# zhangganlin/GlORIE-SLAM

Measured on AMD Instinct MI355X. Metric: DSPO BA-update iters/sec + rendered rays/sec, 640x480 Replica keyframe graph, higher is better.
Workload: dtype f16 corr/ConvGRU, f32 Jacobians, f64 solve; render: f32 (decoder matmuls as 3-term f16 splits, f32 accumulate); 1 GPU; G8: 8 keyframes, 36 edges, 60x80 (640x480/8), BA itrs=2, DSPO stages alternating, context part of the GRU gates (one map per source keyframe) re-evaluated for all keyframes every 12 steps; multiview_filter.thresh = 0.25 (reference ships 0.01, configs/mono_point_slam.yaml:75: with untrained weights 0.01 rejects > 80 % of every frame and no depth_scale step would reach stage 2); render: 524k-point c; edges_local=36, edges_total=36, hw=4800, keyframes=8, parallelism=single GPU

## Files before the change

glorie_slam_amd/_lib.py:

```python
import ctypes
import os
import threading

import torch

_PKG_DIR = os.path.dirname(os.path.abspath(__file__))
LIB_PATH = os.path.join(_PKG_DIR, "lib", "libglorie_hip.so")

GLORIE_F16, GLORIE_F32 = 0, 1
_STATUS = {0: "GLORIE_OK", -1: "GLORIE_EINVAL", -2: "GLORIE_EHIP", -3: "GLORIE_ENOMEM",
           -4: "GLORIE_EUNSUPPORTED"}

_c_int, _c_f, _vp, _sz = ctypes.c_int, ctypes.c_float, ctypes.c_void_p, ctypes.c_size_t

SIGNATURES = {
    "glorie_version": (ctypes.c_char_p, []),
    "glorie_last_hip_error": (_c_int, []),
    "glorie_ctx_create": (_c_int, [ctypes.POINTER(_vp), _sz]),
    "glorie_ctx_destroy": (_c_int, [_vp]),
    "glorie_ctx_reserve": (_c_int, [_vp, _sz]),
    "glorie_ctx_generation": (ctypes.c_ulonglong, [_vp]),
    "glorie_corr_index_fwd": (_c_int, [_vp, _vp, _vp] + [_c_int] * 7 + [_vp]),
    "glorie_corr_lookup_pyramid": (_c_int, [_vp, _c_int, _vp, _vp] + [_c_int] * 7 + [_vp]),
    "glorie_corr_otf": (_c_int, [_vp, _vp, _c_int, _vp, _vp, _vp, _vp] + [_c_int] * 4 + [_vp]),
    "glorie_corr_otf_encode": (_c_int, [_vp, _vp, _c_int, _vp, _vp, _vp, _vp] + [_c_int] * 4 + [_vp, _vp, _vp, _c_int, _vp]),
    "glorie_altcorr_fwd": (_c_int, [_vp] * 4 + [_c_int] * 8 + [_vp]),
    "glorie_bias_act": (_c_int, [_vp, _c_int, _vp, _vp, _c_int, ctypes.c_long, _c_int, _c_int, _vp]),
    "glorie_gru_glo_terms": (_c_int, [_vp, _c_int, _vp, _vp, _c_int, _vp, _vp, _c_int, _vp, _c_int, _vp, _c_int, _c_int, _vp]),
    "glorie_gru_gate_zr": (_c_int, [_vp, _c_int, _vp, _c_int, _vp, _c_int, _vp, _c_int, _vp, _c_int, _c_int, _c_int, _vp]),
    "glorie_gru_gate_q": (_c_int, [_vp, _c_int, _vp, _c_int, _vp, _c_int, _vp, _c_int, _vp, _c_int, _vp, _c_int, _c_int, _c_int, _vp]),
    "glorie_segment_mean": (_c_int, [_vp, _c_int, _vp, _c_int, _vp, _c_int, _vp, _c_int, _c_int, _c_int, _vp]),
    "glorie_conv3x3_small": (_c_int, [_vp, _c_int, _vp, _c_int, _vp, _vp, _c_int, _c_int, _c_int, ctypes.c_float, _vp, _vp, _c_int, _c_int, _c_int, _vp]),
    "glorie_gru_glo_from_tiles": (_c_int, [_vp, _vp, _vp, _c_int, _vp, _c_int, _c_int, _vp]),
    "glorie_update_bookkeeping": (_c_int, [_vp, _vp, _vp, ctypes.c_long, _vp, _vp, _vp, _vp, _c_int, _c_int, _c_f, _vp, _c_int,
                                           _vp]),
    "glorie_conv_igemm_heads": (_c_int, [_vp, _c_int, _c_int, _vp, _c_int, _c_int, _vp, _vp, _c_int, _c_int, _vp, _vp,
                                         _c_int, _c_int, _c_int, _c_int, _vp]),
    "glorie_conv_upsample": (_c_int, [_vp, _c_int, _c_int, _vp, _vp, _vp, _vp, _vp, _c_int, _c_int, _c_int, _c_int, _vp]),
    "glorie_conv_stencil": (_c_int, [_vp, _vp, _c_int, _c_int, _c_int, ctypes.c_float, _vp, _vp, _c_int, _c_int, _c_int, _vp]),
    "glorie_conv_igemm": (_c_int, [_vp, _c_int, _c_int, _vp, _c_int, _c_int, _vp, _c_int, _c_int, _c_int, _vp,
                                   _c_int, _c_int, _vp, _c_int, _vp, _c_int, _vp, _c_int, _vp, _c_int, _vp, _c_int, _vp,
                                   _c_int, _c_int, _c_int, _vp]),
    "glorie_flow_conv7": (_c_int, [_vp, _vp, _vp, _vp, _c_int, _c_int, _c_int, _c_int, _vp]),
    "glorie_motion": (_c_int, [_vp, _vp, _vp, _vp, _c_int, _c_int, _c_int, ctypes.c_float, _vp]),
    "glorie_motion_padded": (_c_int, [_vp, _vp, _vp, _vp, _c_int, _c_int, _c_int, ctypes.c_float, _vp]),
    "glorie_flow_pad": (_c_int, [_vp, _vp, _c_int, _c_int, _c_int, _vp]),
    "glorie_flow_conv7_padded": (_c_int, [_vp, _vp, _vp, _vp, _c_int, _c_int, _c_int, _c_int, _vp]),
    "glorie_publish_flag": (_c_int, [_vp, _vp, _vp, _vp]),
    "glorie_dspo_prepare": (_c_int, [_vp] * 4 + [_c_int] * 4 + [ctypes.c_float, _c_int, ctypes.c_float, _vp, _vp, _c_int] + [_vp] * 9),
    "glorie_corr_lookup_pyramid_tiled": (_c_int, [_vp, _c_int, _vp, _vp] + [_c_int] * 5 + [_vp]),
    "glorie_corr_build": (_c_int, [_vp] * 5 + [_c_int] * 5 + [_vp]),
    "glorie_corr_lookup_arena": (_c_int, [_vp, _c_int, _vp, _vp, _vp] + [_c_int] * 5 + [_vp]),
    "glorie_corr_lookup_tiled_cl": (_c_int, [_vp, _c_int, _vp, _vp, _c_int, _vp] + [_c_int] * 5 + [_vp]),
    "glorie_corr_dm_level_halfs": (ctypes.c_long, [_c_int, _c_int, _c_int]),
    "glorie_corr_dm_build": (_c_int, [_vp] * 5 + [_c_int] * 5 + [_vp]),
    "glorie_corr_dm_lookup": (_c_int, [_vp, _vp, _vp, _c_int, _c_int, _c_int, _c_int, _vp, _vp, _vp, _vp, _c_int, _vp]),
    "glorie_valid_depth_mask": (_c_int, [_vp] * 4 + [_c_int] * 4 + [ctypes.c_float, _c_int, _vp, _vp, _vp]),
    "glorie_reproject": (_c_int, [_vp] * 7 + [_c_int] * 3 + [_vp]),
    "glorie_reproject_motion": (_c_int, [_vp] * 9 + [_c_int] * 3 + [ctypes.c_float, _vp]),
    "glorie_frame_distance": (_c_int, [_vp] * 6 + [_c_int] * 3 + [_c_f, _vp]),
    "glorie_iproj": (_c_int, [_vp] * 4 + [_c_int] * 3 + [_vp]),
    "glorie_depth_filter": (_c_int, [_vp] * 6 + [_c_int] * 4 + [_vp]),
    "glorie_cvx_upsample": (_c_int, [_vp] * 4 + [_c_int] * 5 + [_vp]),
    "glorie_cvx_upsample_nhwc": (_c_int, [_vp, _vp, _vp, _c_int, _vp, _c_int, _c_int, _c_int, _c_int, _vp]),
    "glorie_ba": (_c_int, [_vp] * 10 + [_c_int] * 8 + [_c_f, _c_f, _c_int, _c_int, _vp, _vp, _vp]),
    "glorie_ba_build_system": (_c_int, [_vp] * 10 + [_c_int] * 8 + [_vp, _vp]),
    "glorie_ba_solve_update": (_c_int, [_vp] * 5 + [_c_int] * 7 + [_c_f, _c_f, _c_int, _c_int] + [_vp] * 4),
    "glorie_ba_pack_system": (_c_int, [_vp, _vp, _c_int, _c_int, _vp]),
    "glorie_comm_unique_id": (_c_int, [_vp]),
    "glorie_comm_init": (_c_int, [_vp, _vp, _c_int, _c_int]),
    "glorie_comm_destroy": (_c_int, [_vp]),
    "glorie_comm_world": (_c_int, [_vp]),
    "glorie_allreduce_normal_eq": (_c_int, [_vp, _vp, _sz, _vp]),
    "glorie_allgather_rows": (_c_int, [_vp, _vp, _vp, _sz, _vp]),
    "glorie_dspo_scale_shift": (_c_int, [_vp] * 14 + [_c_int] * 6 + [_c_f, _c_f, _c_f, _vp, _vp]),
    "glorie_knn_build": (_c_int, [_vp, _vp, _c_int, _c_f, _c_int, _vp, _vp, _vp, _vp]),
    "glorie_knn_query": (_c_int, [_vp, _vp, _vp, _vp, _c_int, _c_int, _c_f, _vp, _vp, _vp, _vp, _vp]),
    "glorie_idw_gather": (_c_int, [_vp, _vp, _vp, _vp, _c_int, _c_int, _c_int, _c_f, _vp, _c_int,
                                   _c_int, _vp, _vp, _vp, _vp]),
    "glorie_knn_query_image": (_c_int, [_vp, _vp, _vp, _vp, _c_int, _c_int, _c_f, _vp, _vp, _vp, _vp, _c_int, _c_int,
                                        _vp]),
    "glorie_knn_query_weights": (_c_int, [_vp, _vp, _vp, _vp, _c_int, _c_f, _vp, _vp, _vp, _vp, _c_int, _c_int, _c_int, _c_int,
                                          _c_int, _vp, _vp, _vp]),
    "glorie_idw_gather2": (_c_int, [_vp, _vp, _vp, _vp, _vp, _c_int, _c_int, _c_int, _c_f, _vp, _c_int,
                                    _c_int, _vp, _vp, _vp, _vp, _vp]),
    "glorie_decoder_pack_floats": (_sz, []),
    "glorie_render_mlp": (_c_int, [_vp] * 10 + [_c_int, _vp, _vp, _c_int, _vp, _vp]),
    "glorie_composite": (_c_int, [_vp, _vp, _c_int, _c_int, _c_f, _vp, _vp, _vp, _vp, _vp]),
    "glorie_ray_samples": (_c_int, [_vp] * 5 + [_c_int, _c_int, _c_f, _c_f] + [_vp] * 6),
    "glorie_ray_samples_camera": (_c_int, [_vp, _c_int, ctypes.c_long] + [_vp] * 3 + [_c_int, _c_int, _c_f, _c_f] + [_vp] * 6),
    "glorie_proj_depth": (_c_int, [_vp, _vp, ctypes.c_long, _vp, _c_f, _c_f, _c_f, _c_f, _c_int, _c_int, _vp, _vp]),
    "glorie_ray_counts": (_c_int, [_vp, _c_int, _c_int, _c_int, _vp, _vp, _vp]),
    "glorie_render_train_workspace": (_sz, [ctypes.c_long]),
    "glorie_render_train_fwd": (_c_int, [_vp] * 9 + [ctypes.c_long, _c_int, _vp, _vp, _vp]),
    "glorie_render_train_bwd": (_c_int, [_vp] * 10 + [ctypes.c_long, _c_int, _vp, _vp, _vp, _vp, _vp]),
    "glorie_composite_bwd": (_c_int, [_vp, _vp, _c_int, _c_int, _c_f, _vp, _vp, _vp, _vp]),
    "glorie_adam_step": (_c_int, [_vp, _vp, _vp, _vp, ctypes.c_long, _c_f, _c_f, _c_f, _c_f, _c_int, _vp, _c_int, _vp]),
    "glorie_adam_multi": (_c_int, [_vp, _c_int, ctypes.c_long, _c_int, _vp, _vp]),
    "glorie_adam_step_dev": (_c_int, [_vp, _vp, _vp, _vp, ctypes.c_long, _c_f, _c_f, _c_f, _c_f, _vp, _vp, _c_int, _vp]),
    "glorie_adam_multi_dev": (_c_int, [_vp, _c_int, ctypes.c_long, _vp, _vp, _vp]),
    "glorie_counter_add": (_c_int, [_vp, _c_int, _vp]),
    "glorie_ba_status": (_c_int, [_vp, ctypes.POINTER(_c_int), _vp]),
    "glorie_ba_set_gate": (_c_int, [_vp, _vp, _vp]),
    "glorie_pix_warp_workspace": (_sz, [_c_int]),
    "glorie_pix_warp_fwd": (_c_int, [_vp] * 4 + [_c_int, _vp, _vp, _c_int, _vp, _vp, _c_int, _c_int, _c_int] + [_c_f] * 4
                            + [_vp, _c_int] + [_vp] * 5 + [_vp]),
    "glorie_pix_warp_bwd": (_c_int, [_vp, _vp, _vp, _c_int, _vp, _vp]),
    "glorie_frustum_select_workspace": (_sz, [_c_int]),
    "glorie_frustum_select": (_c_int, [_vp, _c_int, _vp] + [_c_f] * 4 + [_c_int, _c_int, _c_f] + [_vp] * 6),
    "glorie_keyframe_overlap": (_c_int, [_vp, _vp, _vp, _c_int, _c_int, _vp, _c_int] + [_c_f] * 4
                                + [_c_int, _c_int, _c_f, _vp, _vp]),
    "glorie_color_grad_maps": (_c_int, [_vp, _c_int, _c_int, _c_int, _vp] + [ctypes.c_double] * 4 + [_vp] * 6),
    "glorie_topm_workspace": (_sz, [_c_int]),
    "glorie_topm": (_c_int, [_vp, _c_int, _c_int, _vp, _vp, _vp, _vp]),
    "glorie_npc_deform_workspace": (_sz, [_c_int]),
    "glorie_npc_deform": (_c_int, [_vp] * 4 + [_c_int] * 3 + [_vp] * 5 + [ctypes.c_long, _vp, ctypes.c_long, _c_int]
                          + [_c_f, _c_f, _c_int] + [_c_f] * 4 + [_vp, _vp, _vp]),
    "glorie_iproj_dirty": (_c_int, [_vp] * 5 + [_c_int] * 3 + [_vp, _vp, _c_int, _vp]),
    "glorie_proxy_depth": (_c_int, [_vp, _vp] + [_c_int] * 4 + [_vp] + [_c_f] * 4 + [_vp] * 5),
}

_lib = None
_lock = threading.Lock()


class GlorieError(RuntimeError):
    pass


def load():
    global _lib
    with _lock:
        if _lib is None:
            if not os.path.exists(LIB_PATH):
                raise GlorieError(
                    f"{LIB_PATH} is missing: build it with `python glorie_slam_amd/build.py` "
                    "(or __graft_entry__.build()); there is no CPU fallback for the hot path")
            lib = ctypes.CDLL(LIB_PATH)
            for name, (res, args) in SIGNATURES.items():
                fn = getattr(lib, name)
                fn.restype = res
                fn.argtypes = args
            _lib = lib
    return _lib


def check(status, what):
    if status != 0:
        lib = load()
        raise GlorieError(f"{what} failed: {_STATUS.get(status, status)} "
                          f"(hipError {lib.glorie_last_hip_error()})")


def stream_ptr(device=None):
    return ctypes.c_void_p(torch.cuda.current_stream(device).cuda_stream)


def ptr(t):
    return ctypes.c_void_p(t.data_ptr()) if t is not None else ctypes.c_void_p(0)


BA_TARGETS_HWC = 2


def need_cuda(*tensors):
    for t in tensors:
        if t is not None and not t.is_cuda:
            raise GlorieError("glorie_hip kernels take device tensors; got a CPU tensor "
                              "(there is no CPU fallback on the product path)")


def need_contiguous(**named):
    for k, t in named.items():
        if t is not None and not t.is_contiguous():
            raise RuntimeError(f"{k} must be contiguous")


def dtype_code(t):
    if t.dtype == torch.float16:
        return GLORIE_F16
    if t.dtype == torch.float32:
        return GLORIE_F32
    raise GlorieError(f"unsupported dtype {t.dtype}")


class Context:
# ... 36 lines not shown
```

glorie_slam_amd/csrc/ba.hip:

```cpp
#include <hip/hip_runtime.h>
#include <stdint.h>
#include <math.h>
#include "common.hiph"
#include "se3.hiph"
#include "ba_common.hiph"

namespace glorie {

__device__ __forceinline__ void block_inclusive_scan(int* a, int n) {
  const int tid = threadIdx.x;
  for (int off = 1; off < n; off <<= 1) {
    int tmp[4];
#pragma unroll
    for (int q = 0; q < 4; ++q) {
      const int f = tid + q * 1024;
      tmp[q] = (f < n) ? a[f] + (f >= off ? a[f - off] : 0) : 0;
    }
    __syncthreads();
#pragma unroll
    for (int q = 0; q < 4; ++q) {
      const int f = tid + q * 1024;
      if (f < n) a[f] = tmp[q];
    }
    __syncthreads();
// ... 986 lines not shown
}

constexpr int kPanelRows = 128;
__global__ __launch_bounds__(1024) void chol_panel_gemm_kernel(BaWork wk, int n, int j0, int nb) {
  if (ba_skipped(wk)) return;
  __shared__ double Wl[kCB * kCBP], P[kPanelRows * kCBP];
  if (wk.status[0] & (BA_ST_SOLVE_ABORT | BA_ST_M_MISMATCH)) return;
  const int tid = threadIdx.x, br = tid >> 5, bc = tid & 31;
  double* A = wk.Hd;
  const int base = j0 + nb, rem = n - base;
  if (br < nb && bc < nb) {
    double v = 0.0;
    if (bc < br) v = A[(size_t)(j0 + bc) * n + j0 + br];
    else if (bc == br) v = 1.0 / A[(size_t)(j0 + br) * n + j0 + br];
    Wl[br * kCBP + bc] = v;
  }
  const int t0 = blockIdx.x * kPanelRows;
  for (int idx = tid; idx < kPanelRows * kCB; idx += 1024) {
    const int tl = idx >> 5, m = idx & 31, t = t0 + tl;
    P[tl * kCBP + m] = (t <= rem && m < nb) ? A[(size_t)(t < rem ? base + t : n) * n + j0 + m] : 0.0;
  }
  __syncthreads();
  const int tl = tid & (kPanelRows - 1), g = tid >> 7, t = t0 + tl;
  double x[4];
#pragma unroll
  for (int q = 0; q < 4; ++q) x[q] = 0.0;
  const double* wg = Wl + g * kCBP;
  const double* ap = P + tl * kCBP;
#pragma unroll 4
  for (int m = 0; m < kCB; ++m) {
    const double am = ap[m];
#pragma unroll
    for (int q = 0; q < 4; ++q) x[q] = fma(am, (m <= 8 * q + g) ? wg[8 * q * kCBP + m] : 0.0, x[q]);
  }
  if (t <= rem) {
    double* arow = A + (size_t)(t < rem ? base + t : n) * n + j0;
#pragma unroll
    for (int q = 0; q < 4; ++q) {
      const int c = 8 * q + g;
      if (c < nb) arow[c] = x[q];
    }
  }
}

__global__ __launch_bounds__(256) void chol_backsub_block_kernel(BaWork wk, int n, int j0, int nb) {
  if (ba_skipped(wk)) return;
  __shared__ double Wl[kCB * kCBP], yb[kCB], xb[kCB];
  const int tid = threadIdx.x;
  double* A = wk.Hd;
  double* y = A + (size_t)n * n;
  if (wk.status[0] & (BA_ST_SOLVE_ABORT | BA_ST_M_MISMATCH)) {
    if (blockIdx.x == 0 && tid < nb) wk.dx[j0 + tid] = 0.0f;
    return;
  }
  for (int idx = tid; idx < kCB * kCB; idx += 256) {
    const int r = idx >> 5, c = idx & 31;
    double v = 0.0;
    if (r < nb && c < nb) {
      if (c < r) v = A[(size_t)(j0 + c) * n + j0 + r];
      else if (c == r) v = 1.0 / A[(size_t)(j0 + r) * n + j0 + r];
    }
    Wl[r * kCBP + c] = v;
  }
  if (tid < kCB) yb[tid] = tid < nb ? y[j0 + tid] : 0.0;
  __syncthreads();
  if (tid < kCB) {
    double v = 0.0;
    for (int r = tid; r < nb; ++r) v = fma(Wl[r * kCBP + tid], yb[r], v);
    xb[tid] = v;
  }
  __syncthreads();
  if (blockIdx.x == 0 && tid < nb) wk.dx[j0 + tid] = (float)xb[tid];
  const int r = blockIdx.x * 256 + tid;
  if (r < j0) {
    double v = y[r];
    for (int c = 0; c < nb; ++c) v -= A[(size_t)(j0 + c) * n + r] * xb[c];
    y[r] = v;
  }
}

__global__ __launch_bounds__(kBaThreads) void ba_update_kernel(
    BaWork wk, float* __restrict__ poses, float* __restrict__ disps,
    const int64_t* __restrict__ ii, const int64_t* __restrict__ jj, int HW, int t0, int t1,
    int motion_only, int depth_only, float* __restrict__ dx_out, float* __restrict__ dz_out) {
  if (ba_skipped(wk)) return;
  constexpr int EB = 128;
  __shared__ float ys[EB * 6];
  const int tid = threadIdx.x;
  const int s = blockIdx.y;
  if (wk.status[0] & BA_ST_M_MISMATCH) return;
  const int P = t1 - t0;
  if (blockIdx.x == 0 && s == 0) {
    for (int p = tid; p < P; p += kBaThreads) {
      float xi[6];
#pragma unroll
      for (int q = 0; q < 6; ++q) xi[q] = wk.dx[p * 6 + q];
      if (dx_out) {
#pragma unroll
        for (int q = 0; q < 6; ++q) dx_out[p * 6 + q] = xi[q];
      }
      if (!depth_only) {
        float* pp = poses + (size_t)(t0 + p) * 7;
        const Pose g = se3_retract(xi, load_pose(pp));
        pp[0] = g.t.x; pp[1] = g.t.y; pp[2] = g.t.z;
        pp[3] = g.q.x; pp[4] = g.q.y; pp[5] = g.q.z; pp[6] = g.q.w;
      }
    }
  }
  if (motion_only) return;
  const int k = wk.kx[s];
  const int e0 = wk.csr_ptr[s];
  const int deg = wk.csr_ptr[s + 1] - e0;
  const int pk = k - t0;
  const bool self_on = (pk > 0 && pk < P);
  const int px = blockIdx.x * kBaThreads + tid;
  float dw = 0.0f;
  for (int a0 = 0; a0 < deg; a0 += EB) {
    const int nb = min(EB, deg - a0);
    __syncthreads();
    for (int idx = tid; idx < nb * 6; idx += kBaThreads) {
      const int a = idx / 6, r = idx % 6;
      const int n = wk.csr_edge[e0 + a0 + a];
      const int pj = (int)jj[n] - t0;
      float y = (pj > 0 && pj < P) ? wk.dx[pj * 6 + r] : 0.0f;
      if (self_on) {
        const float* L = wk.Ledge + (size_t)n * 36;
        float acc = 0.0f;
#pragma unroll
        for (int m = 0; m < 6; ++m) acc += L[m * 6 + r] * wk.dx[pk * 6 + m];
        y -= acc;
      }
      ys[idx] = y;
    }
    __syncthreads();
    if (px < HW) {
      for (int a = 0; a < nb; ++a) {
        const int n = wk.csr_edge[e0 + a0 + a];
#pragma unroll
        for (int r = 0; r < 6; ++r) dw += wk.Eij[((size_t)n * 6 + r) * HW + px] * ys[a * 6 + r];
      }
    }
  }
  if (px >= HW) return;
  const float dz = wk.Q[(size_t)s * HW + px] * (wk.W[(size_t)s * HW + px] - dw);
  disps[(size_t)k * HW + px] += dz;
  if (dz_out) dz_out[(size_t)s * HW + px] = dz;
}

int ba_prepare(const BaWork& wk, const int64_t* ii, int B, int N, int M, int t0, int t1,
               hipStream_t st) {
  const size_t prep_lds = sizeof(int) * ((size_t)3 * B + (size_t)N);
  if (prep_lds > 150 * 1024) return GLORIE_EUNSUPPORTED;
  static PerDeviceOnce attr_set;
  if (attr_set.first()) {
    (void)hipFuncSetAttribute(reinterpret_cast<const void*>(ba_prepare_kernel),
                              hipFuncAttributeMaxDynamicSharedMemorySize, 150 * 1024);
  }
  hipLaunchKernelGGL(ba_prepare_kernel, dim3(1), dim3(1024), prep_lds, st, wk, ii, B, N, M, t0, t1);
  return check_launch();
}

}

using namespace glorie;

namespace glorie {

struct BaPlan {
  BaWork wk;
  int B, N, M, h, w, HW, t0, t1, P, n6, ppt, chunk_px, nchunks;
  size_t scratch_used;
};

static int ba_plan(glorie_ctx* ctx, int B, int N, int M, int h, int w, int t0, int t1,
                   double* hv_ext, BaPlan& pl) {
  if (!ctx || B < 0 || N < 0 || M < 0 || h < 0 || w < 0 || t1 < t0) return GLORIE_EINVAL;
  if (B > kMaxFramesLds || N > kMaxEdgesLds || t1 > B) return GLORIE_EUNSUPPORTED;
  pl.B = B; pl.N = N; pl.M = M; pl.h = h; pl.w = w; pl.HW = h * w; pl.t0 = t0; pl.t1 = t1;
  pl.P = t1 - t0; pl.n6 = 6 * pl.P;
#ifdef EXP_BA_CHUNK_WGS
  constexpr long kChunkWgs = EXP_BA_CHUNK_WGS;
#else
  constexpr long kChunkWgs = 256;
#endif
  int ppt = 1;
  const int per1 = (pl.HW + kBaThreads - 1) / kBaThreads;
  while (ppt < 4 && (long)M * ((per1 + ppt - 1) / ppt) > kChunkWgs) ++ppt;
  pl.ppt = ppt;
  pl.chunk_px = kBaThreads * ppt;
  pl.nchunks = (pl.HW + pl.chunk_px - 1) / pl.chunk_px;
  const size_t HW = pl.HW, n6 = pl.n6;
  size_t off = 0;
  auto carve = [&](size_t bytes) { size_t o = off; off = align_up(off + bytes, 256); return o; };
  const size_t o_slot = carve(sizeof(int) * (size_t)B);
  const size_t o_kx = carve(sizeof(int) * (size_t)(M + 1));
  const size_t o_ptr = carve(sizeof(int) * (size_t)(M + 2));
  const size_t o_edge = carve(sizeof(int) * (size_t)N);
  const size_t o_L = carve(sizeof(float) * 36 * (size_t)N);
  const size_t o_E = carve(sizeof(float) * 6 * (size_t)N * HW);
  const size_t o_Hp = carve(sizeof(float) * 27 * (size_t)N * pl.nchunks);
  const size_t o_Q = carve(sizeof(float) * (size_t)M * HW);
  const size_t o_W = carve(sizeof(float) * (size_t)M * HW);
  const size_t o_CW = carve(sizeof(float) * 2 * (size_t)N * HW);
  const size_t o_Hd = carve(sizeof(double) * (n6 * n6 + n6));
  const size_t o_acc = carve(2 * sizeof(unsigned long long) * (n6 * n6 + n6));
  const size_t o_dx = carve(sizeof(float) * n6);
  GLORIE_TRY(ctx_reserve(ctx, off));
  pl.scratch_used = off;
  char* base = reinterpret_cast<char*>(ctx->scratch);
  BaWork& wk = pl.wk;
  wk.slot_of_frame = reinterpret_cast<int*>(base + o_slot);
  wk.kx = reinterpret_cast<int*>(base + o_kx);
  wk.csr_ptr = reinterpret_cast<int*>(base + o_ptr);
  wk.csr_edge = reinterpret_cast<int*>(base + o_edge);
  wk.status = ctx->dstatus;
  wk.Ledge = reinterpret_cast<float*>(base + o_L);
  wk.Eij = reinterpret_cast<float*>(base + o_E);
  wk.Hpart = reinterpret_cast<float*>(base + o_Hp);
  wk.Q = reinterpret_cast<float*>(base + o_Q);
  wk.W = reinterpret_cast<float*>(base + o_W);
  wk.CWpart = reinterpret_cast<float*>(base + o_CW);
  wk.Hd = hv_ext ? hv_ext : reinterpret_cast<double*>(base + o_Hd);
  wk.vd = wk.Hd + n6 * n6;
  wk.Hacc = reinterpret_cast<unsigned long long*>(base + o_acc);
  wk.dx = reinterpret_cast<float*>(base + o_dx);
  wk.gate = ctx->ba_gate;
  wk.gate_hits = nullptr;
  static PerDeviceOnce attr_set;
  if (attr_set.first()) {
    (void)hipFuncSetAttribute(reinterpret_cast<const void*>(ba_solve_fused_kernel),
                              hipFuncAttributeMaxDynamicSharedMemorySize, 160 * 1024 - 64);
    (void)hipFuncSetAttribute(reinterpret_cast<const void*>(ba_solve_band_kernel),
                              hipFuncAttributeMaxDynamicSharedMemorySize, 160 * 1024 - 64);
  }
  return GLORIE_OK;
}

static int ba_build_system(const BaPlan& pl, const float* poses, const float* disps,
                           const float* intrinsics, const float* disps_sens, const float* targets,
                           const float* weights, const float* eta, const int64_t* ii,
                           const int64_t* jj, int flags, bool to_f64, hipStream_t st) {
  const BaWork& wk = pl.wk;
  const int motion_only = flags & 1, hwc = (flags & GLORIE_BA_TARGETS_HWC) ? 1 : 0;
  hipLaunchKernelGGL(ba_jacobian_kernel, dim3(pl.nchunks, pl.N), dim3(kBaThreads), 0, st, wk, poses,
                     disps, intrinsics, disps_sens, targets, weights, eta, ii, jj, pl.HW, pl.w,
                     pl.nchunks, pl.ppt, motion_only, hwc, (long)pl.n6 * pl.n6 + pl.n6);
  if (!motion_only)
    hipLaunchKernelGGL(ba_gram_kernel, dim3(pl.nchunks, pl.M), dim3(kBaThreads), 0, st, wk, ii, jj, pl.HW,
                       pl.chunk_px, pl.t0, pl.t1, pl.nchunks, eta, disps, disps_sens);
  else
    hipLaunchKernelGGL(ba_assemble_kernel, dim3(pl.N), dim3(64), 0, st, wk, ii, jj, pl.nchunks, pl.t0, pl.t1);
  if (to_f64) {
    const long total = (long)pl.n6 * pl.n6 + pl.n6;
    hipLaunchKernelGGL(ba_system_f64_kernel, dim3((unsigned)((total + 255) / 256)), dim3(256), 0, st, wk, total);
  }
  return check_launch();
}

static int ba_solve_update(const BaPlan& pl, float* poses, float* disps, const int64_t* ii,
                           const int64_t* jj, float lm, float ep, int motion_only, int depth_only,
                           float* dx_out, float* dz_out, bool from_acc, hipStream_t st) {
  const BaWork& wk = pl.wk;
  const int n6 = pl.n6;
  if (n6 <= kSolveMaxN) {
    const int bwf = n6 > 1 ? n6 - 1 : 1;
    const int need = n6 * (bwf + 1) + 2 * n6;
    hipLaunchKernelGGL(ba_solve_band_kernel, dim3(1), dim3(kBandThreads), sizeof(double) * (size_t)need, st, wk, n6,
                       lm, ep, need, bwf, from_acc ? 1 : 0);
  } else if (n6 <= kFusedMaxN) {
    const size_t rows = (size_t)(n6 + 1 > kCB ? n6 + 1 - kCB : 1);
    const size_t lds = sizeof(double) * (2 * kCB * kCBP + (rows * kCBP > (size_t)n6 ? rows * kCBP : (size_t)n6));
    const int band_doubles = (160 * 1024 - 256) / (int)sizeof(double);
    hipLaunchKernelGGL(ba_bandwidth_kernel, dim3(n6), dim3(64), 0, st, wk, n6);
    hipLaunchKernelGGL(ba_solve_band_kernel, dim3(1), dim3(kBandThreads), sizeof(double) * (size_t)band_doubles, st,
                       wk, n6, lm, ep, band_doubles, -1, 0);
    hipLaunchKernelGGL(ba_solve_fused_kernel, dim3(1), dim3(1024), lds, st, wk, n6, lm, ep);
  } else {
    hipLaunchKernelGGL(chol_damp_kernel, dim3((n6 + 255) / 256), dim3(256), 0, st, wk, n6, lm, ep);
    for (int j0 = 0; j0 < n6; j0 += kCB) {
      const int nb = (n6 - j0 < kCB) ? (n6 - j0) : kCB;
      const int rem = n6 - j0 - nb;
      hipLaunchKernelGGL(chol_diag_inv_kernel, dim3(1), dim3(1024), 0, st, wk, n6, j0, nb);
      hipLaunchKernelGGL(chol_panel_gemm_kernel, dim3((rem + kPanelRows) / kPanelRows), dim3(1024), 0, st, wk, n6, j0, nb);
      if (rem > 0) {
        const int tl = (rem + kTrailTile) / kTrailTile;
        hipLaunchKernelGGL(chol_trail_kernel, dim3(tl, tl), dim3(256), 0, st, wk, n6, j0, nb);
      }
    }
    for (int j0 = ((n6 - 1) / kCB) * kCB; j0 >= 0; j0 -= kCB) {
      const int nb = (n6 - j0 < kCB) ? (n6 - j0) : kCB;
      hipLaunchKernelGGL(chol_backsub_block_kernel, dim3(j0 > 0 ? (j0 + 255) / 256 : 1), dim3(256), 0, st, wk, n6, j0,
                         nb);
    }
  }
  const int upd_chunks = (pl.HW + kBaThreads - 1) / kBaThreads;
  hipLaunchKernelGGL(ba_update_kernel, dim3(upd_chunks, pl.M), dim3(kBaThreads), 0, st, wk, poses,
                     disps, ii, jj, pl.HW, pl.t0, pl.t1, motion_only, depth_only, dx_out, dz_out);
  return check_launch();
}

__global__ __launch_bounds__(256) void ba_zero_gated_kernel(const int* __restrict__ gate, int* __restrict__ dstatus,
                                                            double* __restrict__ hv, size_t n) {
  if (*gate != 0) return;
  const size_t i = (size_t)blockIdx.x * 256 + threadIdx.x;
  if (i < 4) dstatus[i] = 0;
  if (i < n) hv[i] = 0.0;
}

}

extern "C" int glorie_ba(glorie_ctx* ctx, float* poses, float* disps, const float* intrinsics,
                         const float* disps_sens, const float* targets, const float* weights,
                         const float* eta, const int64_t* ii, const int64_t* jj, int B, int N,
                         int M, int h, int w, int t0, int t1, int iterations, float lm, float ep,
                         int motion_only, int depth_only, float* dx_out, float* dz_out,
                         void* stream) {
  if (iterations < 0) return GLORIE_EINVAL;
  const int flags = motion_only;
  motion_only = flags & 1;
  BaPlan pl;
  GLORIE_TRY(ba_plan(ctx, B, N, M, h, w, t0, t1, nullptr, pl));
  if (N == 0 || pl.P == 0 || pl.HW == 0 || iterations == 0) return GLORIE_OK;
  if (!poses || !disps || !intrinsics || !targets || !weights || !ii || !jj) return GLORIE_EINVAL;
  if (!motion_only && !eta) return GLORIE_EINVAL;
  hipStream_t st = (hipStream_t)stream;
  GLORIE_TRY(ctx_poison(ctx, pl.scratch_used, st));
  {
    BaWork w0 = pl.wk;
    if (ctx->ba_gate && ctx->ba_gate_count) { w0.gate_hits = ctx->ba_gate_hits; ctx->ba_gate_count = false; }
    GLORIE_TRY(ba_prepare(w0, ii, B, N, M, t0, t1, st));
  }
  const bool direct = pl.n6 <= kSolveMaxN;
  for (int it = 0; it < iterations; ++it) {
    GLORIE_TRY(ba_build_system(pl, poses, disps, intrinsics, disps_sens, targets, weights, eta, ii, jj,
                               flags, !direct, st));
    GLORIE_TRY(ba_solve_update(pl, poses, disps, ii, jj, lm, ep, motion_only, depth_only, dx_out,
                               dz_out, direct, st));
  }
  return GLORIE_OK;
}

extern "C" int glorie_ba_build_system(glorie_ctx* ctx, const float* poses, const float* disps,
                                      const float* intrinsics, const float* disps_sens,
                                      const float* targets, const float* weights, const float* eta,
                                      const int64_t* ii, const int64_t* jj, int B, int N, int M,
                                      int h, int w, int t0, int t1, int motion_only, double* hv_out,
                                      void* stream) {
  BaPlan pl;
  GLORIE_TRY(ba_plan(ctx, B, N, M, h, w, t0, t1, hv_out, pl));
  if (!hv_out || pl.P == 0) return GLORIE_EINVAL;
  hipStream_t st = (hipStream_t)stream;
  if (N == 0 || pl.HW == 0) {
    const size_t nhv = (size_t)pl.n6 * pl.n6 + pl.n6;
    if (ctx->ba_gate) {
      hipLaunchKernelGGL(ba_zero_gated_kernel, dim3((unsigned)((nhv + 255) / 256)), dim3(256), 0, st, ctx->ba_gate,
                         ctx->dstatus, hv_out, nhv);
      return check_launch();
    }
    GLORIE_TRY(check_hip(hipMemsetAsync(ctx->dstatus, 0, 4 * sizeof(int), st)));
    return check_hip(hipMemsetAsync(hv_out, 0, sizeof(double) * nhv, st));
  }
  if (!poses || !disps || !intrinsics || !targets || !weights || !ii || !jj) return GLORIE_EINVAL;
  if (!(motion_only & 1) && !eta) return GLORIE_EINVAL;
  GLORIE_TRY(ctx_poison(ctx, pl.scratch_used, st));
  {
    BaWork w0 = pl.wk;
    if (ctx->ba_gate && ctx->ba_gate_count) { w0.gate_hits = ctx->ba_gate_hits; ctx->ba_gate_count = false; }
    GLORIE_TRY(ba_prepare(w0, ii, B, N, M, t0, t1, st));
  }
  return ba_build_system(pl, poses, disps, intrinsics, disps_sens, targets, weights, eta, ii, jj,
                         motion_only, true, st);
}

extern "C" int glorie_ba_solve_update(glorie_ctx* ctx, float* poses, float* disps,
                                      const int64_t* ii, const int64_t* jj, int B, int N, int M,
                                      int h, int w, int t0, int t1, float lm, float ep,
                                      int motion_only, int depth_only, const double* hv,
                                      float* dx_out, float* dz_out, void* stream) {
  BaPlan pl;
  GLORIE_TRY(ba_plan(ctx, B, N, M, h, w, t0, t1, const_cast<double*>(hv), pl));
  if (!hv || !poses || !disps || pl.P == 0) return GLORIE_EINVAL;
  if (N > 0 && (!ii || !jj)) return GLORIE_EINVAL;
  hipStream_t st = (hipStream_t)stream;
  if (N == 0 || pl.HW == 0) {
    pl.M = 1;
    return ba_solve_update(pl, poses, disps, ii, jj, lm, ep, 1, depth_only, dx_out,
                           nullptr, false, st);
  }
  return ba_solve_update(pl, poses, disps, ii, jj, lm, ep, motion_only, depth_only, dx_out, dz_out,
                         false, st);
}

extern "C" int glorie_ba_set_gate(glorie_ctx* ctx, const int* run_if_zero, int* hits) {
  if (!ctx) return GLORIE_EINVAL;
  ctx->ba_gate = run_if_zero;
  ctx->ba_gate_hits = run_if_zero ? hits : nullptr;
  ctx->ba_gate_count = run_if_zero && hits;
  return GLORIE_OK;
}

namespace glorie {
__global__ __launch_bounds__(256) void hv_pack_kernel(const double* __restrict__ hv, double* __restrict__ packed,
                                                      int n, int unpack) {
  const int r = blockIdx.y, c = blockIdx.x * 256 + threadIdx.x;
  double* dense = const_cast<double*>(hv);
  if (r == n) {
    if (c < n) {
      const size_t k = (size_t)n * (n + 1) / 2 + c;
      if (unpack) dense[(size_t)n * n + c] = packed[k];
      else packed[k] = hv[(size_t)n * n + c];
    }
    return;
  }
  if (c > r) return;
  const size_t k = (size_t)r * (r + 1) / 2 + c;
  if (unpack) dense[(size_t)r * n + c] = packed[k];
  else packed[k] = hv[(size_t)r * n + c];
}
}

extern "C" int glorie_ba_pack_system(const double* hv, double* packed, int n6, int unpack, void* stream) {
  if (!hv || !packed || n6 < 0) return GLORIE_EINVAL;
  if (n6 == 0) return GLORIE_OK;
  hipLaunchKernelGGL(glorie::hv_pack_kernel, dim3((n6 + 255) / 256, n6 + 1), dim3(256), 0, (hipStream_t)stream, hv,
                     packed, n6, unpack);
  return glorie::check_launch();
}

extern "C" int glorie_ba_status(glorie_ctx* ctx, int* status_out, void* stream) {
  if (!ctx || !status_out) return GLORIE_EINVAL;
  hipStream_t st = (hipStream_t)stream;
  GLORIE_TRY(check_hip(hipMemcpyAsync(status_out, ctx->dstatus, sizeof(int) * 4, hipMemcpyDeviceToHost, st)));
  return check_hip(hipStreamSynchronize(st));
}
```

glorie_slam_amd/csrc/conv.hip:

```cpp
#include <hip/hip_runtime.h>
#include <stdint.h>
#include <stdlib.h>
#include <string.h>
#include <type_traits>
#include "common.hiph"

namespace glorie {

typedef __attribute__((ext_vector_type(8))) _Float16 f16x8;
typedef __attribute__((ext_vector_type(4))) _Float16 f16x4;
typedef __attribute__((ext_vector_type(4))) float f32x4;

enum { EPI_BIAS_ACT = 0, EPI_GRU_ZR = 1, EPI_GRU_Q = 2, EPI_GLO = 3, EPI_HEADS = 4, EPI_UPSAMPLE = 5 };
enum { CACT_NONE = 0, CACT_RELU = 1, CACT_SIGMOID = 2 };

struct ConvArgs {
  const _Float16* xa; int xa_stride; int cha;
  const _Float16* xb; int xb_stride; int chb;
  const _Float16* w;
  int taps, npad, nout;
  long P; int H, W, HW;
  _Float16* out; int out_stride;
  _Float16* out2; int out2_stride;
  const float* terms; int terms_stride; int act;
// ... 286 lines not shown
      t[rb][ni] = s;
    }
  }
  float* red = reinterpret_cast<float*>(smem);
  __syncthreads();
  if (wm == 1) {
#pragma unroll
    for (int rb = 0; rb < 2; ++rb)
#pragma unroll
      for (int ni = 0; ni < NB; ++ni)
#pragma unroll
        for (int r = 0; r < 4; ++r) red[((wn * 8 + rb * 4 + ni) * 4 + r) * 64 + lane] = t[rb][ni][r];
  }
  __syncthreads();
  if (wm == 0) {
#pragma unroll
    for (int ni = 0; ni < NB; ++ni) {
      const long p = p0 + wn * 64 + ni * 16 + col;
      if (p >= a.P) continue;
      float* dst = a.tap_out + (size_t)(grp * a.tap_ncols) * a.P + p;
#pragma unroll
      for (int rb = 0; rb < 2; ++rb) {
        const int n = rb * 16 + kg * 4;
#pragma unroll
        for (int r = 0; r < 4; ++r) {
          const float v = t[rb][ni][r] + red[((wn * 8 + rb * 4 + ni) * 4 + r) * 64 + lane];
          if (n + r < a.tap_ncols) dst[(size_t)(n + r) * a.P] = v;
        }
      }
    }
  }
}

template <int MB, int NB>
__device__ __forceinline__ void conv_epilogue_glo(const ConvArgs& a, f32x4 (&acc)[MB][NB], long p0, long pbase, int wm,
                                                  int wn, int kg, int col, char* smem, int tile) {
  static_assert(MB == 4, "128-channel tile");
  const long pend = (p0 / a.HW + 1) * a.HW;
  float s0[MB][4];
#pragma unroll
  for (int mi = 0; mi < MB; ++mi)
#pragma unroll
    for (int k = 0; k < 4; ++k) s0[mi][k] = 0.0f;
  const int nb = wm * 64 + kg * 4;
#pragma unroll
  for (int ni = 0; ni < NB; ++ni) {
    const long p = pbase + ni * 16;
    const bool okp = p < pend;
    const long pc = okp ? p : pend - 1;
#pragma unroll
    for (int mi = 0; mi < MB; ++mi) {
      const int n = nb + mi * 16;
      const float4 b = *reinterpret_cast<const float4*>(a.terms + n);
      const f16x4 nv = *reinterpret_cast<const f16x4*>(a.net + pc * a.net_stride + n);
      const f32x4 v = acc[mi][ni];
      s0[mi][0] += okp ? csigmoid(v[0] + b.x) * (float)nv[0] : 0.0f;
      s0[mi][1] += okp ? csigmoid(v[1] + b.y) * (float)nv[1] : 0.0f;
      s0[mi][2] += okp ? csigmoid(v[2] + b.z) * (float)nv[2] : 0.0f;
      s0[mi][3] += okp ? csigmoid(v[3] + b.w) * (float)nv[3] : 0.0f;
    }
  }
#pragma unroll
  for (int mi = 0; mi < MB; ++mi)
#pragma unroll
    for (int k = 0; k < 4; ++k)
#pragma unroll
      for (int off = 8; off > 0; off >>= 1) s0[mi][k] += __shfl_xor(s0[mi][k], off, 64);
  float* red = reinterpret_cast<float*>(smem);
  __syncthreads();
  if (col == 0) {
#pragma unroll
    for (int mi = 0; mi < MB; ++mi)
#pragma unroll
      for (int k = 0; k < 4; ++k) red[wn * 128 + nb + mi * 16 + k] = s0[mi][k];
  }
  __syncthreads();
  const int tid = threadIdx.x;
  if (tid < 128) reinterpret_cast<float*>(a.out)[(size_t)tile * 128 + tid] = red[tid] + red[128 + tid];
}

__device__ __forceinline__ float round_prob(float v, bool f32) { return f32 ? v : (float)(_Float16)v; }

template <int MB, int NB>
__device__ __forceinline__ void conv_epilogue_upsample(const ConvArgs& a, f32x4 (&acc)[MB][NB], long p0, int n0, int wm,
                                                       int wn, int kg, int col, char* smem) {
  static_assert(MB == 4 && NB == 4, "128 x 128 tile");
  _Float16* T = reinterpret_cast<_Float16*>(smem);
  float4 bias[MB];
#pragma unroll
  for (int mi = 0; mi < MB; ++mi) bias[mi] = *reinterpret_cast<const float4*>(a.terms + n0 + wm * 64 + mi * 16 + kg * 4);
  __syncthreads();
#pragma unroll
  for (int ni = 0; ni < NB; ++ni) {
    const int pl = wn * 64 + ni * 16 + col;
#pragma unroll
    for (int mi = 0; mi < MB; ++mi) {
      const int b = wm * 4 + mi;
      const f32x4 v = acc[mi][ni];
      const f16x4 h = {(_Float16)(v[0] + bias[mi].x), (_Float16)(v[1] + bias[mi].y), (_Float16)(v[2] + bias[mi].z),
                       (_Float16)(v[3] + bias[mi].w)};
      *reinterpret_cast<f16x4*>(T + pl * 128 + ((b ^ (pl & 7)) * 16 + kg * 4)) = h;
    }
  }
  __syncthreads();
  const int tid = threadIdx.x;
  const int pl = tid & 127, hb = tid >> 7;
  const long p = p0 + pl;
  if (p >= a.P) return;
  const int asub = n0 >> 7;
  const int m = (int)(p / a.HW);
  const int q = (int)(p - (long)m * a.HW);
  const int y = q / a.W, x = q - y * a.W;
  const int frame = (int)a.up_ix[m];
  const float* dmap = a.up_disps + (size_t)frame * a.HW;
  float nb[9];
#pragma unroll
  for (int k = 0; k < 9; ++k) {
    const int yy = y + k / 3 - 1, xx = x + k % 3 - 1;
    const bool in = yy >= 0 && yy < a.H && xx >= 0 && xx < a.W;
    nb[k] = dmap[in ? yy * a.W + xx : q];
    if (!in) nb[k] = 0.0f;
  }
  float outv[4];
#pragma unroll
  for (int j = 0; j < 4; ++j) {
    const int b = hb * 4 + j;
    const f16x8* src = reinterpret_cast<const f16x8*>(T + pl * 128 + (b ^ (pl & 7)) * 16);
    const f16x8 lo = src[0], hi = src[1];
    float v[9];
#pragma unroll
    for (int k = 0; k < 8; ++k) v[k] = (float)lo[k];
    v[8] = (float)hi[0];
    float mx = v[0];
#pragma unroll
    for (int k = 1; k < 9; ++k) mx = fmaxf(mx, v[k]);
    float e[9], sum = 0.0f;
#pragma unroll
    for (int k = 0; k < 9; ++k) { e[k] = expf(v[k] - mx); sum += e[k]; }
    float o = 0.0f;
#pragma unroll
    for (int k = 0; k < 9; ++k)
      o = __fadd_rn(o, __fmul_rn(round_prob(e[k] / sum, a.up_f32 != 0), nb[k]));
    outv[j] = o;
  }
  float* dst = a.up_out + (size_t)frame * 64 * a.HW + (size_t)(8 * y + asub) * (8 * a.W) + 8 * x + hb * 4;
  *reinterpret_cast<float4*>(dst) = make_float4(outv[0], outv[1], outv[2], outv[3]);
}

template <int EPI, int NB, int BK, int NW, int ST, int MB = 4>
__global__ __launch_bounds__(64 * NW, (ST == 1 && MB * NB <= 16) ? 3 : 2) void conv_igemm_kernel(ConvArgs a) {
  constexpr int TN = 32 * MB;
  static_assert(ST == 1 || ST == 2, "LDS stages");
#if defined(__HIP_DEVICE_COMPILE__)
  constexpr int PT = (NW / 2) * 16 * NB;
  constexpr int RB = BK * 2;
  constexpr int SL = RB / 16;
  constexpr int RPI = 64 / SL;
  constexpr int XI = PT / RPI / NW;
  constexpr int WI = TN / RPI / NW;
  constexpr int XBYTES = PT * RB, WBYTES = TN * RB;
  constexpr int KK = BK / 32;
  extern __shared__ __attribute__((aligned(16))) char smem[];
  const int tid = threadIdx.x, lane = tid & 63, wv = tid >> 6;
  const int col = lane & 15, kg = lane >> 4;
  const int wm = wv & 1, wn = wv >> 1;

  auto key = [](int row) { return RB == 128 ? (row & 7) : ((row >> 1) & 3); };

  const int nwg = gridDim.x, ntn = (a.nout + TN - 1) / TN;
  const int xcd = blockIdx.x & 7, q = nwg >> 3, r = nwg & 7;
  const int lid = (xcd < r ? xcd * (q + 1) : r * (q + 1) + (xcd - r) * q) + (blockIdx.x >> 3);
  const int pt = lid / ntn, nt = lid - pt * ntn;
  const int tpm = (a.HW + PT - 1) / PT;
  const long p0 = EPI == EPI_GLO ? (long)(pt / tpm) * a.HW + (long)(pt % tpm) * PT : a.pbeg + (long)pt * PT;
  const int n0 = nt * TN;

  const int cpc = 64 / BK;
  const int nsteps_tap = (a.cha + a.chb) * cpc;
  const int C = (a.cha + a.chb) * 64;
  const int T = a.taps * nsteps_tap;

  const int back = a.taps == 9 ? a.W + 1 : 0;
  const __amdgpu_buffer_rsrc_t rA = __builtin_amdgcn_make_buffer_rsrc(
      (void*)(a.xa - (long)back * a.xa_stride), 0, 0x7fffffff, 0x00020000);
  const __amdgpu_buffer_rsrc_t rB = __builtin_amdgcn_make_buffer_rsrc(
      (void*)(a.xb - (long)back * a.xb_stride), 0, 0x7fffffff, 0x00020000);
  const __amdgpu_buffer_rsrc_t rW = __builtin_amdgcn_make_buffer_rsrc((void*)a.w, 0, 0x7fffffff, 0x00020000);

  const int srow = lane / SL, slot = lane % SL;
  const int row0 = wv * RPI + srow;
  const int sw0 = (slot ^ key(row0)) << 3;
  const unsigned voffA0 = (unsigned)(((p0 + row0) * a.xa_stride + sw0) * 2);
  const unsigned voffB0 = (unsigned)(((p0 + row0) * a.xb_stride + sw0) * 2);
  const unsigned woff0 = (unsigned)(((size_t)row0 * C + sw0) * 2);
  int vmask[XI];
#pragma unroll
  for (int i = 0; i < XI; ++i) {
    const long p = p0 + (i * NW + wv) * RPI + srow;
    int m = 0;
    if (p < a.P) {
      const int pi_ = (int)p, xw = pi_ % a.W, yh = (pi_ / a.W) % a.H;
      if (a.taps == 9) {
#pragma unroll
        for (int d = 0; d < 9; ++d) {
          const int dy = d / 3 - 1, dx = d % 3 - 1;
          if ((unsigned)(yh + dy) < (unsigned)a.H && (unsigned)(xw + dx) < (unsigned)a.W) m |= 1 << d;
        }
      } else {
        m = 1;
      }
    }
    vmask[i] = m;
  }

  auto stage = [&](int t, int buf) {
    const int per_chunk = a.taps * cpc;
    const int ch = t / per_chunk, rem = t - ch * per_chunk;
    const int d = rem / cpc, sub = rem - d * cpc;
    const int shift = (a.taps == 9 ? (d / 3 - 1) * a.W + (d % 3 - 1) : 0) + back;
    const bool segA = ch < a.cha;
    const int xs = segA ? a.xa_stride : a.xb_stride;
    const unsigned xsoff = (unsigned)((shift * xs + (segA ? ch : ch - a.cha) * 64 + sub * BK) * 2);
    const unsigned wsoff = (unsigned)((((size_t)d * a.npad + n0) * C + ch * 64 + sub * BK) * 2);
    char* lx = smem + buf * (XBYTES + WBYTES);
    char* lw = lx + XBYTES;
    const unsigned xstep = (unsigned)(NW * RPI * xs * 2), wstep = (unsigned)(NW * RPI * C * 2);
#ifdef EXP_NO_PIXEL_DMA
    if (d == 0)
#endif
// ... 843 lines not shown
  long full_pt = pt_all * ntn / ncu * ncu / ntn;
  full_pt -= full_pt % 8;
  if (full_pt < 0) full_pt = 0;
  long rest_px = a.P - full_pt * 512;
  int nbr = 4;
  long rest_pt = 0;
  if (rest_px > 0) {
    const long per_cu = (rest_px * ntn + ncu - 1) / ncu;
    nbr = (int)((per_cu + 127) / 128);
    if (nbr > 4 || full_pt == 0) nbr = 4;
    if (nbr < 1) nbr = 1;
    rest_pt = (rest_px + 128 * nbr - 1) / (128 * nbr);
  }
  if (nbr == 4) { full_pt = pt_all; rest_pt = 0; }
  const long nwg = (full_pt + rest_pt) * ntn;
  if (nwg <= 0) return GLORIE_OK;
  if (nwg > 0x7fffffffL) return GLORIE_EINVAL;
  a.pp_full = (int)(full_pt * ntn);
  a.pp_nbr = nbr;
  const dim3 grid((unsigned)nwg);
  switch (epilogue) {
    case EPI_BIAS_ACT: launch_ppw_one<EPI_BIAS_ACT>(a, grid, st); break;
    case EPI_GRU_Q: launch_ppw_one<EPI_GRU_Q>(a, grid, st); break;
    case EPI_HEADS: launch_ppw_one<EPI_HEADS>(a, grid, st); break;
    default: return GLORIE_EUNSUPPORTED;
  }
  return check_launch();
}

template <int MB>
static int launch_conv_halo(const ConvArgs& a, int epilogue, hipStream_t st) {
  constexpr int PT = 128, TN = 32 * MB;
  if (a.pair && (MB % 2)) return GLORIE_EINVAL;
  const long ptiles = (a.P - a.pbeg + PT - 1) / PT;
  if (ptiles <= 0) return GLORIE_OK;
  const long nwg = ptiles * ((a.nout + TN - 1) / TN);
  if (nwg > 0x7fffffffL) return GLORIE_EINVAL;
  const dim3 grid((unsigned)nwg);
  const size_t lds = halo_lds_bytes(a.W, MB);
  switch (epilogue) {
    case EPI_BIAS_ACT: launch_halo_one<EPI_BIAS_ACT, MB>(a, grid, lds, st); break;
    case EPI_GRU_ZR: launch_halo_one<EPI_GRU_ZR, MB>(a, grid, lds, st); break;
    case EPI_GRU_Q:
      if constexpr (MB == 4) launch_halo_one<EPI_GRU_Q, MB>(a, grid, lds, st);
      else return GLORIE_EUNSUPPORTED;
      break;
    case EPI_HEADS:
      if constexpr (MB == 4) launch_halo_one<EPI_HEADS, MB>(a, grid, lds, st);
      else return GLORIE_EUNSUPPORTED;
      break;
    default: return GLORIE_EUNSUPPORTED;
  }
  return check_launch();
}

template <int NB, int BK, int NW, int ST, int MB = 4>
static int launch_conv(const ConvArgs& a, int epilogue, hipStream_t st, long max_ptiles = -1) {
  constexpr int PT = (NW / 2) * 16 * NB;
  if (a.pair && (MB % 2)) return GLORIE_EINVAL;
  long ptiles = (a.P - a.pbeg + PT - 1) / PT;
  if (epilogue == EPI_GLO) ptiles = (a.P / a.HW) * ((a.HW + PT - 1) / PT);
  if (max_ptiles >= 0) ptiles = ptiles < max_ptiles ? ptiles : max_ptiles;
  if (ptiles <= 0) return GLORIE_OK;
  const long nwg = ptiles * ((a.nout + 32 * MB - 1) / (32 * MB));
  if (nwg > 0x7fffffffL) return GLORIE_EINVAL;
  const dim3 grid((unsigned)nwg);
  switch (epilogue) {
    case EPI_BIAS_ACT: launch_one<EPI_BIAS_ACT, NB, BK, NW, ST, MB>(a, grid, st); break;
    case EPI_GRU_ZR: launch_one<EPI_GRU_ZR, NB, BK, NW, ST, MB>(a, grid, st); break;
    case EPI_GLO:
      if constexpr (MB == 4 && NB == 4 && NW == 4 && ST == 1) launch_one<EPI_GLO, NB, BK, NW, ST, MB>(a, grid, st);
      else return GLORIE_EUNSUPPORTED;
      break;
    case EPI_HEADS:
      if constexpr (MB == 4 && NB == 4 && NW == 4 && ST == 1) launch_one<EPI_HEADS, NB, BK, NW, ST, MB>(a, grid, st);
      else return GLORIE_EUNSUPPORTED;
      break;
    case EPI_UPSAMPLE:
      if constexpr (MB == 4 && NB == 4 && NW == 4 && ST == 1) launch_one<EPI_UPSAMPLE, NB, BK, NW, ST, MB>(a, grid, st);
      else return GLORIE_EUNSUPPORTED;
      break;
    default: launch_one<EPI_GRU_Q, NB, BK, NW, ST, MB>(a, grid, st); break;
  }
  return check_launch();
}

}

using namespace glorie;

static int conv_igemm_impl(const void* xa, int xa_stride, int ca, const void* xb, int xb_stride,
                           int cb, const void* w_packed, int taps, int nout, int epilogue,
                           const float* terms, int terms_stride, int act, const void* net,
                           int net_stride, const void* z, int z_stride, void* out, int out_stride,
                           void* out2, int out2_stride, const void* pre, int pre_stride, const int* pre_map,
                           int N, int H, int W, void* stream, const void* tap_w, float* tap_out, int tap_groups,
                           int tap_ncols, const float* up_disps = nullptr, const int64_t* up_ix = nullptr,
                           float* up_out = nullptr, int up_f32 = 0) {
  if (N < 0 || H <= 0 || W <= 0 || (taps != 1 && taps != 9) || nout <= 0 || (nout & 3)) return GLORIE_EINVAL;
  if (ca < 0 || cb < 0 || (ca % 64) || (cb % 64) || ca + cb == 0) return GLORIE_EINVAL;
  const int pair = (epilogue >> 8) & 1;
  const int policy = (epilogue >> 12) & 15;
  epilogue &= 0xff;
  if (policy > 7) return GLORIE_EINVAL;
  if (epilogue < 0 || epilogue > 5) return GLORIE_EINVAL;
  if (pair && (epilogue > EPI_GRU_Q || (nout & 31))) return GLORIE_EINVAL;
  if (epilogue == EPI_UPSAMPLE && (!up_disps || !up_ix || !up_out || !terms || nout != 1024 || taps != 1 || pre))
    return GLORIE_EINVAL;
  if (epilogue == EPI_HEADS && (!tap_w || !tap_out || !terms || tap_groups < 1 || tap_ncols < 1 || tap_ncols > 32 ||
                                nout < 128 * tap_groups || (nout & 127) || act != CACT_RELU || pre))
    return GLORIE_EINVAL;
  if (N == 0) return GLORIE_OK;
  if ((ca && (!xa || (xa_stride & 7))) || (cb && (!xb || (xb_stride & 7)))) return GLORIE_EINVAL;
  if (!w_packed || !out || (out_stride & 3)) return GLORIE_EINVAL;
  if (epilogue == EPI_GRU_ZR && (nout != 256 || !terms || !net || !out2 || (terms_stride & 3))) return GLORIE_EINVAL;
  if (epilogue == EPI_GRU_Q && (nout != 128 || !terms || !net || !z || (terms_stride & 3))) return GLORIE_EINVAL;
  if (pre && (epilogue == EPI_BIAS_ACT || epilogue == EPI_GLO || (pre_stride & 3))) return GLORIE_EINVAL;
  if (epilogue == EPI_GLO && (nout != 128 || taps != 1 || !terms || !net)) return GLORIE_EINVAL;
  ConvArgs a;
  a.xa = reinterpret_cast<const _Float16*>(xa); a.xa_stride = xa_stride; a.cha = ca / 64;
  a.xb = reinterpret_cast<const _Float16*>(xb); a.xb_stride = xb_stride; a.chb = cb / 64;
  a.w = reinterpret_cast<const _Float16*>(w_packed);
  a.taps = taps; a.nout = nout; a.npad = (nout + kTileN - 1) / kTileN * kTileN;
  a.P = (long)N * H * W; a.H = H; a.W = W; a.HW = H * W;
  a.out = reinterpret_cast<_Float16*>(out); a.out_stride = out_stride;
  a.out2 = reinterpret_cast<_Float16*>(out2); a.out2_stride = out2_stride;
  a.terms = terms; a.terms_stride = terms_stride; a.act = act;
  a.net = reinterpret_cast<const _Float16*>(net); a.net_stride = net_stride;
  a.z = reinterpret_cast<const _Float16*>(z); a.z_stride = z_stride;
  a.pre = reinterpret_cast<const _Float16*>(pre); a.pre_stride = pre_stride; a.pre_map = pre ? pre_map : nullptr;
  a.pbeg = 0;
  a.tap_w = reinterpret_cast<const f16x8*>(tap_w); a.tap_out = tap_out; a.tap_groups = tap_groups;
  a.tap_ncols = tap_ncols;
  a.up_disps = up_disps; a.up_ix = up_ix; a.up_out = up_out; a.up_f32 = up_f32;
  a.pair = pair;
  a.pp_full = 0; a.pp_nbr = 4;
#ifdef EXP_CONV_STAMPS
  a.stamps = getenv("GLORIE_CONV_STAMPS") ? (unsigned long long*)strtoull(getenv("GLORIE_CONV_STAMPS"), nullptr, 0) : nullptr;
#else
  a.stamps = nullptr;
#endif
  const long lim = 0x7fffffffL;
  if (((a.P + W + 2) * (long)xa_stride + 64) * 2 > lim || ((a.P + W + 2) * (long)xb_stride + 64) * 2 > lim ||
      ((long)taps * a.npad * (ca + cb) + 64) * 2 > lim || (pre && (a.P * (long)pre_stride + 512) * 2 > lim) ||
      (a.P * (long)out_stride + nout) * 2 > lim || (out2 && (a.P * (long)out2_stride + 128) * 2 > lim))
    return GLORIE_EINVAL;
  hipStream_t st = (hipStream_t)stream;
  if (policy == 6) return launch_conv_pp(a, epilogue, st);
  if (policy == 7) return launch_conv_ppw(a, epilogue, st);
  {
    const char* ppw = getenv("GLORIE_CONV_PPW");
    const bool fits = (nout & 127) == 0 && (epilogue == EPI_BIAS_ACT || epilogue == EPI_GRU_Q || epilogue == EPI_HEADS);
    const bool want = ppw ? ppw[0] == '1' : (taps == 9 && (nout == 128 || epilogue == EPI_HEADS) && epilogue != EPI_BIAS_ACT &&
                                             a.P >= kConvPpwMinPixels);
    if (policy == 0 && fits && want && !(ppw && ppw[0] == '0')) return launch_conv_ppw(a, epilogue, st);
  }
  {
    if (policy == 0 && taps == 9 && a.pbeg == 0) {
      const long tiles128 = (a.P + 127) / 128 * ((nout + 127) / 128);
      if (nout > 64 && (nout & 255) != 0 && W <= 83 && (epilogue <= EPI_GRU_Q || epilogue == EPI_HEADS) &&
          !(epilogue == EPI_BIAS_ACT && tiles128 <= 384))
        return launch_conv_halo<4>(a, epilogue, st);
    }
  }
  if (epilogue == EPI_HEADS || epilogue == EPI_UPSAMPLE) return launch_conv<4, 64, 4, 1>(a, epilogue, st);
  if (nout <= 64 && epilogue == EPI_BIAS_ACT) return launch_conv<4, 64, 4, 1, 2>(a, epilogue, st);
  const int ntn = (nout + 127) / 128;
  const long slots128 = 3L * 256;
  const long full_rounds = ((a.P + 127) / 128 * ntn) / slots128;
  const long pt_a = full_rounds * slots128 / ntn;
  const char t0c = policy == 1 ? '1' : policy == 2 ? '6' : policy == 3 ? 's' : policy == 4 ? 'w' : 0;
  if (policy == 0 && (nout & 255) == 0 && taps == 9 && epilogue <= EPI_GRU_ZR && a.P >= 256L * 256)
    return launch_conv_pp(a, epilogue, st);
  if (t0c == 0 && (nout & 255) == 0) return launch_conv<4, 64, 4, 1, 8>(a, epilogue, st);
  if (t0c == 0 && epilogue == EPI_BIAS_ACT && (a.P + 127) / 128 * ntn <= 384) return launch_conv<2, 64, 4, 1>(a, epilogue, st);
  if (t0c == 0 && epilogue == EPI_BIAS_ACT && taps == 1) return launch_conv<2, 64, 4, 1>(a, epilogue, st);
  if (t0c == 'w') return launch_conv<8, 64, 4, 1, 4>(a, epilogue, st);
  if (t0c == '6') return launch_conv<2, 64, 4, 1>(a, epilogue, st);
  if (t0c == 's' && full_rounds >= 1) {
    const int rc_a = launch_conv<4, 64, 4, 1>(a, epilogue, st, pt_a);
    if (rc_a != GLORIE_OK) return rc_a;
    a.pbeg = pt_a * 128;
    return a.pbeg < a.P ? launch_conv<2, 64, 4, 1>(a, epilogue, st) : GLORIE_OK;
  }
  return launch_conv<4, 64, 4, 1>(a, epilogue, st);
}

extern "C" int glorie_conv_igemm(const void* xa, int xa_stride, int ca, const void* xb, int xb_stride,
                                 int cb, const void* w_packed, int taps, int nout, int epilogue,
                                 const float* terms, int terms_stride, int act, const void* net,
                                 int net_stride, const void* z, int z_stride, void* out, int out_stride,
                                 void* out2, int out2_stride, const void* pre, int pre_stride, const int* pre_map,
                                 int N, int H, int W, void* stream) {
  if ((epilogue & 0xff) == EPI_HEADS || (epilogue & 0xff) == EPI_UPSAMPLE) return GLORIE_EINVAL;
  return conv_igemm_impl(xa, xa_stride, ca, xb, xb_stride, cb, w_packed, taps, nout, epilogue, terms, terms_stride, act,
                         net, net_stride, z, z_stride, out, out_stride, out2, out2_stride, pre, pre_stride, pre_map, N, H,
                         W, stream, nullptr, nullptr, 0, 0);
}

extern "C" int glorie_conv_igemm_heads(const void* x, int x_stride, int c, const void* w_packed, int taps, int nout,
                                       const float* bias, const void* tap_w, int groups, int K, float* tap_out,
                                       void* out, int out_stride, int N, int H, int W, void* stream) {
  if (K < 1 || K > 3 || groups < 1 || groups > 4) return GLORIE_EINVAL;
  if (nout > 128 * groups && !out) return GLORIE_EINVAL;
  void* o = out ? out : (void*)tap_out;
  return conv_igemm_impl(x, x_stride, c, nullptr, 0, 0, w_packed, taps, nout, EPI_HEADS, bias, 0, CACT_RELU, nullptr, 0,
                         nullptr, 0, o, out ? out_stride : 4, nullptr, 0, nullptr, 0, nullptr, N, H, W, stream, tap_w,
                         tap_out, groups, 9 * K);
}

extern "C" int glorie_conv_upsample(const void* x, int x_stride, int c, const void* w_packed, const float* bias,
                                    const float* disps, const int64_t* ix, float* disps_up, int softmax_f32, int M,
                                    int H, int W, void* stream) {
  if (!disps || !ix || !disps_up || !bias) return GLORIE_EINVAL;
  return conv_igemm_impl(x, x_stride, c, nullptr, 0, 0, w_packed, 1, 1024, EPI_UPSAMPLE, bias, 0, CACT_NONE, nullptr, 0,
                         nullptr, 0, disps_up, 4, nullptr, 0, nullptr, 0, nullptr, M, H, W, stream, nullptr, nullptr, 0,
                         0, disps, ix, disps_up, softmax_f32);
}
```

glorie_slam_amd/csrc/dspo.hip:

```cpp
#include <hip/hip_runtime.h>
#include <stdint.h>
#include "common.hiph"
#include "se3.hiph"
#include "ba_common.hiph"

namespace glorie {

struct Dspo2Args {
  const float* poses;
  float* disps;
  const float* intr;
  const float* mono;
  float* scales;
  float* shifts;
  const uint8_t* vmask;
  const float* target;
  const float* weight;
  const float* eta;
  const int64_t* ii;
  const int64_t* jj;
  const uint8_t* edge_on;
  float alpha;
};

// ... 57 lines not shown
  }
}

__global__ __launch_bounds__(kBaThreads) void dspo2_accum_kernel(BaWork wk, Dspo2Args a, int HW,
                                                                 int w, int nchunks) {
  __shared__ float red[4][10];
  const int tid = threadIdx.x, lane = tid & 63, wv = tid >> 6;
  const int chunk = blockIdx.x, s = blockIdx.y;
  if (wk.status[0] & BA_ST_M_MISMATCH) return;
  const int k = wk.kx[s];
  const int e0 = wk.csr_ptr[s], e1 = wk.csr_ptr[s + 1];
  const int px = chunk * kBaThreads + tid;
  const bool live = px < HW;
  float Cp = 0.0f, Wp = 0.0f;
  int n_on = 0;
  const float fxi = a.intr[k * 4 + 0], fyi = a.intr[k * 4 + 1];
  const float cxi = a.intr[k * 4 + 2], cyi = a.intr[k * 4 + 3];
  const int yy = live ? px / w : 0, xx = live ? px - yy * w : 0;
  const float dsp = live ? a.disps[(size_t)k * HW + px] : 1.0f;
  for (int ei = e0; ei < e1; ++ei) {
    const int n = wk.csr_edge[ei];
    if (a.edge_on && !a.edge_on[n]) continue;
    ++n_on;
    const int jx = (int)a.jj[n];
    const Pose g = (jx == k) ? stereo_pose()
                             : relative_pose(load_pose(a.poses + k * 7), load_pose(a.poses + jx * 7));
    const float fxj = a.intr[jx * 4 + 0], fyj = a.intr[jx * 4 + 1];
    const float cxj = a.intr[jx * 4 + 2], cyj = a.intr[jx * 4 + 3];
    if (!live) continue;
    float X0[4], X1[4];
    X0[0] = ((float)xx - cxi) / fxi;
    X0[1] = ((float)yy - cyi) / fyi;
    X0[2] = 1.0f;
    X0[3] = dsp;
    se3_act(g, X0, X1);
    const float Z = (X1[2] < 0.1f) ? 1.0f : X1[2];
    const float d = 1.0f / Z;
    const float cu = fxj * (X1[0] * d) + cxj, cv = fyj * (X1[1] * d) + cyj;
    const float valid = (X1[2] > 0.2f) ? 1.0f : 0.0f;
    const float2 tg = reinterpret_cast<const float2*>(a.target)[(size_t)n * HW + px];
    const float2 wg = reinterpret_cast<const float2*>(a.weight)[(size_t)n * HW + px];
    const float wu = 0.001f * (valid * wg.x), wvv = 0.001f * (valid * wg.y);
    const float ru = tg.x - cu, rv = tg.y - cv;
    const float Jzu = fxj * d * g.t.x - fxj * X1[0] * d * d * g.t.z;
    const float Jzv = fyj * d * g.t.y - fyj * X1[1] * d * d * g.t.z;
    Cp += wu * Jzu * Jzu + wvv * Jzv * Jzv;
    Wp += wu * ru * Jzu + wvv * rv * Jzv;
  }
  if (n_on != 0) {
    float sums[10];
#pragma unroll
    for (int q = 0; q < 10; ++q) sums[q] = 0.0f;
    if (live) {
      const float mono = a.mono[(size_t)k * HW + px];
      const PriorJ J = prior_jacobians(mono, a.vmask[(size_t)k * HW + px] != 0, a.alpha);
      const float rd = sqrtf(a.alpha) * (dsp - (a.scales[k] * mono + a.shifts[k]));
      const float C = Cp + J.Jd * J.Jd + a.eta[(size_t)s * HW + px];
      const float Wv = Wp - J.Jd * rd;
      const float Q = 1.0f / C;
      wk.Q[(size_t)s * HW + px] = Q;
      wk.W[(size_t)s * HW + px] = Wv;
      const float e1v = J.Js * J.Jd, e2v = J.Jq * J.Jd;
      sums[0] = J.Js * J.Js; sums[1] = J.Js * J.Jq; sums[2] = J.Jq * J.Jq;
      sums[3] = e1v * Q * e1v; sums[4] = e1v * Q * e2v; sums[5] = e2v * Q * e2v;
      sums[6] = -J.Js * rd; sums[7] = -J.Jq * rd;
      sums[8] = e1v * Q * Wv; sums[9] = e2v * Q * Wv;
    }
#pragma unroll
    for (int q = 0; q < 10; ++q) sums[q] = wave_sum(sums[q]);
    if (lane == 0) {
#pragma unroll
      for (int q = 0; q < 10; ++q) red[wv][q] = sums[q];
    }
    __syncthreads();
    if (tid < 10)
      wk.Hpart[((size_t)s * nchunks + chunk) * 10 + tid] =
          (red[0][tid] + red[1][tid]) + (red[2][tid] + red[3][tid]);
  }
}

template <bool INLINE>
__global__ __launch_bounds__(kBaThreads) void dspo2_update_kernel(BaWork wk, Dspo2Args a, int HW,
                                                                  float* __restrict__ dz_out, int M, int nchunks,
                                                                  float lm, float ep) {
  __shared__ double vsum[INLINE ? 25 * 10 : 1];
  __shared__ float sdx[INLINE ? 2 * 25 : 1];
  __shared__ int fail;
  const int tid = threadIdx.x;
  const int s = blockIdx.y;
  if (wk.status[0] & BA_ST_M_MISMATCH) return;
  float ds, dq;
  if constexpr (INLINE) {
    if (tid == 0) fail = 0;
    if (tid < 10 * M) {
      const int f = tid / 10, q = tid - f * 10;
      double v = 0.0;
      for (int c = 0; c < nchunks; ++c) v += (double)wk.Hpart[((size_t)f * nchunks + c) * 10 + q];
      vsum[tid] = v;
    }
    __syncthreads();
    if (tid < M) {
      const bool on = frame_enabled(wk, a.edge_on, tid);
      double x1 = 0.0, x2 = 0.0;
      if (on) {
        const double* v = vsum + tid * 10;
        const double H11 = v[0] + ep + lm * v[0], H22 = v[2] + ep + lm * v[2];
        const double S11 = H11 - v[3], S12 = v[1] - v[4], S22 = H22 - v[5];
        const double b1 = v[6] - v[8], b2 = v[7] - v[9];
        const double l21 = (S11 > 0.0) ? S12 / sqrt(S11) : 0.0;
        const double l22sq = S22 - l21 * l21;
        if (!(S11 > 0.0) || !(l22sq > 0.0)) {
          atomicOr(&fail, 1);
        } else {
          const double det = S11 * S22 - S12 * S12;
          x1 = (S22 * b1 - S12 * b2) / det;
          x2 = (S11 * b2 - S12 * b1) / det;
        }
      }
      sdx[2 * tid + 0] = (float)x1;
      sdx[2 * tid + 1] = (float)x2;
    }
    __syncthreads();
    ds = fail ? 0.0f : sdx[2 * s + 0];
    dq = fail ? 0.0f : sdx[2 * s + 1];
    if (blockIdx.x == 0 && s == 0) {
      if (tid < 2 * M) wk.dx[tid] = fail ? 0.0f : sdx[tid];
      if (tid == 0 && fail) {
        atomicOr(&wk.status[0], BA_ST_CHOL_FAILED);
        atomicAdd(&wk.status[2], 1);
      }
    }
  } else {
    ds = wk.dx[2 * s + 0];
    dq = wk.dx[2 * s + 1];
  }
  if (!frame_enabled(wk, a.edge_on, s)) return;
  const int k = wk.kx[s];
  if (blockIdx.x == 0 && tid == 0) {
    a.scales[k] += ds;
    a.shifts[k] += dq;
  }
  const int px = blockIdx.x * kBaThreads + tid;
  if (px >= HW) return;
  const PriorJ J = prior_jacobians(a.mono[(size_t)k * HW + px], a.vmask[(size_t)k * HW + px] != 0, a.alpha);
  const float dz = wk.Q[(size_t)s * HW + px] *
                   (wk.W[(size_t)s * HW + px] - (J.Js * J.Jd * ds + J.Jq * J.Jd * dq));
  a.disps[(size_t)k * HW + px] = fmaxf(a.disps[(size_t)k * HW + px] + dz, 0.0f);
  if (dz_out) dz_out[(size_t)s * HW + px] = dz;
}

}

using namespace glorie;

extern "C" int glorie_dspo_scale_shift(glorie_ctx* ctx, const float* poses, float* disps,
                                       const float* intrinsics, const float* mono_disps,
                                       float* scales, float* shifts, const uint8_t* valid_mask,
                                       const float* target, const float* weight, const float* eta,
                                       const int64_t* ii, const int64_t* jj, const uint8_t* edge_on,
                                       int B, int N, int M, int h, int w, int iterations, float lm,
                                       float ep, float alpha, float* dz_out, void* stream) {
  if (!ctx || B < 0 || N < 0 || M < 0 || h < 0 || w < 0 || iterations < 0) return GLORIE_EINVAL;
  const int HW = h * w;
  if (N == 0 || M == 0 || HW == 0 || iterations == 0) return GLORIE_OK;
  if (!poses || !disps || !intrinsics || !mono_disps || !scales || !shifts || !valid_mask || !target ||
      !weight || !eta || !ii || !jj)
    return GLORIE_EINVAL;
  if (B > kMaxFramesLds || N > kMaxEdgesLds) return GLORIE_EUNSUPPORTED;
  hipStream_t st = (hipStream_t)stream;
  const int nchunks = (HW + kBaThreads - 1) / kBaThreads;
  size_t off = 0;
  auto carve = [&](size_t bytes) { size_t o = off; off = align_up(off + bytes, 256); return o; };
  const size_t o_slot = carve(sizeof(int) * (size_t)B);
  const size_t o_kx = carve(sizeof(int) * (size_t)(M + 1));
  const size_t o_ptr = carve(sizeof(int) * (size_t)(M + 2));
  const size_t o_edge = carve(sizeof(int) * (size_t)N);
  const size_t o_Hp = carve(sizeof(float) * 10 * (size_t)M * nchunks);
  const size_t o_Q = carve(sizeof(float) * (size_t)M * HW);
  const size_t o_W = carve(sizeof(float) * (size_t)M * HW);
  const size_t o_dx = carve(sizeof(float) * 2 * (size_t)M);
  GLORIE_TRY(ctx_reserve(ctx, off));
  GLORIE_TRY(ctx_poison(ctx, off, st));
  char* base = reinterpret_cast<char*>(ctx->scratch);
  BaWork wk{};
  wk.slot_of_frame = reinterpret_cast<int*>(base + o_slot);
  wk.kx = reinterpret_cast<int*>(base + o_kx);
  wk.csr_ptr = reinterpret_cast<int*>(base + o_ptr);
  wk.csr_edge = reinterpret_cast<int*>(base + o_edge);
  wk.status = ctx->dstatus;
  wk.Hpart = reinterpret_cast<float*>(base + o_Hp);
  wk.Q = reinterpret_cast<float*>(base + o_Q);
  wk.W = reinterpret_cast<float*>(base + o_W);
  wk.dx = reinterpret_cast<float*>(base + o_dx);
  GLORIE_TRY(ba_prepare(wk, ii, B, N, M, 0, 0, st));
  Dspo2Args a{poses, disps, intrinsics, mono_disps, scales, shifts, valid_mask, target, weight, eta,
              ii, jj, edge_on, alpha};
  for (int it = 0; it < iterations; ++it) {
    hipLaunchKernelGGL(dspo2_accum_kernel, dim3(nchunks, M), dim3(kBaThreads), 0, st, wk, a, HW, w, nchunks);
    if (M <= 25) {
      hipLaunchKernelGGL(dspo2_update_kernel<true>, dim3(nchunks, M), dim3(kBaThreads), 0, st, wk, a, HW, dz_out, M,
                         nchunks, lm, ep);
    } else {
      hipLaunchKernelGGL(dspo2_solve_kernel, dim3(1), dim3(256), 0, st, wk, a, M, nchunks, lm, ep);
      hipLaunchKernelGGL(dspo2_update_kernel<false>, dim3(nchunks, M), dim3(kBaThreads), 0, st, wk, a, HW, dz_out, M,
                         nchunks, lm, ep);
    }
    GLORIE_TRY(check_launch());
  }
  return GLORIE_OK;
}
```

glorie_slam_amd/csrc/gru.hip:

```cpp
#include <hip/hip_runtime.h>
#include <stdint.h>
#include "common.hiph"

namespace glorie {

typedef __attribute__((ext_vector_type(8))) _Float16 h8;

__device__ __forceinline__ float sigmoidf_(float x) { return 1.0f / (1.0f + __expf(-x)); }
__device__ __forceinline__ float tanhf_(float x) {
  const float e = __expf(-2.0f * fabsf(x));
  const float t = (1.0f - e) / (1.0f + e);
  return copysignf(t, x);
}

enum { ACT_NONE = 0, ACT_RELU = 1, ACT_SIGMOID = 2, ACT_SOFTPLUS = 3 };

template <int C8T>
__global__ __launch_bounds__(256) void bias_act_kernel(const _Float16* __restrict__ x, int xs,
                                                       const float* __restrict__ bias,
                                                       _Float16* __restrict__ y, int ys, long P,
                                                       int C8R, int act) {
  const int C8 = C8T ? C8T : C8R;
  const long idx = (long)blockIdx.x * 256 + threadIdx.x;
  if (idx >= P * C8) return;
// ... 188 lines not shown
template <int NT>
__global__ __launch_bounds__(256) void conv_taps_kernel(const _Float16* __restrict__ x, int xs,
                                                        const float* __restrict__ in_bias, int in_relu,
                                                        const f16x8* __restrict__ wp,
                                                        float* __restrict__ taps, int ncols, int tstride,
                                                        long P) {
  const int lane = threadIdx.x & 63, wv = threadIdx.x >> 6;
  const int col = lane & 15, kg = lane >> 4;
  const int grp = blockIdx.y;
  f16x8 bfrag[NT][4];
#pragma unroll
  for (int t = 0; t < NT; ++t)
#pragma unroll
    for (int kk = 0; kk < 4; ++kk) bfrag[t][kk] = wp[(((size_t)grp * NT + t) * 4 + kk) * 64 + lane];
  float ib[4][8];
#pragma unroll
  for (int kk = 0; kk < 4; ++kk)
#pragma unroll
    for (int k = 0; k < 8; ++k) ib[kk][k] = in_bias ? in_bias[grp * 128 + kk * 32 + kg * 8 + k] : 0.0f;
  const long ntiles = (P + 15) / 16;
  for (long tile = (long)blockIdx.x * 4 + wv; tile < ntiles; tile += (long)gridDim.x * 4) {
    const long p0 = tile * 16;
    const long pa = min(p0 + col, P - 1);
    const f16x8* src = reinterpret_cast<const f16x8*>(x + pa * xs + grp * 128 + kg * 8);
    f16x8 afrag[4];
#pragma unroll
    for (int kk = 0; kk < 4; ++kk) afrag[kk] = src[kk * 4];
    if (in_bias || in_relu) {
#pragma unroll
      for (int kk = 0; kk < 4; ++kk)
#pragma unroll
        for (int k = 0; k < 8; ++k) {
          float f = (float)afrag[kk][k] + ib[kk][k];
          if (in_relu) f = fmaxf(f, 0.0f);
          afrag[kk][k] = (_Float16)f;
        }
    }
#pragma unroll
    for (int t = 0; t < NT; ++t) {
      f32x4 acc = f32x4{0.f, 0.f, 0.f, 0.f};
#pragma unroll
      for (int kk = 0; kk < 4; ++kk)
        acc = __builtin_amdgcn_mfma_f32_16x16x32_f16(afrag[kk], bfrag[t][kk], acc, 0, 0, 0);
      const int n = t * 16 + col;
      if (n < ncols) {
#pragma unroll
        for (int r = 0; r < 4; ++r) {
          const long pr = p0 + kg * 4 + r;
          if (pr < P) taps[pr * tstride + grp * ncols + n] = acc[r];
        }
      }
    }
  }
}

__device__ __forceinline__ float softplusf_(float x) { return x > 20.0f ? x : log1pf(__expf(x)); }

template <bool PLANAR>
__global__ __launch_bounds__(256) void conv_stencil_kernel(const float* __restrict__ taps, int ncols,
                                                           int tstride, const float* __restrict__ bias,
                                                           int K, int groups, int act_packed, float scale,
                                                           float* __restrict__ out, long P, int H, int W,
                                                           float* __restrict__ out_last = nullptr) {
  const long idx = (long)blockIdx.x * 256 + threadIdx.x;
  if (idx >= P * K * groups) return;
  const int gk = PLANAR ? (int)(idx / P) : (int)(idx % (K * groups));
  const long p = PLANAR ? idx - (long)gk * P : idx / (K * groups);
  const int grp = gk / K, j = gk - grp * K;
  const int xw = (int)(p % W), yh = (int)((p / W) % H);
  float acc = bias ? bias[grp * K + j] : 0.0f;
#pragma unroll
  for (int d = 0; d < 9; ++d) {
    const int dy = d / 3 - 1, dx = d % 3 - 1;
    if ((unsigned)(yh + dy) < (unsigned)H && (unsigned)(xw + dx) < (unsigned)W)
      acc += PLANAR ? taps[(size_t)(grp * ncols + d * K + j) * P + (p + dy * W + dx)]
                    : taps[(p + dy * W + dx) * tstride + grp * ncols + d * K + j];
  }
  const int act = (act_packed >> (4 * grp)) & 15;
  if (act == ACT_RELU) acc = fmaxf(acc, 0.0f);
  else if (act == ACT_SIGMOID) acc = sigmoidf_(acc);
  else if (act == ACT_SOFTPLUS) acc = softplusf_(acc);
  if (out_last && grp == groups - 1) out_last[(size_t)p * K + j] = acc * scale;
  else out[((size_t)grp * P + p) * K + j] = acc * scale;
}

}

using namespace glorie;

extern "C" int glorie_bias_act(const void* x, int x_stride, const float* bias, void* y, int y_stride,
                               long P, int C, int act, void* stream) {
  if (P < 0 || C <= 0 || (C & 7) || (x_stride & 7) || (y_stride & 7)) return GLORIE_EINVAL;
  if (P == 0) return GLORIE_OK;
  if (!x || !y) return GLORIE_EINVAL;
  const long total = P * (C / 8);
  const dim3 grid((unsigned)((total + 255) / 256));
  auto launch = [&](auto kernel) {
    hipLaunchKernelGGL(kernel, grid, dim3(256), 0, (hipStream_t)stream,
                       reinterpret_cast<const _Float16*>(x), x_stride, bias,
                       reinterpret_cast<_Float16*>(y), y_stride, P, C / 8, act);
  };
  switch (C / 8) {
    case 8: launch(bias_act_kernel<8>); break;
    case 16: launch(bias_act_kernel<16>); break;
    case 48: launch(bias_act_kernel<48>); break;
    default: launch(bias_act_kernel<0>); break;
  }
  return check_launch();
}

__global__ __launch_bounds__(128) void glo_from_tiles_kernel(const float* __restrict__ tiles, const float* __restrict__ G,
                                                             const float* __restrict__ Gb, int M,
                                                             float* __restrict__ g, int HW) {
  __shared__ float glo[128];
  const int n = blockIdx.x;
  const int tpm = (HW + 127) >> 7;
  const float* tp = tiles + (size_t)n * tpm * 128 + threadIdx.x;
  float s = 0.0f;
  int t = 0;
  for (; t + 8 <= tpm; t += 8) {
    float v[8];
#pragma unroll
    for (int k = 0; k < 8; ++k) v[k] = tp[(size_t)(t + k) * 128];
#pragma unroll
    for (int k = 0; k < 8; ++k) s += v[k];
  }
  for (; t < tpm; ++t) s += tp[(size_t)t * 128];
  const int o = blockIdx.y * 128 + threadIdx.x;
  const int oc = min(o, M - 1);
  float gv[16];
#pragma unroll
  for (int k = 0; k < 16; ++k) gv[k] = G[(size_t)k * M + oc];
  glo[threadIdx.x] = s / (float)HW;
  __syncthreads();
  if (o >= M) return;
  float acc0 = Gb[o], acc1 = 0.0f, acc2 = 0.0f, acc3 = 0.0f;
#pragma unroll
  for (int c0 = 0; c0 < 128; c0 += 16) {
    float nx[16];
    if (c0 + 16 < 128) {
#pragma unroll
      for (int k = 0; k < 16; ++k) nx[k] = G[(size_t)(c0 + 16 + k) * M + o];
    }
#pragma unroll
    for (int k = 0; k < 16; k += 4) {
      acc0 = fmaf(glo[c0 + k], gv[k], acc0);
      acc1 = fmaf(glo[c0 + k + 1], gv[k + 1], acc1);
      acc2 = fmaf(glo[c0 + k + 2], gv[k + 2], acc2);
      acc3 = fmaf(glo[c0 + k + 3], gv[k + 3], acc3);
    }
    if (c0 + 16 < 128) {
#pragma unroll
      for (int k = 0; k < 16; ++k) gv[k] = nx[k];
    }
  }
  g[(size_t)n * M + o] = (acc0 + acc1) + (acc2 + acc3);
}

extern "C" int glorie_gru_glo_from_tiles(const float* tiles, const float* G, const float* Gb, int M, float* g, int N,
                                         int HW, void* stream) {
  if (N < 0 || HW < 1 || M <= 0) return GLORIE_EINVAL;
  if (N == 0) return GLORIE_OK;
  if (!tiles || !G || !Gb || !g) return GLORIE_EINVAL;
  hipLaunchKernelGGL(glo_from_tiles_kernel, dim3(N, (M + 127) / 128), dim3(128), 0, (hipStream_t)stream, tiles, G, Gb, M,
                     g, HW);
  return check_launch();
// ... 43 lines not shown
}

__global__ __launch_bounds__(256) void update_bookkeeping_kernel(
    const float* __restrict__ coords1, const float* __restrict__ delta, float* __restrict__ target, long n_target,
    const float* __restrict__ eta, const int64_t* __restrict__ frames, float* __restrict__ damping_table,
    float* __restrict__ damping_ba, long n_eta, int HW, float ep, int64_t* __restrict__ age, int n_edges) {
#pragma clang fp contract(off)
  const long i = (long)blockIdx.x * 256 + threadIdx.x;
  if (i < n_target) target[i] = coords1[i] + delta[i];
  if (i < n_eta) {
    const float e = eta[i];
    const long g = i / HW;
    damping_table[(size_t)frames[g] * HW + (i - g * HW)] = e;
    const float m = e * 0.2f;
    damping_ba[i] = m + ep;
  }
  if (age && i < n_edges) age[i] += 1;
}

extern "C" int glorie_update_bookkeeping(const float* coords1, const float* delta, float* target, long n_target,
                                         const float* eta, const int64_t* frames, float* damping_table,
                                         float* damping_ba, int G, int HW, float ep, int64_t* age, int n_edges,
                                         void* stream) {
  if (n_target < 0 || G < 0 || HW <= 0 || n_edges < 0) return GLORIE_EINVAL;
  const long n_eta = (long)G * HW;
  const long n = n_target > n_eta ? n_target : n_eta;
  if (n == 0) return GLORIE_OK;
  if ((n_target && (!coords1 || !delta || !target)) || (n_eta && (!eta || !frames || !damping_table || !damping_ba)))
    return GLORIE_EINVAL;
  hipLaunchKernelGGL(update_bookkeeping_kernel, dim3((unsigned)((n + 255) / 256)), dim3(256), 0, (hipStream_t)stream,
                     coords1, delta, target, n_target, eta, frames, damping_table, damping_ba, n_eta, HW, ep, age, n_edges);
  return check_launch();
}

extern "C" int glorie_segment_mean(const void* x, int x_stride, const float* bias, int relu,
                                   const int64_t* ix, int N, void* out, int o_stride, int G, int HW,
                                   void* stream) {
  if (N < 0 || G < 0 || HW <= 0 || (x_stride & 7) || (o_stride & 7)) return GLORIE_EINVAL;
  if (G == 0) return GLORIE_OK;
  if (!out || (N > 0 && (!x || !ix))) return GLORIE_EINVAL;
  hipLaunchKernelGGL(segment_mean_kernel, dim3((HW * 16 + 255) / 256, G), dim3(256), 0,
                     (hipStream_t)stream, reinterpret_cast<const _Float16*>(x), x_stride, bias, relu,
                     ix, N, reinterpret_cast<_Float16*>(out), o_stride, HW);
  return check_launch();
}

extern "C" int glorie_conv3x3_small(const void* x, int x_stride, const float* in_bias, int in_relu,
                                    const void* w_packed, const float* out_bias, int groups, int K,
                                    int act_packed, float scale, float* taps, float* out, int N, int H,
                                    int W, void* stream) {
  if (N < 0 || H <= 0 || W <= 0 || groups < 1 || groups > 4 || K < 1 || K > 3 || (x_stride & 7))
    return GLORIE_EINVAL;
  if (N == 0) return GLORIE_OK;
  if (!x || !w_packed || !taps || !out) return GLORIE_EINVAL;
  const long P = (long)N * H * W;
  const int ncols = 9 * K, tstride = ncols * groups;
  const long ntiles = (P + 15) / 16;
  const unsigned gx = (unsigned)min((ntiles + 3) / 4, (long)2048);
  hipStream_t st = (hipStream_t)stream;
  if (ncols <= 16)
    hipLaunchKernelGGL(conv_taps_kernel<1>, dim3(gx, groups), dim3(256), 0, st,
                       reinterpret_cast<const _Float16*>(x), x_stride, in_bias, in_relu,
                       reinterpret_cast<const f16x8*>(w_packed), taps, ncols, tstride, P);
  else
    hipLaunchKernelGGL(conv_taps_kernel<2>, dim3(gx, groups), dim3(256), 0, st,
                       reinterpret_cast<const _Float16*>(x), x_stride, in_bias, in_relu,
                       reinterpret_cast<const f16x8*>(w_packed), taps, ncols, tstride, P);
  const long total = P * K * groups;
  hipLaunchKernelGGL(conv_stencil_kernel<false>, dim3((unsigned)((total + 255) / 256)), dim3(256), 0, st, taps,
                     ncols, tstride, out_bias, K, groups, act_packed, scale, out, P, H, W);
  return check_launch();
}

extern "C" int glorie_conv_stencil(const float* taps, const float* out_bias, int groups, int K, int act_packed,
                                   float scale, float* out, float* out_last, int N, int H, int W, void* stream) {
  if (N < 0 || H <= 0 || W <= 0 || groups < 1 || groups > 4 || K < 1 || K > 3) return GLORIE_EINVAL;
  if (N == 0) return GLORIE_OK;
  if (!taps || !out) return GLORIE_EINVAL;
  const long P = (long)N * H * W, total = P * K * groups;
  hipLaunchKernelGGL(conv_stencil_kernel<true>, dim3((unsigned)((total + 255) / 256)), dim3(256), 0, (hipStream_t)stream,
                     taps, 9 * K, 9 * K * groups, out_bias, K, groups, act_packed, scale, out, P, H, W, out_last);
  return check_launch();
}
```

glorie_slam_amd/depth_video.py:

```python
import os

import numpy as np
import torch
from torch.multiprocessing import Value

from . import droid_backends
from . import _lib as L


class DepthVideo:
    def __init__(self, cfg, printer=None):
        self.cfg = cfg
        self.output = f"{cfg['data']['output']}/{cfg['setting']}/{cfg['scene']}" if 'data' in cfg else ''
        ht = self.ht = cfg['cam']['H_out']
        wd = self.wd = cfg['cam']['W_out']
        self.counter = Value('i', 0)
        buffer = cfg['tracking']['buffer']
        self.BA_type = cfg['tracking']['backend']['BA_type']
        self.mono_thres = cfg['tracking']['mono_thres']
        self.device = cfg['device']
        self.down_scale = s = 8
        dev = self.device
        f32 = dict(device=dev, dtype=torch.float)

# ... 201 lines not shown
            n = self.counter.value
            s = self.disps[:n].mean()
            self.disps[:n] /= s
            self.poses[:n, :3] *= s
            self.set_dirty(0, n)

    def reproject(self, ii, jj, motion=None):
        ii, jj = DepthVideo.format_indicies(ii, jj, self.device)
        coords, valid = droid_backends.reproject(self.poses, self.disps, self.intrinsics, ii, jj, motion=motion)
        return coords[None], valid[None]

    def distance(self, ii=None, jj=None, beta=0.3, bidirectional=True):
        return_matrix = False
        if ii is None:
            return_matrix = True
            N = self.counter.value
            ii, jj = torch.meshgrid(torch.arange(N), torch.arange(N), indexing="ij")
        ii, jj = DepthVideo.format_indicies(ii, jj, self.device)
        intr0 = self.intrinsics[0].contiguous()
        if bidirectional:
            poses = self.poses[:self.counter.value].clone()
            d1 = droid_backends.frame_distance(poses, self.disps, intr0, ii, jj, beta)
            d2 = droid_backends.frame_distance(poses, self.disps, intr0, jj, ii, beta)
            d = .5 * (d1 + d2)
        else:
            d = droid_backends.frame_distance(self.poses, self.disps, intr0, ii, jj, beta)
        return d.reshape(N, N) if return_matrix else d

    def deferred_flag_init(self):
        if getattr(self, "_flag_host", None) is None:
            self._flag_host = torch.zeros(1, dtype=torch.int32).pin_memory()
            self._flag_np = self._flag_host.numpy()
            self._flag_count = torch.zeros(2, dtype=torch.int32, device=self.device)
            self._flag_expected = 0

    def publish_target(self):
        self.deferred_flag_init()
        return self._flag_count, self._flag_host.data_ptr()

    def publish_any_on(self, any_on):
        from . import _lib as L
        self.deferred_flag_init()
        L.check(L.load().glorie_publish_flag(L.ptr(any_on), L.ptr(self._flag_count), self._flag_host.data_ptr(),
                                             L.stream_ptr()), "glorie_publish_flag")

    def await_any_on(self, timeout=0.05):
        import time
        self._flag_expected += 1
        want = self._flag_expected
        t_end = time.perf_counter() + timeout
        while True:
            word = int(self._flag_np[0])
            if (word >> 1) == want:
                return word & 1
            if time.perf_counter() > t_end:
                torch.cuda.current_stream().synchronize()
                word = int(self._flag_np[0])
                if (word >> 1) > want:
                    import warnings
                    warnings.warn("deferred depth_scale decision: launch count %d, expected %d - resynchronised"
                                  % (word >> 1, want))
                    self._flag_expected = word >> 1
                elif (word >> 1) < want:
                    self._flag_expected = word >> 1
                    raise RuntimeError("deferred depth_scale decision: the replay published nothing (launch count %d, "
                                       "expected %d)" % (word >> 1, want))
                return word & 1

    def dspo(self, target, weight, eta, ii, jj, t0=1, t1=None, itrs=2, lm=1e-4, ep=0.1,
             motion_only=False, opt_type="pose_depth", gate=None):
        with self.get_lock():
            if t1 is None:
                t1 = max(ii.max().item(), jj.max().item()) + 1
            h, w = self.ht // self.down_scale, self.wd // self.down_scale
            if opt_type == "pose_depth":
                target = target.reshape(-1, h, w, 2).contiguous()
                weight = weight.reshape(-1, h, w, 2).contiguous()
                if self.is_sharded():
                    from . import dist as gdist
                    gdist.ba_sharded(self.ctx(), self.poses, self.disps, self.intrinsics[0].contiguous(),
                                     target, weight, eta.contiguous(), ii, jj, t0, t1, itrs, lm, ep,
                                     motion_only, False, group=self.shard["group"], targets_hwc=True,
                                     force_collective=self.shard["force"])
                else:
                    droid_backends.ba(self.poses, self.disps, self.intrinsics[0].contiguous(), None,
                                      target, weight, eta, ii, jj, t0, t1, itrs, lm, ep, motion_only,
                                      False, ctx=self.ctx(), want_updates=False, targets_hwc=True, gate=gate)
                self.disps.clamp_(min=1e-5)
                return True
            elif opt_type == "depth_scale":
                from . import dspo as _dspo
                return _dspo.depth_scale_stage(self, target, weight, eta, ii, jj, itrs, lm, ep)
            raise NotImplementedError(opt_type)

    def ba(self, target, weight, eta, ii, jj, t0=1, t1=None, iters=2, lm=1e-4, ep=0.1,
           motion_only=False, opt_type="pose_depth", eta_fallback=None):
        if self.BA_type == "DSPO":
            ok = self.dspo(target, weight, eta, ii, jj, t0, t1, iters, lm, ep, motion_only, opt_type)
            if isinstance(ok, torch.Tensor):
                if self._fb_hits is None:
                    if torch.cuda.is_current_stream_capturing():
                        raise RuntimeError("the fallback counter must exist before a capture (run one eager step first)")
                    self._fb_hits = torch.zeros(1, dtype=torch.int32, device=ok.device)
                self.dspo(target, weight, eta if eta_fallback is None else eta_fallback, ii, jj, t0, t1, iters, lm, ep,
                          motion_only, "pose_depth", gate=(ok, self._fb_hits))
                return
            if not ok:
                self.count_host_fallback()
                self.dspo(target, weight, eta if eta_fallback is None else eta_fallback, ii, jj, t0, t1, iters, lm, ep,
                          motion_only, "pose_depth")
        elif self.BA_type == "DBA":
            self.dspo(target, weight, eta, ii, jj, t0, t1, iters, lm, ep, motion_only, "pose_depth")
        else:
            raise NotImplementedError(self.BA_type)

    @torch.no_grad()
    def update_valid_depth_mask(self, up=True, fused=True):
        if up:
            with self.get_lock():
                dirty_index, = torch.where(self.dirty.clone())
            if len(dirty_index) == 0:
                return
        else:
            dirty_index = torch.arange(self.counter.value, device=self.device)
        src = self.fresh_disps_up() if up else self.disps
        intr = (self.intrinsics[0].detach() * (self.down_scale if up else 1.0)).contiguous()
        mv = self.cfg['tracking']['multiview_filter']
        if fused and src.is_cuda:
            masks = droid_backends.valid_depth_mask(self.poses, src, intr, dirty_index.contiguous(), mv['thresh'],
                                                    mv['visible_num'])
        else:
            disps = torch.index_select(src, 0, dirty_index)
            depths = 1.0 / disps
            thresh = (mv['thresh'] * depths.mean(dim=[1, 2])).contiguous()
            count = droid_backends.depth_filter(self.poses, src, intr, dirty_index.contiguous(), thresh)
            depths[~(count >= mv['visible_num'])] = torch.nan
            med = depths.view(depths.shape[0], -1).nanmedian(dim=1).values
            masks = depths < 3 * med[:, None, None]
        if up:
            self.valid_depth_mask[dirty_index] = masks
            self.dirty[dirty_index] = False
        else:
            self.valid_depth_mask_small[dirty_index] = masks

    def get_depth_scale_and_shift(self, index, mono_depth, est_depth, weights):
        from .common import align_scale_and_shift
        scale, shift, _ = align_scale_and_shift(mono_depth, est_depth, weights)
        self.depth_scale[index] = scale
        self.depth_shift[index] = shift
        return [self.depth_scale[index], self.depth_shift[index]]

    def get_pose(self, index, device):
        p = self.poses[index].detach().to(device=device, dtype=torch.float32)
        t, (qx, qy, qz, qw) = p[:3], p[3:]
        R = torch.stack([torch.stack([1 - 2 * (qy * qy + qz * qz), 2 * (qx * qy - qz * qw), 2 * (qx * qz + qy * qw)]),
                         torch.stack([2 * (qx * qy + qz * qw), 1 - 2 * (qx * qx + qz * qz), 2 * (qy * qz - qx * qw)]),
                         torch.stack([2 * (qx * qz - qy * qw), 2 * (qy * qz + qx * qw), 1 - 2 * (qx * qx + qy * qy)])])
        c2w = torch.eye(4, dtype=torch.float32, device=p.device)
        c2w[:3, :3] = R.t()
        c2w[:3, 3] = -(R.t() @ t)
        return c2w

    def get_depth_and_pose(self, index, device):
        with self.get_lock():
            est_depth = 1.0 / self.fresh_disps_up()[index].clone().to(device)
            depth_mask = self.valid_depth_mask[index].clone().to(device)
            c2w = self.get_pose(index, device)
        return est_depth, depth_mask, c2w

    def save_video(self, path):
        poses, depths, stamps, masks = [], [], [], []
# ... 14 lines not shown
```

glorie_slam_amd/droid_backends.py:

```python
import ctypes
import os

import torch

from . import _lib as L


_CHECK_STATUS = os.environ.get("GLORIE_CHECK_STATUS", "0") not in ("", "0")


def _i64(t, name):
    if t.dtype != torch.int64:
        raise RuntimeError(f"{name} must be int64 (the reference kernels read `long`)")
    return t


def corr_index_forward(volume, coords, radius):
    L.need_cuda(volume, coords)
    L.need_contiguous(volume=volume, coords=coords)
    if coords.dtype != torch.float32:
        raise RuntimeError("coords must be float32")
    N, h1, w1, h2, w2 = volume.shape
    rd = 2 * radius + 1
    out = torch.empty((N, rd, rd, h1, w1), dtype=volume.dtype, device=volume.device)
# ... 248 lines not shown
    L.need_cuda(coords1, coords0, target)
    L.need_contiguous(coords1=coords1, coords0=coords0, target=target)
    h, w = coords0.shape[-3], coords0.shape[-2]
    n = coords1.numel() // (h * w * 2)
    if target.numel() != coords1.numel() or coords0.numel() != h * w * 2:
        raise RuntimeError("motion: shape mismatch")
    out = torch.empty((n, h, w, 4), dtype=torch.float32, device=coords1.device)
    L.check(L.load().glorie_motion(L.ptr(coords1), L.ptr(coords0), L.ptr(target), L.ptr(out), n, h, w,
                                   float(limit), L.stream_ptr()), "glorie_motion")
    return out


def motion_padded(coords1, coords0, target, padded, limit=64.0):
    L.need_cuda(coords1, coords0, target, padded.buf)
    L.need_contiguous(coords1=coords1, coords0=coords0, target=target)
    h, w = coords0.shape[-3], coords0.shape[-2]
    n = coords1.numel() // (h * w * 2)
    if target.numel() != coords1.numel() or coords0.numel() != h * w * 2 or not padded.fits(n, h, w, coords1.device):
        raise RuntimeError("motion_padded: shape mismatch")
    L.check(L.load().glorie_motion_padded(L.ptr(coords1), L.ptr(coords0), L.ptr(target), L.ptr(padded.buf), n, h, w,
                                          float(limit), L.stream_ptr()), "glorie_motion_padded")
    return padded


def valid_depth_mask(poses, disps, intrinsics, ix, mv_thresh, visible_num):
    L.need_cuda(poses, disps, intrinsics, ix)
    L.need_contiguous(poses=poses, disps=disps, intrinsics=intrinsics, ix=ix)
    _i64(ix, "ix")
    B, h, w = disps.shape
    num = ix.shape[0]
    mask = torch.empty((num, h, w), dtype=torch.bool, device=disps.device)
    scratch = torch.empty(num * h * w * 4 + num * 1044 + 64, dtype=torch.uint8, device=disps.device)
    L.check(L.load().glorie_valid_depth_mask(L.ptr(poses), L.ptr(disps), L.ptr(intrinsics), L.ptr(ix), B, num, h, w,
                                             float(mv_thresh), int(visible_num), L.ptr(mask), L.ptr(scratch),
                                             L.stream_ptr()), "glorie_valid_depth_mask")
    return mask


def dspo_prepare(poses, disps, intrinsics, mono_disps, n, mv_thresh, visible_num, mono_thres, ii, jj,
                 valid_mask, depth_scale, depth_shift, publish=None):
    L.need_cuda(poses, disps, intrinsics, mono_disps, ii, jj, valid_mask, depth_scale, depth_shift)
    L.need_contiguous(poses=poses, disps=disps, intrinsics=intrinsics, mono_disps=mono_disps, ii=ii, jj=jj,
                      valid_mask=valid_mask, depth_scale=depth_scale, depth_shift=depth_shift)
    _i64(ii, "ii"), _i64(jj, "jj")
    if valid_mask.dtype != torch.bool or valid_mask.shape != disps.shape:
        raise RuntimeError("valid_mask must be a bool tensor of the shape of disps")
    B, h, w = disps.shape
    N = ii.shape[0]
    dev = disps.device
    edge_on = torch.empty(N, dtype=torch.uint8, device=dev)
    any_on = torch.empty(1, dtype=torch.int32, device=dev)
    scratch = torch.empty(n * h * w * 4 + n * 32 + 64, dtype=torch.uint8, device=dev)
    L.check(L.load().glorie_dspo_prepare(L.ptr(poses), L.ptr(disps), L.ptr(intrinsics), L.ptr(mono_disps), B,
                                         int(n), h, w, float(mv_thresh), int(visible_num),
                                         float(mono_thres or 0.0), L.ptr(ii), L.ptr(jj), N, L.ptr(valid_mask),
                                         L.ptr(depth_scale), L.ptr(depth_shift), L.ptr(edge_on), L.ptr(any_on),
                                         L.ptr(scratch), L.ptr(publish[0]) if publish else None,
                                         publish[1] if publish else None, L.stream_ptr()), "glorie_dspo_prepare")
    return edge_on, any_on


def cvx_upsample(disps, ix, mask, disps_up, softmax_f32=False):
    L.need_cuda(disps, ix, mask, disps_up)
    _i64(ix, "ix")
    M = ix.shape[0]
    h, w = disps.shape[1:]
    if mask.numel() != M * 576 * h * w:
        raise RuntimeError(f"mask has {mask.numel()} elements, expected {M}*576*{h}*{w}")
    if mask.dim() == 4 and mask.dtype == torch.float16 and not mask.is_contiguous() \
            and mask.is_contiguous(memory_format=torch.channels_last):
        L.need_contiguous(disps=disps, ix=ix, disps_up=disps_up)
        L.check(L.load().glorie_cvx_upsample_nhwc(L.ptr(disps), L.ptr(ix), L.ptr(mask), 576, L.ptr(disps_up),
                                                  M, h, w, int(bool(softmax_f32)), L.stream_ptr()),
                "glorie_cvx_upsample_nhwc")
        return disps_up
    L.need_contiguous(disps=disps, ix=ix, mask=mask, disps_up=disps_up)
    L.check(L.load().glorie_cvx_upsample(L.ptr(disps), L.ptr(ix), L.ptr(mask), L.ptr(disps_up), M, h,
                                         w, L.dtype_code(mask), int(bool(softmax_f32)),
                                         L.stream_ptr()), "glorie_cvx_upsample")
    return disps_up


def ba(poses, disps, intrinsics, disps_sens, targets, weights, eta, ii, jj, t0, t1,
       iterations, lm, ep, motion_only, depth_only=False, ctx=None, want_updates=True, targets_hwc=False, gate=None):
    L.need_cuda(poses, disps, intrinsics, targets, weights, ii, jj)
    L.need_contiguous(targets=targets, weights=weights, poses=poses, disps=disps,
                      intrinsics=intrinsics, disps_sens=disps_sens, ii=ii, jj=jj)
    _i64(ii, "ii"), _i64(jj, "jj")
    if eta is not None and not eta.is_contiguous():
        eta = eta.contiguous()
    B, h, w = disps.shape
    N = ii.shape[0]
    P = t1 - t0
    M = eta.shape[0] if eta is not None else 0
    if motion_only and eta is None:
        M = 0
    ctx = ctx or L.default_context()
    dx = torch.zeros((max(P, 0), 6), dtype=torch.float32, device=poses.device) if want_updates else None
    dz = torch.zeros((M, h * w), dtype=torch.float32, device=poses.device) if want_updates else None
    if disps_sens is not None and (disps_sens.shape != disps.shape):
        raise RuntimeError("disps_sens must have the shape of disps")
    if motion_only and M == 0:
        M = int(torch.unique(torch.cat([torch.arange(t0, t1, device=ii.device), ii])).numel())
    lib = L.load()
    if gate is not None:
        L.check(lib.glorie_ba_set_gate(ctx.handle, L.ptr(gate[0]), L.ptr(gate[1])), "glorie_ba_set_gate")
    try:
        L.check(lib.glorie_ba(ctx.handle, L.ptr(poses), L.ptr(disps), L.ptr(intrinsics),
                              L.ptr(disps_sens), L.ptr(targets), L.ptr(weights), L.ptr(eta),
                              L.ptr(ii), L.ptr(jj), B, N, M, h, w, int(t0), int(t1),
                              int(iterations), float(lm), float(ep),
                              int(bool(motion_only)) | (L.BA_TARGETS_HWC if targets_hwc else 0),
                              int(bool(depth_only)), L.ptr(dx),
                              L.ptr(dz) if (dz is not None and dz.numel()) else None,
                              L.stream_ptr()), "glorie_ba")
    finally:
        if gate is not None:
            lib.glorie_ba_set_gate(ctx.handle, None, None)
    if _CHECK_STATUS:
        st = ctx.ba_status()
        if st[0] & 1:
            raise RuntimeError(f"ba: eta has {M} rows but unique(cat(arange(t0, t1), ii)) has {st[1]} frames")
        if st[0] & 4:
            import warnings
            warnings.warn(f"ba: {st[2]} Gauss-Newton iteration(s) had a non positive definite system (zero update)")
    return [dx, dz] if want_updates else []
```

glorie_slam_amd/droid_net.py:

```python
import os

import numpy as np
import torch
import torch.nn as nn
import torch.nn.functional as F

from . import droid_backends


def _conv(cin, cout, k):
    return nn.Conv2d(cin, cout, kernel_size=(k, k), padding=(k // 2, k // 2))


def cvx_upsample(data, mask):
    batch, ht, wd, dim = data.shape
    mask = mask.reshape(batch, 576, ht, wd)
    ix = torch.arange(batch, device=data.device)
    out = torch.empty(batch, 8 * ht, 8 * wd, dim, dtype=torch.float32, device=data.device)
    for c in range(dim):
        up = torch.empty(batch, 8 * ht, 8 * wd, dtype=torch.float32, device=data.device)
        droid_backends.cvx_upsample(data[..., c].float().contiguous(), ix, mask.contiguous(), up, softmax_f32=True)
        out[..., c] = up
    return out

# ... 231 lines not shown
        W["ce1_p"] = OtfCorrBlock.pack_encoder(m.corr_encoder[0].weight)
        W["ce1_cl"] = U.pack_corr_encoder(m.corr_encoder[0].weight)
        W["ce1_dm"] = U.pack_corr_encoder_dm(m.corr_encoder[0].weight)
        W["ce2"], W["ce2_b"] = U.pack_conv_igemm(m.corr_encoder[2].weight, pair=True), f32(m.corr_encoder[2].bias)
        W["fe1"], W["fe1_b"] = U.pack_flow_conv7(m.flow_encoder[0].weight), f32(m.flow_encoder[0].bias)
        W["fe2"], W["fe2_b"] = U.pack_conv_igemm(m.flow_encoder[2].weight, pair=True), f32(m.flow_encoder[2].bias)
        W["zr"] = U.pack_conv_igemm(torch.cat([g.convz.weight, g.convr.weight], 0), pair=True)
        W["q"] = U.pack_conv_igemm(g.convq.weight, pair=True)
        dyn = lambda wt: torch.cat([wt[:, 0:128], wt[:, 256:448]], 1)
        W["zr_dyn"] = U.pack_conv_igemm(torch.cat([dyn(g.convz.weight), dyn(g.convr.weight)], 0), pair=True)
        W["q_dyn"] = U.pack_conv_igemm(dyn(g.convq.weight), pair=True)
        W["pre"] = U.pack_conv_igemm(torch.cat([g.convz.weight[:, 128:256], g.convr.weight[:, 128:256],
                                                g.convq.weight[:, 128:256]], 0), pair=True)
        W["w"], W["w_b"] = U.pack_conv_igemm(g.w.weight), f32(g.w.bias)
        W["G"] = f32(torch.cat([g.convz_glo.weight.view(128, 128), g.convr_glo.weight.view(128, 128),
                                g.convq_glo.weight.view(128, 128)], 0).t())
        W["G_b"] = f32(torch.cat([g.convz_glo.bias + g.convz.bias, g.convr_glo.bias + g.convr.bias,
                                  g.convq_glo.bias + g.convq.bias]))
        W["h1"] = U.pack_conv_igemm(torch.cat([m.delta[0].weight, m.weight[0].weight, m.agg.conv1.weight], 0))
        W["h1_b"] = f32(torch.cat([m.delta[0].bias, m.weight[0].bias, m.agg.conv1.bias]))
        W["h2"] = U.pack_conv3x3_small([m.delta[2].weight, m.weight[2].weight])
        W["h2_taps"] = U.pack_head_taps([m.delta[2].weight, m.weight[2].weight])
        W["h2_b"] = f32(torch.cat([m.delta[2].bias, m.weight[2].bias]))
        W["a2"], W["a2_b"] = U.pack_conv_igemm(m.agg.conv2.weight, pair=True), f32(m.agg.conv2.bias)
        W["eta"], W["eta_b"] = U.pack_conv3x3_small([m.agg.eta[0].weight]), f32(m.agg.eta[0].bias)
        W["up"], W["up_b"] = U.pack_conv_igemm(m.agg.upmask[0].weight), f32(m.agg.upmask[0].bias)
        W["up_cvx"], W["up_cvx_b"] = U.pack_upmask_conv(m.agg.upmask[0].weight, m.agg.upmask[0].bias)
        self.W = W
        self._ver = ver
        self._inp_key = None

    @torch.no_grad()
    def precompute_context(self):
        from . import update_ops as U
        hx = self._hx
        n, _, ht, wd = hx.shape
        if self._pre is None or self._pre.shape[0] != n or self._pre.shape[2:] != hx.shape[2:] \
                or self._pre.device != hx.device:
            self._pre = torch.empty((n, 384, ht, wd), dtype=torch.float16, device=hx.device,
                                    memory_format=torch.channels_last)
        U.conv_igemm(hx[:, 0:128], None, self.W["pre"], 9, 384, self._pre)
        return self._pre

    @staticmethod
    def _cl(t):
        b, n, c, h, w = t.shape
        return t.reshape(b * n, c, h, w).half().contiguous(memory_format=torch.channels_last)

    def _side_streams(self, dev):
        if self._streams is None or self._streams[0].device != dev:
            self._streams = (torch.cuda.Stream(dev), torch.cuda.Stream(dev))
        return self._streams

    @torch.no_grad()
    def precompute_shared_context(self, context):
        from . import update_ops as U
        table, frames, index = context
        g = int(frames.shape[0])
        ht, wd = table.shape[-2:]
        x = table[frames].half().contiguous(memory_format=torch.channels_last)
        if self._pre_kf is None or self._pre_kf.shape[0] < g or tuple(self._pre_kf.shape[2:]) != (ht, wd) \
                or self._pre_kf.device != x.device:
            self._pre_kf = torch.empty((max(g, 8), 384, ht, wd), dtype=torch.float16, device=x.device,
                                       memory_format=torch.channels_last)
        U.conv_igemm(x, None, self.W["pre"], 9, 384, self._pre_kf[:g])
        n = int(index.shape[0])
        if self._pre_map is None or self._pre_map.shape[0] < n or self._pre_map.device != x.device:
            self._pre_map = torch.zeros(max(n, 64), dtype=torch.int32, device=x.device)
        self._pre_map[:n].copy_(index)
        return self._pre_kf[:g], self._pre_map[:n]

    def _shared_context(self, context):
        table, frames, index = context
        key = (table.data_ptr(), table._version, frames.data_ptr(), frames._version, index.data_ptr(), index._version,
               int(frames.shape[0]), int(index.shape[0]), self._ver)
        if self._ctx_key != key:
            self.precompute_shared_context(context)
            self._ctx_key = key
            self._ctx_refs = (table, frames, index)
        return self._pre_kf[:int(frames.shape[0])], self._pre_map[:int(index.shape[0])]

    @torch.no_grad()
    def __call__(self, net, inp, corr, flow=None, ii=None, jj=None, groups=None, context=None, lazy_up=False,
                 weight_out=None):
        from . import update_ops as U
        self._sync()
        W = self.W
        batch, num, _, ht, wd = net.shape
        n, hw = batch * num, ht * wd
        dev = net.device
        cl_map = lambda c: torch.empty((n, c, ht, wd), dtype=torch.float16, device=dev,
                                       memory_format=torch.channels_last)
        if self._hx is None or tuple(self._hx.shape) != (n, 320, ht, wd) or self._hx.device != dev:
            self._hx = cl_map(320)
            self._inp_key = None
        hx = self._hx
        net0 = self._cl(net)
        main = torch.cuda.current_stream(dev)
        side = self._side_streams(dev) if self.parallel else ((main, self._side_streams(dev)[1]) if self.glo_stream
                                                              else (main, main))
        for st in side:
            if st is not main:
                st.wait_stream(main)
        with torch.cuda.stream(side[0]):
            if isinstance(flow, U.PaddedFlow):
                pf = flow
            else:
                if flow is None:
                    flow = torch.zeros(batch, num, 4, ht, wd, device=dev)
                fl = flow.reshape(n, 4, ht, wd).permute(0, 2, 3, 1).float().contiguous()
                if self._flow_pad is None or not self._flow_pad.fits(n, ht, wd, dev):
                    self._flow_pad = U.PaddedFlow(n, ht, wd, dev)
                pf = U.flow_pad(fl, self._flow_pad)
            f1 = U.flow_conv7_padded(pf, W["fe1"], W["fe1_b"], cl_map(128))
            U.conv_igemm(f1, None, W["fe2"], 9, 64, hx[:, 256:320], terms=W["fe2_b"], act=U.ACT_RELU)
        shared = context is not None and self.hoist_inp
        with torch.cuda.stream(side[1]):
            if shared:
                pre_kf, pre_map = self._shared_context(context)
            elif self._inp_key is None or self._inp_key[0] is not inp or self._inp_key[1] != inp._version:
                U.bias_act(self._cl(inp), None, U.ACT_NONE, out=hx[:, 0:128])
                self._inp_key = (inp, inp._version)
                if self.hoist_inp:
                    self.precompute_context()
            if self.fuse_glo:
                g = U.gru_glo_terms_fused(net0, W["w"], W["w_b"], W["G"], W["G_b"])
            else:
                wn = U.conv_igemm(net0, None, W["w"], 1, 128, cl_map(128))
                g = U.gru_glo_terms(wn, W["w_b"], net0, W["G"], W["G_b"])
        if self.glo_stream and not self.parallel:
            main.wait_stream(side[1])
        if hasattr(corr, "encode_into"):
            c1 = cl_map(128)
            evc = self.corr_events
            if evc is not None:
                c0e, c1e = torch.cuda.Event(enable_timing=True), torch.cuda.Event(enable_timing=True)
                c0e.record()
            corr.encode_into(W, c1)
            if evc is not None:
                c1e.record()
                evc.append((c0e, c1e))
        else:
            if callable(corr):
                corr = corr()
            if corr.dim() == 4 and corr.shape[1] == 256 and corr.dtype == torch.float16:
                c1 = U.conv_igemm(corr, None, W["ce1_cl"], 1, 128, cl_map(128), terms=W["ce1_b"], act=U.ACT_RELU)
            else:
                c1 = torch.matmul(corr.reshape(n, -1, hw).half().transpose(1, 2), W["ce1_t"])
                c1 = c1.view(n, ht, wd, 128).permute(0, 3, 1, 2)
                U.bias_act(c1, W["ce1_b"], U.ACT_RELU)
        U.conv_igemm(c1, None, W["ce2"], 9, 128, hx[:, 128:256], terms=W["ce2_b"], act=U.ACT_RELU)
        for st in side:
            if st is not main:
                main.wait_stream(st)
        z, rnet = cl_map(128), cl_map(128)
        aliased = net0.data_ptr() == net.data_ptr() and net.dtype == torch.float16
        new = net0 if (self.inplace and aliased) else cl_map(128)
        if self.hoist_inp:
            dynx = hx[:, 128:320]
            pre, pmap = (pre_kf, pre_map) if shared else (self._pre, None)
            ev = self.gate_events
            if ev is not None:
                e0, e1 = torch.cuda.Event(enable_timing=True), torch.cuda.Event(enable_timing=True)
                e0.record()
            U.conv_igemm(net0, dynx, W["zr_dyn"], 9, 256, z, epilogue=U.EPI_GRU_ZR, terms=g[:, 0:256], net=net0,
                         out2=rnet, pre=pre[:, 0:256], pre_map=pmap)
            if ev is not None:
                e1.record()
                ev.append((e0, e1))
            evq = self.q_events
            if evq is not None:
                q0, q1 = torch.cuda.Event(enable_timing=True), torch.cuda.Event(enable_timing=True)
                q0.record()
            U.conv_igemm(rnet, dynx, W["q_dyn"], 9, 128, new, epilogue=U.EPI_GRU_Q, terms=g[:, 256:384], net=net0,
                         z=z, pre=pre[:, 256:384], pre_map=pmap)
            if evq is not None:
                q1.record()
                evq.append((q0, q1))
        else:
            U.conv_igemm(net0, hx, W["zr"], 9, 256, z, epilogue=U.EPI_GRU_ZR, terms=g[:, 0:256], net=net0, out2=rnet)
            U.conv_igemm(rnet, hx, W["q"], 9, 128, new, epilogue=U.EPI_GRU_Q, terms=g[:, 256:384], net=net0, z=z)
        net_out = new.view(batch, num, 128, ht, wd)
        if self.fuse_heads:
            agg_in = cl_map(128)
            evh = self.heads_events
            if evh is not None:
                h0, h1e = torch.cuda.Event(enable_timing=True), torch.cuda.Event(enable_timing=True)
                h0.record()
            rows = U.conv_igemm_heads(new, W["h1"], 9, 384, W["h1_b"], W["h2_taps"], 2, out=agg_in)
            if evh is not None:
                h1e.record()
                evh.append((h0, h1e))
            wo = weight_out if (weight_out is not None and weight_out.is_cuda and weight_out.dtype == torch.float32
                                and weight_out.is_contiguous() and weight_out.numel() == n * ht * wd * 2) else None
            dw = U.conv_stencil(rows, W["h2_b"], n, ht, wd, 2, 2, (U.ACT_NONE, U.ACT_SIGMOID), out_last=wo)
        else:
            h1 = U.conv_igemm(new, None, W["h1"], 9, 384, cl_map(384), terms=W["h1_b"], act=U.ACT_RELU)
            dw = U.conv3x3_small(h1, W["h2"], W["h2_b"], 2, (U.ACT_NONE, U.ACT_SIGMOID))
            agg_in = h1[:, 256:384]
        delta = dw[0].view(batch, num, ht, wd, 2)
        weight = dw[1].view(batch, num, ht, wd, 2) if (not self.fuse_heads or wo is None) else \
            weight_out.view(batch, num, ht, wd, 2)
        if ii is None:
            return net_out, delta, weight
        if groups is None:
            uniq, ix = torch.unique(ii.to(dev), sorted=True, return_inverse=True)
            ngroups = uniq.shape[0]
        else:
            ix, ngroups = groups
        agg = U.segment_mean(agg_in, ix.contiguous(), ngroups)
        a2 = torch.empty((ngroups, 128, ht, wd), dtype=torch.float16, device=dev,
                         memory_format=torch.channels_last)
        U.conv_igemm(agg, None, W["a2"], 9, 128, a2, terms=W["a2_b"], act=U.ACT_RELU)
        eta = U.conv3x3_small(a2, W["eta"], W["eta_b"], 1, (U.ACT_SOFTPLUS,), scale=0.01)
        if lazy_up:
            return net_out, delta, weight, eta.view(batch, ngroups, ht, wd), U.LazyUpmask(a2, W["up_cvx"], W["up_cvx_b"])
        up = torch.empty((ngroups, 576, ht, wd), dtype=torch.float16, device=dev,
                         memory_format=torch.channels_last)
        U.conv_igemm(a2, None, W["up"], 1, 576, up, terms=W["up_b"])
        return net_out, delta, weight, eta.view(batch, ngroups, ht, wd), up.view(batch, ngroups, 576, ht, wd)


class CorrBlock:

    def __init__(self, fmap1, fmap2, num_levels=4, radius=3, tiled=None):
        self.num_levels = num_levels
        self.radius = radius
        corr = CorrBlock.corr(fmap1, fmap2)
        batch, num, h1, w1, h2, w2 = corr.shape
        self.dims = (h1, w1, h2, w2)
        if tiled is None:
            tiled = corr.is_cuda and radius == 3 and (h1 * w1) % 8 == 0 and corr.dtype == torch.float16
        self.tiled = bool(tiled)
        corr = corr.reshape(batch * num * h1 * w1, 1, h2, w2)
        self.corr_pyramid = []
        for i in range(num_levels):
            if self.tiled:
                self.corr_pyramid.append(droid_backends.tile_corr_level(corr[:, 0]))
            else:
                self.corr_pyramid.append(corr.view(batch * num, h1, w1, h2 // 2 ** i, w2 // 2 ** i))
            if i + 1 < num_levels:
                corr = F.avg_pool2d(corr, kernel_size=2, stride=2)

    @staticmethod
    def corr(fmap1, fmap2):
        batch, num, dim, ht, wd = fmap1.shape
        a = fmap1.reshape(batch * num, dim, ht * wd) / 4.0
        b = fmap2.reshape(batch * num, dim, ht * wd) / 4.0
        return torch.matmul(a.transpose(1, 2), b).view(batch, num, ht, wd, ht, wd)

    def __call__(self, coords, channels_last=False):
        batch, num, ht, wd, _ = coords.shape
        if channels_last and self.tiled and self.num_levels == 4 and self.radius == 3:
            return droid_backends.corr_lookup_tiled_cl(self.corr_pyramid, coords.reshape(batch * num, ht, wd, 2).float()
                                                       .contiguous(), self.dims[2], self.dims[3], interleaved=True)
        c = coords.permute(0, 1, 4, 2, 3).contiguous().view(batch * num, 2, ht, wd).float()
        if self.tiled:
            out = droid_backends.corr_lookup_pyramid_tiled(self.corr_pyramid, c, self.dims[2], self.dims[3])
        else:
            pyr = [v if v.is_contiguous() else v.contiguous() for v in self.corr_pyramid]
            out = droid_backends.corr_lookup_pyramid(pyr, c, self.radius)
        return out.view(batch, num, -1, ht, wd)

    @staticmethod
    def _with_slack(rows):
        total = sum(r.shape[0] for r in rows)
        store = torch.zeros((total + 2, rows[0].shape[1]), dtype=rows[0].dtype, device=rows[0].device)
        at = 1
        for r in rows:
            store[at:at + r.shape[0]] = r
            at += r.shape[0]
        return store[1:total + 1]

    def cat(self, other):
        if self.tiled != other.tiled:
            raise RuntimeError("cannot concatenate tiled and row-major correlation pyramids")
        if self.tiled:
            self.corr_pyramid = [self._with_slack([a, b]) for a, b in zip(self.corr_pyramid, other.corr_pyramid)]
        else:
            self.corr_pyramid = [torch.cat([a, b], 0) for a, b in zip(self.corr_pyramid, other.corr_pyramid)]
        return self

    def __getitem__(self, index):
        if self.tiled:
            hw = self.dims[0] * self.dims[1]
            self.corr_pyramid = [self._with_slack([v.view(-1, hw, v.shape[1])[index].reshape(-1, v.shape[1])])
                                 for v in self.corr_pyramid]
        else:
            self.corr_pyramid = [v[index] for v in self.corr_pyramid]
        return self


class CorrArena:

    def __init__(self, h, w, device, num_levels=4, radius=3, capacity=16, layout=None):
        assert radius == 3
# ... 239 lines not shown
```

glorie_slam_amd/dspo.py:

```python
import torch

from . import _lib as L
from .common import align_scale_and_shift


def scale_shift_step(video, target, weight, eta, ii, jj, edge_on, itrs, lm, ep, alpha=0.01):
    h, w = video.ht // video.down_scale, video.wd // video.down_scale
    target = target.reshape(-1, h, w, 2).contiguous().float()
    weight = weight.reshape(-1, h, w, 2).contiguous().float()
    eta = eta.reshape(-1, h, w).contiguous().float()
    N, M, B = ii.shape[0], eta.shape[0], video.disps.shape[0]
    vm = video.valid_depth_mask_small.contiguous().view(torch.uint8)
    eo = edge_on.to(torch.uint8).contiguous() if edge_on is not None else None
    L.check(L.load().glorie_dspo_scale_shift(
        video.ctx().handle, L.ptr(video.poses), L.ptr(video.disps), L.ptr(video.intrinsics),
        L.ptr(video.mono_disps), L.ptr(video.depth_scale), L.ptr(video.depth_shift), L.ptr(vm),
        L.ptr(target), L.ptr(weight), L.ptr(eta), L.ptr(ii.contiguous()), L.ptr(jj.contiguous()),
        L.ptr(eo), B, N, M, h, w, int(itrs), float(lm), float(ep), float(alpha), None,
        L.stream_ptr()), "glorie_dspo_scale_shift")


def _prepare_torch(video, n, ii, jj):
    video.update_valid_depth_mask(up=False)
    mono_d, est_d, valid_d = video.mono_disps[:n], video.disps[:n], video.valid_depth_mask_small[:n]
    scale_t, shift_t, error_t = align_scale_and_shift(mono_d, est_d, valid_d)
    video.depth_scale[:n] = scale_t
    video.depth_shift[:n] = shift_t
    if not video.mono_thres:
        return None, None
    avg = est_d.mean(dim=[1, 2])
    bad = (error_t / avg > video.mono_thres) | error_t.isnan() | (scale_t < 0) | \
          (valid_d.sum(dim=[1, 2]) < valid_d.shape[1] * valid_d.shape[2] * 0.5)
    bad_full = torch.zeros(video.disps.shape[0], dtype=torch.bool, device=bad.device)
    bad_full[:n] = bad
    edge_on = ~(bad_full[ii] | bad_full[jj])
    return edge_on, edge_on.any().to(torch.int32).reshape(1)


def depth_scale_stage(video, target, weight, eta, ii, jj, itrs, lm, ep, fused=True):
    n = video.counter.value
    self_publish = False
    if fused and video.disps.is_cuda and n > 0:
        from . import droid_backends
        mv = video.cfg['tracking']['multiview_filter']
        shard_ = getattr(video, "shard", None)
        self_publish = bool(video.mono_thres and torch.cuda.is_current_stream_capturing()
                            and not video.is_sharded())
        edge_on, any_on = droid_backends.dspo_prepare(
            video.poses, video.disps, video.intrinsics[0].contiguous(), video.mono_disps, n, mv['thresh'],
            mv['visible_num'], video.mono_thres, ii.contiguous(), jj.contiguous(), video.valid_depth_mask_small,
            video.depth_scale, video.depth_shift, publish=video.publish_target() if self_publish else None)
        if not video.mono_thres:
            edge_on = None
    else:
        edge_on, any_on = _prepare_torch(video, n, ii, jj)
    if edge_on is not None:
        if video.is_sharded():
            from . import dist as gdist
            gdist.allreduce_flag_any(any_on, video.shard["group"], ctx=video._ctx, force=video.shard["force"])
        if any_on.is_cuda and not video.is_sharded() and not torch.cuda.is_current_stream_capturing():
            if n <= 0:
                return False
            scale_shift_step(video, target, weight, eta, ii, jj, edge_on, itrs, lm, ep, alpha=0.01)
            video.disps.clamp_(min=1e-5)
            return any_on
        if any_on.is_cuda and torch.cuda.is_current_stream_capturing():
            if not self_publish:
                video.publish_any_on(any_on)
            video.deferred_fallback = True
        elif not bool(any_on.item()):
            return False
    if n <= 0:
        return False
    scale_shift_step(video, target, weight, eta, ii, jj, edge_on, itrs, lm, ep, alpha=0.01)
    video.disps.clamp_(min=1e-5)
    return True
```

glorie_slam_amd/factor_graph.py:

```python
import numpy as np
import os

import torch

from . import droid_backends
from .droid_net import ArenaLookup, CorrArena, CorrBlock, AltCorrBlock, FusedUpdate, FusedLookup, OtfCorrBlock


def coords_grid(ht, wd, device):
    y, x = torch.meshgrid(torch.arange(ht, device=device).float(),
                          torch.arange(wd, device=device).float(), indexing="ij")
    return torch.stack([x, y], dim=-1)


class FactorGraph:
    def __init__(self, video, update_op, device="cuda:0", corr_impl="volume", max_factors=-1,
                 use_graphs=False, capture_after=1):
        self.video = video
        self.update_op = update_op
        self.device = device
        self.max_factors = max_factors
        self.corr_impl = corr_impl
        self.ht = ht = video.ht // video.down_scale
        self.wd = wd = video.wd // video.down_scale
# ... 257 lines not shown
                                motion_only, "pose_depth")
                self.video.upsample(uniq, upmask)
                if sharded:
                    self.video.sync_owned_state()
                    self.video.mark_upsampled()

    def _capture(self, key, args):
        st = self._graphs.get("static")
        if st is None:
            st = (self.net.clone(memory_format=torch.preserve_format), self.target.clone(), self.weight.clone())
            self._graphs["static"] = st
        s_net, s_target, s_weight = st
        for dst, src in ((s_net, self.net), (s_target, self.target), (s_weight, self.weight)):
            if src is not dst:
                dst.copy_(src)
        keep = (self.net, self.target, self.weight)
        self.video.deferred_flag_init()
        torch.cuda.synchronize()
        graph = torch.cuda.CUDAGraph()
        self.net, self.target, self.weight = s_net, s_target, s_weight
        self.video.deferred_fallback = False
        try:
            dev = self.net.device
            cap = getattr(self, "_capture_stream", None)
            if cap is None:
                cap = self._capture_stream = torch.cuda.Stream(dev)
                self._graph_pool = torch.cuda.graph_pool_handle()
                self._pool_keeper = torch.cuda.CUDAGraph()
                with torch.cuda.stream(cap):
                    self._pool_keeper.capture_begin(pool=self._graph_pool, capture_error_mode="thread_local")
                    self._pool_keeper_buf = torch.zeros(1, device=dev)
                    self._pool_keeper.capture_end()
            if torch.cuda.memory_reserved(dev) - torch.cuda.memory_allocated(dev) > getattr(self, "capture_trim_bytes", 32 << 30):
                torch.cuda.empty_cache()
            with torch.cuda.stream(cap):
                graph.capture_begin(pool=self._graph_pool, capture_error_mode="thread_local")
                try:
                    self._update_eager(*args)
                    if self.net.data_ptr() != s_net.data_ptr():
                        s_net.copy_(self.net)
                    ba_args = tuple(s_target if a is self.target else (s_weight if a is self.weight else a)
                                    for a in self._ba_args)
                    if self.target is not s_target:
                        s_target.copy_(self.target)
                    s_weight.copy_(self.weight)
                finally:
                    graph.capture_end()
        finally:
            self.net, self.target, self.weight = keep
        ent = (graph, s_net, s_target, s_weight, ba_args, bool(self.video.deferred_fallback),
               getattr(self, "_eta_fb", None), self._arena_generations())
        self._graphs[key] = ent
        return ent

    @torch.no_grad()
    def _update_eager(self, t0=None, t1=None, itrs=2, use_inactive=False, EP=1e-7, motion_only=False,
                      opt_type="pose_depth", run_ba=True):
        if run_ba and not torch.cuda.is_current_stream_capturing():
            self.stats["eager"] += 1
        if self.fast_update is not None and self.poses_on_device() and self.target.is_contiguous() \
                and self.target.dtype == torch.float32:
            pf = self._padded_flow(int(self.ii.shape[0]), self.target.device)
            coords1, mask = self.video.reproject(self.ii, self.jj, motion=(self.target, pf))
            motn = pf
        else:
            coords1, mask = self.video.reproject(self.ii, self.jj)
            motn = self._motion(coords1, padded=self.fast_update is not None)
        if self.corr_impl == "otf":
            blk = self._otf_block()
            rig = self._otf_rig
            ck = ("otf_idx", rig)
            if ck not in self._graphs:
                self._graphs[ck] = ((rig * self.ii).contiguous(), (rig * self.jj + (self.ii == self.jj).long()).contiguous())
            oi, oj = self._graphs[ck]
            lookup = FusedLookup(blk, coords1, oi, oj) if (self.fast_update is not None and blk.num_levels == 4) \
                else (lambda: blk(coords1, oi, oj))
        elif self.fast_update is not None and isinstance(self.corr, CorrArena) and self.corr.layout == "dm":
            lookup = ArenaLookup(self.corr, coords1)
        elif self.fast_update is not None and isinstance(self.corr, (CorrArena, CorrBlock)):
            lookup = lambda: self.corr(coords1, channels_last=True)
        else:
            lookup = lambda: self.corr(coords1)
        uniq = self._unique_ii()
        if self.fast_update is not None:
            ix, _ = self._groups()
            self.net, delta, weight, damping, upmask = \
                self.fast_update(self.net, self.inp, lookup, motn, self.ii, self.jj, self._groups(),
                                 context=(self.video.inps, uniq, ix) if self.share_context else None,
                                 lazy_up=True, weight_out=self.weight)
        else:
            corr = lookup()
            with torch.autocast("cuda", enabled=True):
                self.net, delta, weight, damping, upmask = \
                    self.update_op(self.net, self.inp, corr, motn, self.ii, self.jj)
        if t0 is None or t1 is None:
            t0, t1 = self._window(t0, t1, use_inactive)
        sharded = self.video.is_sharded()
        fused_book = (self.fast_update is not None and not use_inactive and not sharded and coords1.is_cuda
                      and self.target.shape == coords1.shape and self.target.dtype == torch.float32
                      and self.target.is_contiguous() and coords1.is_contiguous() and coords1.dtype == torch.float32
                      and delta.dtype == torch.float32 and delta.is_contiguous() and delta.shape == coords1.shape
                      and damping.dtype == torch.float32 and damping.is_contiguous()
                      and self.damping.dtype == torch.float32 and self.damping.is_contiguous()
                      and damping.numel() == uniq.shape[0] * self.ht * self.wd and self.age.is_contiguous())
        damping_ba = None
        if fused_book:
            from . import _lib as L
            damping_ba = torch.empty((uniq.shape[0], self.ht, self.wd), dtype=torch.float32, device=coords1.device)
            L.check(L.load().glorie_update_bookkeeping(
                L.ptr(coords1), L.ptr(delta), L.ptr(self.target), coords1.numel(), L.ptr(damping), L.ptr(uniq),
                L.ptr(self.damping), L.ptr(damping_ba), int(uniq.shape[0]), self.ht * self.wd, float(EP), L.ptr(self.age),
                int(self.age.shape[0]), L.stream_ptr()), "glorie_update_bookkeeping")
            self._age_done = True
        elif self.target.shape == coords1.shape and self.target.dtype == torch.float32 and self.target.is_contiguous():
            torch.add(coords1, delta.to(dtype=torch.float), out=self.target)
        else:
            self.target = coords1 + delta.to(dtype=torch.float)
        self.weight = weight.to(dtype=torch.float)
        if not fused_book:
            self.damping[uniq] = damping.to(self.damping.dtype)
        if use_inactive:
            ck = ("inac", t0)
            c = self._graphs.get(ck)
            if c is None:
                m = (self.ii_inac >= t0 - 3) & (self.jj_inac >= t0 - 3)
                ii_c = torch.cat([self.ii_inac[m], self.ii], 0)
                jj_c = torch.cat([self.jj_inac[m], self.jj], 0)
                tgt = torch.cat([self.target_inac[:, m], self.target], 1)
                wgt = torch.cat([self.weight_inac[:, m], self.weight], 1)
                c = (ii_c, jj_c, torch.unique(ii_c), tgt, wgt, tgt.shape[1] - self.target.shape[1])
                self._graphs[ck] = c
            ii, jj, uq, target, weight, n_inac = c
            target[:, n_inac:] = self.target
            weight[:, n_inac:] = self.weight
        else:
            ii, jj, target, weight, uq = self.ii, self.jj, self.target, self.weight, uniq
        if sharded and opt_type == "pose_depth":
            assert t1 is not None, "sharded BA needs an explicit (global) t1"
            ck = ("uq", self._topo, t0, t1)
            if ck not in self._graphs:
                self._graphs[ck] = torch.unique(torch.cat([torch.arange(t0, t1, device=ii.device), ii]))
            uq = self._graphs[ck]
        if uq is uniq and damping_ba is not None:
            damping = damping_ba
        elif uq is uniq:
            damping = damping.reshape(-1, self.ht, self.wd).to(self.damping.dtype).mul(0.2).add_(EP)
        else:
            damping = .2 * self.damping[uq].contiguous() + EP
        if opt_type == "pose_depth" and not motion_only and not sharded:
            ck = ("slots", t0, t1, bool(use_inactive))
            if ck not in self._graphs:
                self._graphs[ck] = int(np.unique(np.concatenate([np.arange(t0, t1), self._host(ii)])).size)
            if damping.shape[0] != self._graphs[ck]:
                raise RuntimeError(f"FactorGraph.update: eta has {damping.shape[0]} frames, the BA window "
                                   f"[{t0}, {t1}) + the source frames of the edges span {self._graphs[ck]}")
        self._ba_args = (target, weight, damping, ii, jj, uniq, upmask, t0, t1)
        self._eta_fb = None
        if sharded and opt_type == "depth_scale":
            assert t1 is not None, "sharded BA needs an explicit (global) t1"
            ck = ("uq", self._topo, t0, t1)
            if ck not in self._graphs:
                self._graphs[ck] = torch.unique(torch.cat([torch.arange(t0, t1, device=ii.device), ii]))
            self._eta_fb = .2 * self.damping[self._graphs[ck]].contiguous() + EP
        if run_ba:
            self._update_finish(itrs, motion_only, opt_type)

    def _update_finish(self, itrs, motion_only, opt_type):
        target, weight, damping, ii, jj, uniq, upmask, t0, t1 = self._ba_args
        self.video.ba(target, weight, damping, ii, jj, t0, t1, iters=itrs, lm=1e-4, ep=0.1,
                      motion_only=motion_only, opt_type=opt_type, eta_fallback=getattr(self, "_eta_fb", None))
        self.video.upsample(uniq, upmask)
        if self.video.is_sharded():
            self.video.sync_owned_state()
            self.video.mark_upsampled()
        if getattr(self, "_age_done", False):
            self._age_done = False
        else:
            self.age += 1

    @torch.no_grad()
    def update_lowmem(self, t0=None, t1=None, itrs=2, use_inactive=False, EP=1e-7, steps=8,
                      enable_wq=True):
        num, rig, ch, ht, wd = self.video.fmaps.shape
        if getattr(self, "lowmem_corr", "otf") == "otf" and str(self.device).startswith("cuda"):
            corr_op = self._otf_block()
        else:
            corr_op = AltCorrBlock(self.video.fmaps.view(1, num * rig, ch, ht, wd))
        hjj = self._host(self.jj)
        hii = self._host(self.ii)
# ... 153 lines not shown
```

glorie_slam_amd/update_ops.py:

```python
import torch

from . import _lib as L

ACT_NONE, ACT_RELU, ACT_SIGMOID, ACT_SOFTPLUS = 0, 1, 2, 3


def _rows(t, name):
    if t.dtype != torch.float16 or t.dim() != 4:
        raise RuntimeError(f"{name}: expected a 4-D float16 map, got {t.dtype} {tuple(t.shape)}")
    n, c, h, w = t.shape
    sn, sc, sh, sw = t.stride()
    if c > 1 and sc != 1:
        raise RuntimeError(f"{name}: not channels-last (channel stride {sc})")
    if (w > 1 and sh != w * sw) or (h * w > 1 and n > 1 and sn != h * w * sw) or sw < c:
        raise RuntimeError(f"{name}: rows are not uniformly strided {tuple(t.stride())}")
    if sw % 8 or t.data_ptr() % 16:
        raise RuntimeError(f"{name}: rows must be 16-byte aligned")
    return sw


def bias_act(x, bias, act, out=None):
    L.need_cuda(x)
    out = x if out is None else out
    xs, ys = _rows(x, "x"), _rows(out, "out")
# ... 177 lines not shown
        ts = 0
    else:
        ts = _terms(terms, nout, "terms")
        if terms.shape[0] != n:
            raise RuntimeError("conv_igemm: one row of gate terms per map")
    opt = lambda t, name: (L.ptr(t), _rows(t, name) if t is not None else 0)
    (pa, sa), (pb, sb) = opt(xa, "xa"), opt(xb, "xb")
    (pn, sn), (pz, sz), (po2, so2) = opt(net, "net"), opt(z, "z"), opt(out2, "out2")
    pp, sp = opt(pre, "pre")
    if pre is not None and (epilogue == EPI_BIAS_ACT or (pre_map is None and pre.shape[0] != n) or pre.shape[1] != nout
                            or tuple(pre.shape[2:]) != (h, w)):
        raise RuntimeError("conv_igemm: pre needs a gate epilogue and the shape [N,nout,h,w]")
    if pre_map is not None and (pre is None or pre_map.dtype != torch.int32 or pre_map.numel() != n or
                                not pre_map.is_contiguous() or pre_map.device != ref.device):
        raise RuntimeError("conv_igemm: pre_map must be a contiguous int32 [N] on the device, next to pre")
    if out.shape[1] != (128 if (epilogue & 0xff) != EPI_BIAS_ACT else nout) or out.shape[0] != n:
        raise RuntimeError("conv_igemm: bad output shape")
    if pair is None:
        pair = getattr(w_packed, "_glorie_pair", None)
        if pair is None:
            raise RuntimeError("conv_igemm: w_packed carries no row-layout flag (a copy of a pack_conv_igemm result loses "
                               "it): pack again or pass pair=True/False")
    if pair:
        epilogue |= EPI_PAIR16
    epilogue |= CONV_POLICY[policy] << 12
    L.check(L.load().glorie_conv_igemm(pa, sa, ca, pb, sb, cb, L.ptr(w_packed), taps, nout, epilogue,
                                       L.ptr(terms), ts, act, pn, sn, pz, sz, L.ptr(out), _rows(out, "out"),
                                       po2, so2, pp, sp, L.ptr(pre_map), n, h, w, L.stream_ptr()), "glorie_conv_igemm")
    return out


def pack_head_taps(weights):
    K = weights[0].shape[0]
    ncols = 9 * K
    packs = []
    for wgt in weights:
        if tuple(wgt.shape) != (K, 128, 3, 3):
            raise RuntimeError("pack_head_taps: expected [K,128,3,3] weights")
        rows = torch.zeros(32, 128, dtype=torch.float32, device=wgt.device)
        rows[:ncols] = wgt.detach().float().reshape(K, 128, 9).permute(2, 0, 1).reshape(ncols, 128)
        r = rows.view(2, 16, 2, 2, 2, 4, 4)
        packs.append(r.permute(2, 3, 0, 5, 1, 4, 6).reshape(2, 2, 2, 64, 8))
    return torch.stack(packs).half().contiguous()


def conv_igemm_heads(x, w_packed, taps, nout, bias, tap_w, K, out=None):
    L.need_cuda(x, w_packed, tap_w)
    n, c, h, w = x.shape
    groups = tap_w.shape[0]
    if w_packed.dtype != torch.float16 or w_packed.numel() != taps * nout * c + 64 or nout % 128:
        raise RuntimeError("conv_igemm_heads: packed weights do not match (taps, nout, channels)")
    if tap_w.dtype != torch.float16 or tuple(tap_w.shape[1:]) != (2, 2, 2, 64, 8) or not tap_w.is_contiguous():
        raise RuntimeError("conv_igemm_heads: tap_w must come from pack_head_taps")
    if bias.dtype != torch.float32 or bias.numel() != nout or not bias.is_contiguous():
        raise RuntimeError("conv_igemm_heads: bias must be contiguous float32 [nout]")
    rest = nout - 128 * groups
    if rest < 0 or (rest > 0 and (out is None or out.shape[0] != n or out.shape[1] != rest)):
        raise RuntimeError("conv_igemm_heads: `out` must hold the nout - 128*groups trailing channels")
    rows = torch.empty((groups * 9 * K, n * h * w), dtype=torch.float32, device=x.device)
    L.check(L.load().glorie_conv_igemm_heads(L.ptr(x), _rows(x, "x"), c, L.ptr(w_packed), taps, nout, L.ptr(bias),
                                             L.ptr(tap_w), groups, K, L.ptr(rows), L.ptr(out) if rest else None,
                                             _rows(out, "out") if rest else 0, n, h, w, L.stream_ptr()),
            "glorie_conv_igemm_heads")
    return rows


def conv_stencil(rows, out_bias, n, h, w, groups, K, acts, scale=1.0, out_last=None):
    L.need_cuda(rows)
    if rows.dtype != torch.float32 or tuple(rows.shape) != (groups * 9 * K, n * h * w) or not rows.is_contiguous() \
            or len(acts) != groups:
        raise RuntimeError("conv_stencil: bad tap planes")
    out = torch.empty((groups, n, h, w, K), dtype=torch.float32, device=rows.device)
    packed = 0
    for gidx, a in enumerate(acts):
        packed |= int(a) << (4 * gidx)
    if out_last is not None and (out_last.dtype != torch.float32 or not out_last.is_contiguous() or not out_last.is_cuda
                                 or out_last.numel() != n * h * w * K):
        raise RuntimeError("conv_stencil: out_last must be a contiguous float32 CUDA tensor of n*h*w*K elements")
    L.check(L.load().glorie_conv_stencil(L.ptr(rows), L.ptr(out_bias), groups, K, packed, float(scale), L.ptr(out),
                                         L.ptr(out_last), n, h, w, L.stream_ptr()), "glorie_conv_stencil")
    return out


def pack_flow_conv7(weight):
    if tuple(weight.shape) != (128, 4, 7, 7):
        raise RuntimeError("pack_flow_conv7: expected [128,4,7,7]")
    w = torch.zeros(128, 7, 8, 4, dtype=torch.float16, device=weight.device)
    w[:, :, :7] = weight.detach().permute(0, 2, 3, 1).half()
    return w.reshape(128, 224).contiguous()


def pack_upmask_conv(weight, bias):
    if weight.shape[0] != 576 or tuple(weight.shape[2:]) != (1, 1):
        raise RuntimeError("pack_upmask_conv: expected a [576, C, 1, 1] weight")
    C = weight.shape[1]
    w = weight.detach().reshape(9, 8, 8, C)
    wp = torch.zeros(8, 8, 16, C, dtype=w.dtype, device=w.device)
    wp[:, :, :9] = w.permute(1, 2, 0, 3)
    bp = torch.zeros(8, 8, 16, dtype=torch.float32, device=w.device)
    bp[:, :, :9] = bias.detach().float().reshape(9, 8, 8).permute(1, 2, 0)
    return pack_conv_igemm(wp.reshape(1024, C, 1, 1)), bp.reshape(1024).contiguous()


class LazyUpmask:

    def __init__(self, x, w_packed, bias):
        self.x, self.w_packed, self.bias = x, w_packed, bias

    def evaluate(self):
        m, c, h, w = self.x.shape
        wide = torch.empty((m, 1024, h, w), dtype=torch.float16, device=self.x.device, memory_format=torch.channels_last)
        conv_igemm(self.x, None, self.w_packed, 1, 1024, wide, terms=self.bias)
        return wide.view(m, 8, 8, 16, h, w)[:, :, :, :9].permute(0, 3, 1, 2, 4, 5).reshape(m, 576, h, w)


def conv_upsample(up, disps, ix, disps_up, softmax_f32=False):
    L.need_cuda(up.x, up.w_packed, up.bias, disps, ix, disps_up)
    m, c, h, w = up.x.shape
    if ix.dtype != torch.int64 or ix.numel() != m or not ix.is_contiguous():
        raise RuntimeError("conv_upsample: ix must be a contiguous int64 [M]")
    if tuple(disps.shape[1:]) != (h, w) or tuple(disps_up.shape[1:]) != (8 * h, 8 * w) or disps.dtype != torch.float32 \
            or disps_up.dtype != torch.float32 or not disps.is_contiguous() or not disps_up.is_contiguous():
        raise RuntimeError("conv_upsample: disps [B,h,w] / disps_up [B,8h,8w] float32 contiguous expected")
    if up.w_packed.numel() != 1024 * c + 64 or up.bias.numel() != 1024:
        raise RuntimeError("conv_upsample: weights must come from pack_upmask_conv")
    L.check(L.load().glorie_conv_upsample(L.ptr(up.x), _rows(up.x, "x"), c, L.ptr(up.w_packed), L.ptr(up.bias),
                                          L.ptr(disps), L.ptr(ix), L.ptr(disps_up), int(bool(softmax_f32)), m, h, w,
                                          L.stream_ptr()), "glorie_conv_upsample")
    return disps_up


class PaddedFlow:

    def __init__(self, n, h, w, device):
        self.n, self.h, self.w = n, h, w
        self.buf = torch.zeros((n, h + 6, w + 8, 4), dtype=torch.float16, device=device)

    def fits(self, n, h, w, device):
        return (self.n, self.h, self.w) == (n, h, w) and self.buf.device == torch.device(device)

    def interior(self):
        return self.buf[:, 3:3 + self.h, 3:3 + self.w]


def flow_pad(flow, padded):
    L.need_cuda(flow, padded.buf)
    n, h, w, c = flow.shape
    if c != 4 or flow.dtype != torch.float32 or not flow.is_contiguous() or not padded.fits(n, h, w, flow.device):
        raise RuntimeError("flow_pad: flow must be contiguous float32 [N,h,w,4] matching the padded map")
    L.check(L.load().glorie_flow_pad(L.ptr(flow), L.ptr(padded.buf), n, h, w, L.stream_ptr()), "glorie_flow_pad")
    return padded


def flow_conv7_padded(padded, w_packed, bias, out):
    L.need_cuda(padded.buf, w_packed, bias, out)
    if out.shape[1] != 128 or out.shape[0] != padded.n or tuple(out.shape[2:]) != (padded.h, padded.w):
        raise RuntimeError("flow_conv7_padded: bad output shape")
    L.check(L.load().glorie_flow_conv7_padded(L.ptr(padded.buf), L.ptr(w_packed), L.ptr(bias), L.ptr(out),
                                              _rows(out, "out"), padded.n, padded.h, padded.w, L.stream_ptr()),
            "glorie_flow_conv7_padded")
    return out


def flow_conv7(flow, w_packed, bias, out):
    L.need_cuda(flow, w_packed, bias, out)
    n, h, w, c = flow.shape
# ... 6 lines not shown
```

include/glorie_hip.h:

```cpp
#ifndef GLORIE_HIP_H
#define GLORIE_HIP_H

#include <stdint.h>
#include <stddef.h>

#ifdef __cplusplus
extern "C" {
#endif

typedef enum glorie_status {
  GLORIE_OK = 0,
  GLORIE_EINVAL = -1,
  GLORIE_EHIP = -2,
  GLORIE_ENOMEM = -3,
  GLORIE_EUNSUPPORTED = -4
} glorie_status;

typedef enum glorie_dtype { GLORIE_F16 = 0, GLORIE_F32 = 1 } glorie_dtype;

const char* glorie_version(void);
int glorie_last_hip_error(void);

typedef struct glorie_ctx glorie_ctx;

int glorie_ctx_create(glorie_ctx** out, size_t scratch_bytes);
int glorie_ctx_destroy(glorie_ctx* ctx);
int glorie_ctx_reserve(glorie_ctx* ctx, size_t scratch_bytes);
unsigned long long glorie_ctx_generation(const glorie_ctx* ctx);


int glorie_corr_index_fwd(const void* volume, const float* coords, void* out,
                          int N, int h1, int w1, int h2, int w2, int radius,
                          int dtype, void* stream);

int glorie_corr_lookup_pyramid(const void* const* volumes, int num_levels,
                               const float* coords, void* out,
                               int N, int h1, int w1, int h2, int w2, int radius,
                               int dtype, void* stream);

int glorie_corr_lookup_pyramid_tiled(const void* const* volumes, int num_levels, const float* coords,
                                     void* out, int N, int h1, int w1, int h2, int w2, void* stream);

int glorie_corr_build(const void* fmaps_cl, const int64_t* ii, const int64_t* jj, const int* slots,
                      void* const* levels, int num_levels, int n_new, int h, int w, int C, void* stream);

int glorie_corr_lookup_arena(const void* const* levels, int num_levels, const int* slots, const float* coords,
                             void* out, int N, int h1, int w1, int h2, int w2, void* stream);

int glorie_corr_lookup_tiled_cl(const void* const* levels, int num_levels, const int* slots, const float* coords,
                                int coords_xy, void* out, int N, int h1, int w1, int h2, int w2, void* stream);

long glorie_corr_dm_level_halfs(int h, int w, int level);
int glorie_corr_dm_build(const void* fmaps_cl, const int64_t* ii, const int64_t* jj, const int* slots,
                         void* const* levels, int num_levels, int n_new, int h, int w, int C, void* stream);
int glorie_corr_dm_lookup(const void* const* levels, const int* slots, const float* coords, int coords_xy, int N,
                          int h, int w, void* corr_cl, const void* enc_w, const float* enc_b, void* enc_out,
                          int enc_stride, void* stream);

int glorie_corr_otf(const void* fmap1, const void* const* fmap2_levels, int num_levels,
                    const float* coords, const int64_t* ii, const int64_t* jj, void* out,
                    int N, int h, int w, int C, void* stream);

int glorie_corr_otf_encode(const void* fmap1, const void* const* fmap2_levels, int num_levels,
                           const float* coords, const int64_t* ii, const int64_t* jj, void* corr_out,
                           int N, int h, int w, int C, const void* enc_w, const float* enc_b,
                           void* enc_out, int enc_stride, void* stream);

int glorie_altcorr_fwd(const float* fmap1, const float* fmap2, const float* coords,
                       float* out, int B, int S, int H, int W, int H2, int W2, int C,
                       int radius, void* stream);

int glorie_update_bookkeeping(const float* coords1, const float* delta, float* target, long n_target,
                              const float* eta, const int64_t* frames, float* damping_table, float* damping_ba,
                              int G, int HW, float ep, int64_t* age, int n_edges, void* stream);

int glorie_bias_act(const void* x, int x_stride, const float* bias, void* y, int y_stride,
                    long P, int C, int act, void* stream);
int glorie_gru_glo_terms(const void* wn, int w_stride, const float* bw, const void* net, int n_stride,
                         const float* G, const float* Gb, int M, float* partial, int parts, float* g,
                         int N, int HW, void* stream);
int glorie_gru_glo_from_tiles(const float* tiles, const float* G, const float* Gb, int M, float* g, int N, int HW,
                              void* stream);
int glorie_gru_gate_zr(const void* zr, int zr_stride, const float* g, int g_stride, const void* net,
                       int n_stride, void* z, int z_stride, void* rnet, int r_stride, int N, int HW,
                       void* stream);
int glorie_gru_gate_q(const void* qc, int q_stride, const float* gq, int gq_stride, const void* z,
                      int z_stride, const void* net, int n_stride, void* out, int o_stride, void* out2,
                      int o2_stride, int N, int HW, void* stream);
int glorie_segment_mean(const void* x, int x_stride, const float* bias, int relu, const int64_t* ix,
                        int N, void* out, int o_stride, int G, int HW, void* stream);
int glorie_conv3x3_small(const void* x, int x_stride, const float* in_bias, int in_relu,
                         const void* w_packed, const float* out_bias, int groups, int K,
                         int act_packed, float scale, float* taps, float* out, int N, int H, int W,
                         void* stream);

#define GLORIE_CONV_PAIR16 0x100
int glorie_conv_igemm(const void* xa, int xa_stride, int ca, const void* xb, int xb_stride, int cb,
                      const void* w_packed, int taps, int nout, int epilogue, const float* terms,
                      int terms_stride, int act, const void* net, int net_stride, const void* z,
                      int z_stride, void* out, int out_stride, void* out2, int out2_stride,
                      const void* pre, int pre_stride, const int* pre_map, int N, int H, int W, void* stream);

int glorie_conv_igemm_heads(const void* x, int x_stride, int c, const void* w_packed, int taps, int nout,
                            const float* bias, const void* tap_w, int groups, int K, float* tap_out, void* out,
                            int out_stride, int N, int H, int W, void* stream);
int glorie_conv_upsample(const void* x, int x_stride, int c, const void* w_packed, const float* bias,
                         const float* disps, const int64_t* ix, float* disps_up, int softmax_f32, int M, int H, int W,
                         void* stream);
int glorie_conv_stencil(const float* taps, const float* out_bias, int groups, int K, int act_packed, float scale,
                        float* out, float* out_last, int N, int H, int W, void* stream);

int glorie_flow_conv7(const float* flow, const void* w_packed, const float* bias, void* out,
                      int out_stride, int N, int H, int W, void* stream);

int glorie_flow_pad(const float* flow, void* padded, int N, int H, int W, void* stream);
int glorie_flow_conv7_padded(const void* padded, const void* w_packed, const float* bias, void* out, int out_stride,
                             int N, int H, int W, void* stream);


int glorie_reproject(const float* poses, const float* disps, const float* intrinsics,
                     const int64_t* ii, const int64_t* jj, float* coords, float* valid,
                     int N, int h, int w, void* stream);

int glorie_frame_distance(const float* poses, const float* disps, const float* intrinsics,
                          const int64_t* ii, const int64_t* jj, float* dist,
                          int K, int h, int w, float beta, void* stream);

int glorie_iproj(const float* poses, const float* disps, const float* intrinsics,
                 float* points, int num, int h, int w, void* stream);

int glorie_depth_filter(const float* poses, const float* disps, const float* intrinsics,
                        const int64_t* ix, const float* thresh, float* count,
                        int B, int num, int h, int w, void* stream);

int glorie_cvx_upsample(const float* disps, const int64_t* ix, const void* mask,
                        float* disps_up, int M, int h, int w, int mask_dtype,
                        int softmax_f32, void* stream);
int glorie_motion(const float* coords1, const float* coords0, const float* target, float* out, int N,
                  int h, int w, float limit, void* stream);
int glorie_motion_padded(const float* coords1, const float* coords0, const float* target, void* padded, int N, int h,
                         int w, float limit, void* stream);
int glorie_reproject_motion(const float* poses, const float* disps, const float* intrinsics, const int64_t* ii,
                            const int64_t* jj, float* coords, float* valid, const float* target, void* padded_motion,
                            int N, int h, int w, float limit, void* stream);

int glorie_cvx_upsample_nhwc(const float* disps, const int64_t* ix, const void* mask, int mask_stride,
                             float* disps_up, int M, int h, int w, int softmax_f32, void* stream);


#define GLORIE_BA_TARGETS_HWC 2
int glorie_ba(glorie_ctx* ctx, float* poses, float* disps, const float* intrinsics,
              const float* disps_sens, const float* targets, const float* weights,
              const float* eta, const int64_t* ii, const int64_t* jj,
              int B, int N, int M, int h, int w, int t0, int t1, int iterations,
              float lm, float ep, int motion_only, int depth_only,
              float* dx_out, float* dz_out, void* stream);

int glorie_ba_build_system(glorie_ctx* ctx, const float* poses, const float* disps,
                           const float* intrinsics, const float* disps_sens,
                           const float* targets, const float* weights, const float* eta,
                           const int64_t* ii, const int64_t* jj, int B, int N, int M, int h, int w,
                           int t0, int t1, int motion_only, double* hv_out, void* stream);
int glorie_ba_solve_update(glorie_ctx* ctx, float* poses, float* disps, const int64_t* ii,
                           const int64_t* jj, int B, int N, int M, int h, int w, int t0, int t1,
                           float lm, float ep, int motion_only, int depth_only, const double* hv,
                           float* dx_out, float* dz_out, void* stream);

int glorie_ba_set_gate(glorie_ctx* ctx, const int* run_if_zero, int* hits);

#define GLORIE_COMM_ID_BYTES 128
int glorie_comm_unique_id(void* id_out);
int glorie_comm_init(glorie_ctx* ctx, const void* id, int rank, int world);
int glorie_comm_destroy(glorie_ctx* ctx);
int glorie_comm_world(const glorie_ctx* ctx);
int glorie_allreduce_normal_eq(glorie_ctx* ctx, double* hv, size_t n, void* stream);
int glorie_allgather_rows(glorie_ctx* ctx, const void* send, void* recv, size_t bytes_per_rank, void* stream);

int glorie_ba_pack_system(const double* hv, double* packed, int n6, int unpack, void* stream);

int glorie_dspo_scale_shift(glorie_ctx* ctx, const float* poses, float* disps,
                            const float* intrinsics, const float* mono_disps, float* scales,
                            float* shifts, const uint8_t* valid_mask, const float* target,
                            const float* weight, const float* eta, const int64_t* ii,
                            const int64_t* jj, const uint8_t* edge_on, int B, int N, int M, int h,
                            int w, int iterations, float lm, float ep, float alpha, float* dz_out,
                            void* stream);

int glorie_dspo_prepare(const float* poses, const float* disps, const float* intrinsics,
                        const float* mono_disps, int B, int n, int h, int w, float mv_thresh,
                        int visible_num, float mono_thres, const int64_t* ii, const int64_t* jj, int N,
                        uint8_t* valid_mask, float* scales, float* shifts, uint8_t* edge_on,
                        int* any_on, void* scratch, int* publish_state, int* publish_host_word, void* stream);

int glorie_publish_flag(const int* flag, int* counter, int* host_word, void* stream);

int glorie_valid_depth_mask(const float* poses, const float* disps, const float* intrinsics,
                            const int64_t* ix, int B, int num, int h, int w, float mv_thresh,
                            int visible_num, uint8_t* mask, void* scratch, void* stream);


int glorie_knn_build(glorie_ctx* ctx, const float* points, int np, float cell_size,
                     int max_cells, float* sorted_pos, int* cell_start, void* grid,
                     void* stream);

int glorie_knn_query(const float* sorted_pos, const int* cell_start, const void* grid,
                     const float* queries, int Q, int k, float radius, const float* radius_ptr,
                     float* D, int64_t* I, int* nn, void* stream);

int glorie_knn_query_image(const float* sorted_pos, const int* cell_start, const void* grid,
                           const float* queries, int Q, int k, float radius, const float* radius_ptr,
                           float* D, int64_t* I, int* nn, int samples_per_ray, int image_w, void* stream);

int glorie_knn_query_weights(const float* sorted_pos, const int* cell_start, const void* grid,
                             const float* queries, int Q, float radius, const float* radius_ptr, float* D,
                             int64_t* I, int* nn, int samples_per_ray, int image_w, int min_nn,
                             int expo_weighting, int ball_only, float* weights, uint8_t* has, void* stream);

int glorie_idw_gather(const float* D, const int64_t* I, const int* nn, const float* feats,
                      int Q, int k, int c_dim, float radius, const float* radius_ptr,
                      int min_nn, int expo_weighting, float* c_out, float* w_out,
                      uint8_t* has_out, void* stream);

int glorie_idw_gather2(const float* D, const int64_t* I, const int* nn, const float* feats_a,
                       const float* feats_b, int Q, int k, int c_dim, float radius,
                       const float* radius_ptr, int min_nn, int expo_weighting, float* c_out_a,
                       float* c_out_b, float* w_out, uint8_t* has_out, void* stream);

size_t glorie_decoder_pack_floats(void);
int glorie_render_mlp(const float* packed, const float* pts, const float* views,
                      const float* cloud_pos, const float* col_feats, const float* c_geo,
                      const float* geo_feats, const int64_t* I, const float* weights, const uint8_t* has,
                      int Q, float* c_col_scratch, float* raw, int stage_flags, int* range_flag, void* stream);

int glorie_ray_samples(const float* rays_o, const float* rays_d, const float* depth,
                       const float* radius, const float* t_lin, int R, int S, float near_s, float far_s,
                       float* z_vals, float* pts, float* views, float* radius_s, int* n_zero,
                       void* stream);

int glorie_ray_samples_camera(const float* cam, int image_w, long first_pixel, const float* depth, const float* radius,
                              const float* t_lin, int R, int S, float near_s, float far_s, float* z_vals, float* pts,
                              float* views, float* radius_s, int* n_zero, void* stream);

int glorie_proj_depth(const float* points, const uint8_t* mask, long n, const float* w2c, float fx, float fy,
                      float cx, float cy, int H, int W, float* depth_inf, void* stream);

int glorie_ray_counts(const uint8_t* has, int R, int S, int min_samples, int64_t* counts,
                      uint8_t* valid, void* stream);

int glorie_composite(const float* raw, const float* z_vals, int R, int S, float coef,
                     float* depth, float* var, float* rgb, float* weights, void* stream);

int glorie_ba_status(glorie_ctx* ctx, int* status_out, void* stream);
// ... 91 lines not shown
```

Before: 958.1 BA-update iters/s.

## Fuse disparity floor into BA/DSPO updates, add fused upsample conv and update-finish kernel

Three separate fusions. The final BA/DSPO iteration now applies the disparity clamp inside the update kernel, which drops a separate clamp_ pass over all disparities. A dedicated upsample conv kernel streams weight tiles into LDS and computes the softmax-weighted upsampling for all eight output tiles in one block. A new update_finish kernel combines the head taps, eta conv, target update and damping bookkeeping. Together these cut kernel launches and memory passes, at the cost of more complex code paths with many eligibility checks.

New measurement: 941.5 BA-update iters/s. 0.983x the previous value.

```diff
diff --git a/glorie_slam_amd/_lib.py b/glorie_slam_amd/_lib.py
--- a/glorie_slam_amd/_lib.py
+++ b/glorie_slam_amd/_lib.py
@@ -34,6 +34,7 @@
     "glorie_gru_glo_from_tiles": (_c_int, [_vp, _vp, _vp, _c_int, _vp, _c_int, _c_int, _vp]),
     "glorie_update_bookkeeping": (_c_int, [_vp, _vp, _vp, ctypes.c_long, _vp, _vp, _vp, _vp, _c_int, _c_int, _c_f, _vp, _c_int,
                                            _vp]),
+    "glorie_update_finish": (_c_int, [_vp] * 6 + [_vp, _c_int] + [_vp] * 7 + [_c_f, _vp] + [_c_int] * 5 + [_vp]),
     "glorie_conv_igemm_heads": (_c_int, [_vp, _c_int, _c_int, _vp, _c_int, _c_int, _vp, _vp, _c_int, _c_int, _vp, _vp,
                                          _c_int, _c_int, _c_int, _c_int, _vp]),
     "glorie_conv_upsample": (_c_int, [_vp, _c_int, _c_int, _vp, _vp, _vp, _vp, _vp, _c_int, _c_int, _c_int, _c_int, _vp]),
@@ -102,6 +103,7 @@
     "glorie_counter_add": (_c_int, [_vp, _c_int, _vp]),
     "glorie_ba_status": (_c_int, [_vp, ctypes.POINTER(_c_int), _vp]),
     "glorie_ba_set_gate": (_c_int, [_vp, _vp, _vp]),
+    "glorie_ba_set_disp_floor": (_c_int, [_vp, _c_f]),
     "glorie_pix_warp_workspace": (_sz, [_c_int]),
     "glorie_pix_warp_fwd": (_c_int, [_vp] * 4 + [_c_int, _vp, _vp, _c_int, _vp, _vp, _c_int, _c_int, _c_int] + [_c_f] * 4
                             + [_vp, _c_int] + [_vp] * 5 + [_vp]),
diff --git a/glorie_slam_amd/csrc/ba.hip b/glorie_slam_amd/csrc/ba.hip
--- a/glorie_slam_amd/csrc/ba.hip
+++ b/glorie_slam_amd/csrc/ba.hip
@@ -1092,7 +1092,8 @@
 __global__ __launch_bounds__(kBaThreads) void ba_update_kernel(
     BaWork wk, float* __restrict__ poses, float* __restrict__ disps,
     const int64_t* __restrict__ ii, const int64_t* __restrict__ jj, int HW, int t0, int t1,
-    int motion_only, int depth_only, float* __restrict__ dx_out, float* __restrict__ dz_out) {
+    int motion_only, int depth_only, float* __restrict__ dx_out, float* __restrict__ dz_out, int B, int M,
+    float disp_floor) {
   if (ba_skipped(wk)) return;
   constexpr int EB = 128;
   __shared__ float ys[EB * 6];
@@ -1117,6 +1118,7 @@
       }
     }
   }
+  if (disp_floor > 0.0f) floor_other_frames(wk, disps, B, HW, M, disp_floor, [&](int) { return !motion_only; });
   if (motion_only) return;
   const int k = wk.kx[s];
   const int e0 = wk.csr_ptr[s];
@@ -1153,7 +1155,8 @@
   }
   if (px >= HW) return;
   const float dz = wk.Q[(size_t)s * HW + px] * (wk.W[(size_t)s * HW + px] - dw);
-  disps[(size_t)k * HW + px] += dz;
+  const float dnew = disps[(size_t)k * HW + px] + dz;
+  disps[(size_t)k * HW + px] = disp_floor > 0.0f ? disp_floored(dnew, disp_floor) : dnew;
   if (dz_out) dz_out[(size_t)s * HW + px] = dz;
 }
 
@@ -1269,7 +1272,7 @@
 
 static int ba_solve_update(const BaPlan& pl, float* poses, float* disps, const int64_t* ii,
                            const int64_t* jj, float lm, float ep, int motion_only, int depth_only,
-                           float* dx_out, float* dz_out, bool from_acc, hipStream_t st) {
+                           float* dx_out, float* dz_out, bool from_acc, hipStream_t st, float disp_floor = 0.0f) {
   const BaWork& wk = pl.wk;
   const int n6 = pl.n6;
   if (n6 <= kSolveMaxN) {
@@ -1305,7 +1308,7 @@
   }
   const int upd_chunks = (pl.HW + kBaThreads - 1) / kBaThreads;
   hipLaunchKernelGGL(ba_update_kernel, dim3(upd_chunks, pl.M), dim3(kBaThreads), 0, st, wk, poses,
-                     disps, ii, jj, pl.HW, pl.t0, pl.t1, motion_only, depth_only, dx_out, dz_out);
+                     disps, ii, jj, pl.HW, pl.t0, pl.t1, motion_only, depth_only, dx_out, dz_out, pl.B, pl.M, disp_floor);
   return check_launch();
 }
 
@@ -1345,7 +1348,7 @@
     GLORIE_TRY(ba_build_system(pl, poses, disps, intrinsics, disps_sens, targets, weights, eta, ii, jj,
                                flags, !direct, st));
     GLORIE_TRY(ba_solve_update(pl, poses, disps, ii, jj, lm, ep, motion_only, depth_only, dx_out,
-                               dz_out, direct, st));
+                               dz_out, direct, st, it + 1 == iterations ? ctx->ba_disp_floor : 0.0f));
   }
   return GLORIE_OK;
 }
@@ -1409,6 +1412,12 @@
   return GLORIE_OK;
 }
 
+extern "C" int glorie_ba_set_disp_floor(glorie_ctx* ctx, float floor) {
+  if (!ctx) return GLORIE_EINVAL;
+  ctx->ba_disp_floor = floor > 0.0f ? floor : 0.0f;
+  return GLORIE_OK;
+}
+
 namespace glorie {
 __global__ __launch_bounds__(256) void hv_pack_kernel(const double* __restrict__ hv, double* __restrict__ packed,
                                                       int n, int unpack) {
diff --git a/glorie_slam_amd/csrc/conv.hip b/glorie_slam_amd/csrc/conv.hip
--- a/glorie_slam_amd/csrc/conv.hip
+++ b/glorie_slam_amd/csrc/conv.hip
@@ -392,14 +392,12 @@
 __device__ __forceinline__ float round_prob(float v, bool f32) { return f32 ? v : (float)(_Float16)v; }
 
 template <int MB, int NB>
-__device__ __forceinline__ void conv_epilogue_upsample(const ConvArgs& a, f32x4 (&acc)[MB][NB], long p0, int n0, int wm,
-                                                       int wn, int kg, int col, char* smem) {
+__device__ __forceinline__ void upsample_logits_to_lds(const ConvArgs& a, f32x4 (&acc)[MB][NB], int n0, int wm, int wn,
+                                                       int kg, int col, _Float16* T) {
   static_assert(MB == 4 && NB == 4, "128 x 128 tile");
-  _Float16* T = reinterpret_cast<_Float16*>(smem);
   float4 bias[MB];
 #pragma unroll
   for (int mi = 0; mi < MB; ++mi) bias[mi] = *reinterpret_cast<const float4*>(a.terms + n0 + wm * 64 + mi * 16 + kg * 4);
-  __syncthreads();
 #pragma unroll
   for (int ni = 0; ni < NB; ++ni) {
     const int pl = wn * 64 + ni * 16 + col;
@@ -412,49 +410,148 @@
       *reinterpret_cast<f16x4*>(T + pl * 128 + ((b ^ (pl & 7)) * 16 + kg * 4)) = h;
     }
   }
+}
+
+struct UpPixel { int frame, y, x; float nb[9]; };
+
+__device__ __forceinline__ UpPixel upsample_pixel(const ConvArgs& a, long p) {
+  UpPixel u;
+  const int m = (int)(p / a.HW);
+  const int q = (int)(p - (long)m * a.HW);
+  u.y = q / a.W; u.x = q - u.y * a.W;
+  u.frame = (int)a.up_ix[m];
+  const float* dmap = a.up_disps + (size_t)u.frame * a.HW;
+#pragma unroll
+  for (int k = 0; k < 9; ++k) {
+    const int yy = u.y + k / 3 - 1, xx = u.x + k % 3 - 1;
+    const bool in = yy >= 0 && yy < a.H && xx >= 0 && xx < a.W;
+    u.nb[k] = dmap[in ? yy * a.W + xx : q];
+    if (!in) u.nb[k] = 0.0f;
+  }
+  return u;
+}
+
+__device__ __forceinline__ void upsample_finish(const ConvArgs& a, const _Float16* T, int pl, int hb, int asub,
+                                                const UpPixel& u) {
+  float outv[4];
+#pragma unroll
+  for (int j = 0; j < 4; ++j) {
+    const int b = hb * 4 + j;
+    const f16x8* src = reinterpret_cast<const f16x8*>(T + pl * 128 + (b ^ (pl & 7)) * 16);
+    const f16x8 lo = src[0], hi = src[1];
+    float v[9];
+#pragma unroll
+    for (int k = 0; k < 8; ++k) v[k] = (float)lo[k];
+    v[8] = (float)hi[0];
+    float mx = v[0];
+#pragma unroll
+    for (int k = 1; k < 9; ++k) mx = fmaxf(mx, v[k]);
+    float e[9], sum = 0.0f;
+#pragma unroll
+    for (int k = 0; k < 9; ++k) { e[k] = expf(v[k] - mx); sum += e[k]; }
+    float o = 0.0f;
+#pragma unroll
+    for (int k = 0; k < 9; ++k)
+      o = __fadd_rn(o, __fmul_rn(round_prob(e[k] / sum, a.up_f32 != 0), u.nb[k]));
+    outv[j] = o;
+  }
+  float* dst = a.up_out + (size_t)u.frame * 64 * a.HW + (size_t)(8 * u.y + asub) * (8 * a.W) + 8 * u.x + hb * 4;
+  *reinterpret_cast<float4*>(dst) = make_float4(outv[0], outv[1], outv[2], outv[3]);
+}
+
+template <int MB, int NB>
+__device__ __forceinline__ void conv_epilogue_upsample(const ConvArgs& a, f32x4 (&acc)[MB][NB], long p0, int n0, int wm,
+                                                       int wn, int kg, int col, char* smem) {
+  _Float16* T = reinterpret_cast<_Float16*>(smem);
+  __syncthreads();
+  upsample_logits_to_lds<MB, NB>(a, acc, n0, wm, wn, kg, col, T);
   __syncthreads();
   const int tid = threadIdx.x;
   const int pl = tid & 127, hb = tid >> 7;
   const long p = p0 + pl;
   if (p >= a.P) return;
-  const int asub = n0 >> 7;
-  const int m = (int)(p / a.HW);
-  const int q = (int)(p - (long)m * a.HW);
-  const int y = q / a.W, x = q - y * a.W;
-  const int frame = (int)a.up_ix[m];
-  const float* dmap = a.up_disps + (size_t)frame * a.HW;
-  float nb[9];
-#pragma unroll
-  for (int k = 0; k < 9; ++k) {
-    const int yy = y + k / 3 - 1, xx = x + k % 3 - 1;
-    const bool in = yy >= 0 && yy < a.H && xx >= 0 && xx < a.W;
-    nb[k] = dmap[in ? yy * a.W + xx : q];
-    if (!in) nb[k] = 0.0f;
-  }
-  float outv[4];
-#pragma unroll
-  for (int j = 0; j < 4; ++j) {
-    const int b = hb * 4 + j;
-    const f16x8* src = reinterpret_cast<const f16x8*>(T + pl * 128 + (b ^ (pl & 7)) * 16);
-    const f16x8 lo = src[0], hi = src[1];
-    float v[9];
-#pragma unroll
-    for (int k = 0; k < 8; ++k) v[k] = (float)lo[k];
-    v[8] = (float)hi[0];
-    float mx = v[0];
-#pragma unroll
-    for (int k = 1; k < 9; ++k) mx = fmaxf(mx, v[k]);
-    float e[9], sum = 0.0f;
-#pragma unroll
-    for (int k = 0; k < 9; ++k) { e[k] = expf(v[k] - mx); sum += e[k]; }
-    float o = 0.0f;
-#pragma unroll
-    for (int k = 0; k < 9; ++k)
-      o = __fadd_rn(o, __fmul_rn(round_prob(e[k] / sum, a.up_f32 != 0), nb[k]));
-    outv[j] = o;
-  }
-  float* dst = a.up_out + (size_t)frame * 64 * a.HW + (size_t)(8 * y + asub) * (8 * a.W) + 8 * x + hb * 4;
-  *reinterpret_cast<float4*>(dst) = make_float4(outv[0], outv[1], outv[2], outv[3]);
+  const UpPixel u = upsample_pixel(a, p);
+  upsample_finish(a, T, pl, hb, n0 >> 7, u);
+}
+
+__global__ __launch_bounds__(256, 2) void conv_upsample_kernel(ConvArgs a) {
+#if defined(__HIP_DEVICE_COMPILE__)
+  constexpr int MB = 4, NB = 4, RB = 128, C = 128, WCH = 128 * RB;
+  extern __shared__ __attribute__((aligned(16))) char smem[];
+  _Float16* T = reinterpret_cast<_Float16*>(smem);
+  char* lw = smem + 128 * 256;
+  const int tid = threadIdx.x, lane = tid & 63, wv = tid >> 6;
+  const int col = lane & 15, kg = lane >> 4;
+  const int wm = wv & 1, wn = wv >> 1;
+  const long p0 = (long)blockIdx.x * 128;
+
+  const __amdgpu_buffer_rsrc_t rW = __builtin_amdgcn_make_buffer_rsrc((void*)a.w, 0, 0x7fffffff, 0x00020000);
+  const int srow = lane >> 3, slot = lane & 7;
+  const int row0 = wv * 8 + srow;
+  const unsigned woff0 = (unsigned)((row0 * C + ((slot ^ (row0 & 7)) << 3)) * 2);
+  auto stage_w = [&](int nt) {
+#pragma unroll
+    for (int ch = 0; ch < 2; ++ch)
+#pragma unroll
+      for (int i = 0; i < 4; ++i)
+        __builtin_amdgcn_raw_ptr_buffer_load_lds(rW, (__attribute__((address_space(3))) void*)(lw + ch * WCH + (i * 4 + wv) * 8 * RB),
+                                                 16, woff0, (unsigned)(((nt * 128 + i * 32) * C + ch * 64) * 2), 0, 0);
+  };
+  stage_w(0);
+
+  f16x8 xf[2][2][NB];
+#pragma unroll
+  for (int ni = 0; ni < NB; ++ni) {
+    const long pr = min(p0 + wn * 64 + ni * 16 + col, a.P - 1);
+    const f16x8* src = reinterpret_cast<const f16x8*>(a.xa + pr * a.xa_stride + kg * 8);
+#pragma unroll
+    for (int ch = 0; ch < 2; ++ch)
+#pragma unroll
+      for (int kk = 0; kk < 2; ++kk) xf[ch][kk][ni] = src[ch * 8 + kk * 4];
+  }
+  const int pl = tid & 127, hb = tid >> 7;
+  const bool live = p0 + pl < a.P;
+  const UpPixel u = upsample_pixel(a, live ? p0 + pl : a.P - 1);
+
+  int foff[2];
+#pragma unroll
+  for (int kk = 0; kk < 2; ++kk) foff[kk] = col * RB + (((kk * 4 + kg) ^ (col & 7)) << 4);
+  const char* wbase = lw + wm * 64 * RB;
+
+#pragma unroll 1
+  for (int nt = 0; nt < 8; ++nt) {
+    asm volatile("s_waitcnt vmcnt(0)" ::: "memory");
+    __syncthreads();
+    f16x8 wf[2][2][MB];
+#pragma unroll
+    for (int ch = 0; ch < 2; ++ch)
+#pragma unroll
+      for (int kk = 0; kk < 2; ++kk)
+#pragma unroll
+        for (int mi = 0; mi < MB; ++mi)
+          wf[ch][kk][mi] = *reinterpret_cast<const f16x8*>(wbase + ch * WCH + mi * 16 * RB + foff[kk]);
+    asm volatile("s_waitcnt lgkmcnt(0)" ::: "memory");
+    __builtin_amdgcn_s_barrier();
+    if (nt + 1 < 8) stage_w(nt + 1);
+    f32x4 acc[MB][NB];
+#pragma unroll
+    for (int mi = 0; mi < MB; ++mi)
+#pragma unroll
+      for (int ni = 0; ni < NB; ++ni) acc[mi][ni] = f32x4{0.f, 0.f, 0.f, 0.f};
+#pragma unroll
+    for (int ch = 0; ch < 2; ++ch)
+#pragma unroll
+      for (int kk = 0; kk < 2; ++kk)
+#pragma unroll
+        for (int mi = 0; mi < MB; ++mi)
+#pragma unroll
+          for (int ni = 0; ni < NB; ++ni)
+            acc[mi][ni] = __builtin_amdgcn_mfma_f32_16x16x32_f16(wf[ch][kk][mi], xf[ch][kk][ni], acc[mi][ni], 0, 0, 0);
+    upsample_logits_to_lds<MB, NB>(a, acc, nt * 128, wm, wn, kg, col, T);
+    __syncthreads();
+    if (live) upsample_finish(a, T, pl, hb, nt, u);
+  }
+#endif
 }
 
 template <int EPI, int NB, int BK, int NW, int ST, int MB = 4>
@@ -1464,6 +1561,19 @@
       break;
     default: launch_one<EPI_GRU_Q, NB, BK, NW, ST, MB>(a, grid, st); break;
   }
+  return check_launch();
+}
+
+static int launch_conv_upsample(const ConvArgs& a, hipStream_t st) {
+  constexpr size_t lds = 64 * 1024;
+  static PerDeviceOnce attr;
+  if (attr.first()) {
+    (void)hipFuncSetAttribute(reinterpret_cast<const void*>(conv_upsample_kernel),
+                              hipFuncAttributeMaxDynamicSharedMemorySize, (int)lds);
+  }
+  const long ptiles = (a.P + 127) / 128;
+  if (ptiles > 0x7fffffffL) return GLORIE_EINVAL;
+  hipLaunchKernelGGL(conv_upsample_kernel, dim3((unsigned)ptiles), dim3(256), lds, st, a);
   return check_launch();
 }
 
@@ -1545,6 +1655,7 @@
         return launch_conv_halo<4>(a, epilogue, st);
     }
   }
+  if (epilogue == EPI_UPSAMPLE && ca == 128 && cb == 0 && policy == 0) return launch_conv_upsample(a, st);
   if (epilogue == EPI_HEADS || epilogue == EPI_UPSAMPLE) return launch_conv<4, 64, 4, 1>(a, epilogue, st);
   if (nout <= 64 && epilogue == EPI_BIAS_ACT) return launch_conv<4, 64, 4, 1, 2>(a, epilogue, st);
   const int ntn = (nout + 127) / 128;
diff --git a/glorie_slam_amd/csrc/dspo.hip b/glorie_slam_amd/csrc/dspo.hip
--- a/glorie_slam_amd/csrc/dspo.hip
+++ b/glorie_slam_amd/csrc/dspo.hip
@@ -163,7 +163,7 @@
 template <bool INLINE>
 __global__ __launch_bounds__(kBaThreads) void dspo2_update_kernel(BaWork wk, Dspo2Args a, int HW,
                                                                   float* __restrict__ dz_out, int M, int nchunks,
-                                                                  float lm, float ep) {
+                                                                  float lm, float ep, int B, float disp_floor) {
   __shared__ double vsum[INLINE ? 25 * 10 : 1];
   __shared__ float sdx[INLINE ? 2 * 25 : 1];
   __shared__ int fail;
@@ -215,6 +215,8 @@
     ds = wk.dx[2 * s + 0];
     dq = wk.dx[2 * s + 1];
   }
+  if (disp_floor > 0.0f)
+    floor_other_frames(wk, a.disps, B, HW, M, disp_floor, [&](int sl) { return frame_enabled(wk, a.edge_on, sl); });
   if (!frame_enabled(wk, a.edge_on, s)) return;
   const int k = wk.kx[s];
   if (blockIdx.x == 0 && tid == 0) {
@@ -226,7 +228,8 @@
   const PriorJ J = prior_jacobians(a.mono[(size_t)k * HW + px], a.vmask[(size_t)k * HW + px] != 0, a.alpha);
   const float dz = wk.Q[(size_t)s * HW + px] *
                    (wk.W[(size_t)s * HW + px] - (J.Js * J.Jd * ds + J.Jq * J.Jd * dq));
-  a.disps[(size_t)k * HW + px] = fmaxf(a.disps[(size_t)k * HW + px] + dz, 0.0f);
+  const float dnew = fmaxf(a.disps[(size_t)k * HW + px] + dz, 0.0f);
+  a.disps[(size_t)k * HW + px] = disp_floor > 0.0f ? disp_floored(dnew, disp_floor) : dnew;
   if (dz_out) dz_out[(size_t)s * HW + px] = dz;
 }
 
@@ -277,14 +280,15 @@
   Dspo2Args a{poses, disps, intrinsics, mono_disps, scales, shifts, valid_mask, target, weight, eta,
               ii, jj, edge_on, alpha};
   for (int it = 0; it < iterations; ++it) {
+    const float fl = it + 1 == iterations ? ctx->ba_disp_floor : 0.0f;
     hipLaunchKernelGGL(dspo2_accum_kernel, dim3(nchunks, M), dim3(kBaThreads), 0, st, wk, a, HW, w, nchunks);
     if (M <= 25) {
       hipLaunchKernelGGL(dspo2_update_kernel<true>, dim3(nchunks, M), dim3(kBaThreads), 0, st, wk, a, HW, dz_out, M,
-                         nchunks, lm, ep);
+                         nchunks, lm, ep, B, fl);
     } else {
       hipLaunchKernelGGL(dspo2_solve_kernel, dim3(1), dim3(256), 0, st, wk, a, M, nchunks, lm, ep);
       hipLaunchKernelGGL(dspo2_update_kernel<false>, dim3(nchunks, M), dim3(kBaThreads), 0, st, wk, a, HW, dz_out, M,
-                         nchunks, lm, ep);
+                         nchunks, lm, ep, B, fl);
     }
     GLORIE_TRY(check_launch());
   }
diff --git a/glorie_slam_amd/csrc/gru.hip b/glorie_slam_amd/csrc/gru.hip
--- a/glorie_slam_amd/csrc/gru.hip
+++ b/glorie_slam_amd/csrc/gru.hip
@@ -294,6 +294,56 @@
   else if (act == ACT_SOFTPLUS) acc = softplusf_(acc);
   if (out_last && grp == groups - 1) out_last[(size_t)p * K + j] = acc * scale;
   else out[((size_t)grp * P + p) * K + j] = acc * scale;
+}
+
+__global__ __launch_bounds__(256) void update_finish_kernel(
+    const float* __restrict__ head_taps, const float* __restrict__ head_bias, float* __restrict__ delta,
+    float* __restrict__ weight, const float* __restrict__ coords1, float* __restrict__ target, long P, int H, int W,
+    int pix_blocks, const float* __restrict__ eta_taps, const float* __restrict__ eta_bias, float* __restrict__ eta,
+    const int64_t* __restrict__ frames, float* __restrict__ damping_table, float* __restrict__ damping_ba, long n_eta,
+    float ep, int64_t* __restrict__ age, int n_age) {
+#pragma clang fp contract(off)
+  const long gi = (long)blockIdx.x * 256 + threadIdx.x;
+  if (age && gi < n_age) age[gi] += 1;
+  if ((int)blockIdx.x < pix_blocks) {
+    const long p = gi;
+    if (p >= P) return;
+    const int xw = (int)(p % W), yh = (int)((p / W) % H);
+    float acc[4];
+#pragma unroll
+    for (int gk = 0; gk < 4; ++gk) acc[gk] = head_bias[gk];
+#pragma unroll
+    for (int d = 0; d < 9; ++d) {
+      const int dy = d / 3 - 1, dx = d % 3 - 1;
+      if ((unsigned)(yh + dy) < (unsigned)H && (unsigned)(xw + dx) < (unsigned)W) {
+        const long q = p + dy * W + dx;
+#pragma unroll
+        for (int gk = 0; gk < 4; ++gk) acc[gk] += head_taps[(size_t)((gk >> 1) * 18 + d * 2 + (gk & 1)) * P + q];
+      }
+    }
+    const float2 c1 = reinterpret_cast<const float2*>(coords1)[p];
+    reinterpret_cast<float2*>(delta)[p] = make_float2(acc[0], acc[1]);
+    reinterpret_cast<float2*>(target)[p] = make_float2(c1.x + acc[0], c1.y + acc[1]);
+    reinterpret_cast<float2*>(weight)[p] = make_float2(sigmoidf_(acc[2]), sigmoidf_(acc[3]));
+  } else {
+    const long i = gi - (long)pix_blocks * 256;
+    if (i >= n_eta) return;
+    const int HW = H * W;
+    const int xw = (int)(i % W), yh = (int)((i / W) % H);
+    float acc = eta_bias[0];
+#pragma unroll
+    for (int d = 0; d < 9; ++d) {
+      const int dy = d / 3 - 1, dx = d % 3 - 1;
+      if ((unsigned)(yh + dy) < (unsigned)H && (unsigned)(xw + dx) < (unsigned)W)
+        acc += eta_taps[(i + dy * W + dx) * 9 + d];
+    }
+    const float e = softplusf_(acc) * 0.01f;
+    eta[i] = e;
+    const long g = i / HW;
+    damping_table[(size_t)frames[g] * HW + (i - g * HW)] = e;
+    const float m = e * 0.2f;
+    damping_ba[i] = m + ep;
+  }
 }
 
 }
@@ -503,3 +553,30 @@
                      taps, 9 * K, 9 * K * groups, out_bias, K, groups, act_packed, scale, out, P, H, W, out_last);
   return check_launch();
 }
+
+extern "C" int glorie_update_finish(const float* head_taps, const float* head_bias, float* delta, float* weight,
+                                    const float* coords1, float* target, const void* x, int x_stride,
+                                    const void* eta_w, const float* eta_bias, float* eta_taps, float* eta,
+                                    const int64_t* frames, float* damping_table, float* damping_ba, float ep,
+                                    int64_t* age, int n_age, int N, int G, int H, int W, void* stream) {
+  if (N < 0 || G < 0 || H <= 0 || W <= 0 || n_age < 0 || (x_stride & 7)) return GLORIE_EINVAL;
+  const long HW = (long)H * W, P = (long)N * HW, n_eta = (long)G * HW;
+  if (P >= (1L << 31) / 36 || n_eta >= (1L << 31) / 9) return GLORIE_EUNSUPPORTED;
+  if (P && (!head_taps || !head_bias || !delta || !weight || !coords1 || !target)) return GLORIE_EINVAL;
+  if (n_eta && (!x || !eta_w || !eta_bias || !eta_taps || !eta || !frames || !damping_table || !damping_ba))
+    return GLORIE_EINVAL;
+  const long pix_blocks = (P + 255) / 256, eta_blocks = (n_eta + 255) / 256;
+  if (pix_blocks + eta_blocks == 0) return n_age ? GLORIE_EINVAL : GLORIE_OK;
+  if (n_age > (pix_blocks + eta_blocks) * 256) return GLORIE_EINVAL;
+  hipStream_t st = (hipStream_t)stream;
+  if (n_eta) {
+    const long ntiles = (n_eta + 15) / 16;
+    hipLaunchKernelGGL(conv_taps_kernel<1>, dim3((unsigned)min((ntiles + 3) / 4, (long)2048), 1), dim3(256), 0, st,
+                       reinterpret_cast<const _Float16*>(x), x_stride, nullptr, 0,
+                       reinterpret_cast<const f16x8*>(eta_w), eta_taps, 9, 9, n_eta);
+  }
+  hipLaunchKernelGGL(update_finish_kernel, dim3((unsigned)(pix_blocks + eta_blocks)), dim3(256), 0, st, head_taps,
+                     head_bias, delta, weight, coords1, target, P, H, W, (int)pix_blocks, eta_taps, eta_bias, eta, frames,
+                     damping_table, damping_ba, n_eta, ep, age, n_age);
+  return check_launch();
+}
diff --git a/glorie_slam_amd/depth_video.py b/glorie_slam_amd/depth_video.py
--- a/glorie_slam_amd/depth_video.py
+++ b/glorie_slam_amd/depth_video.py
@@ -307,11 +307,17 @@
                                      target, weight, eta.contiguous(), ii, jj, t0, t1, itrs, lm, ep,
                                      motion_only, False, group=self.shard["group"], targets_hwc=True,
                                      force_collective=self.shard["force"])
+                    self.disps.clamp_(min=1e-5)
+                elif itrs > 0 and self.disps.is_cuda and self.disps.is_contiguous() and ii.shape[0] > 0 and t1 > t0:
+                    droid_backends.ba(self.poses, self.disps, self.intrinsics[0].contiguous(), None,
+                                      target, weight, eta, ii, jj, t0, t1, itrs, lm, ep, motion_only,
+                                      False, ctx=self.ctx(), want_updates=False, targets_hwc=True, gate=gate,
+                                      disp_floor=1e-5)
                 else:
                     droid_backends.ba(self.poses, self.disps, self.intrinsics[0].contiguous(), None,
                                       target, weight, eta, ii, jj, t0, t1, itrs, lm, ep, motion_only,
                                       False, ctx=self.ctx(), want_updates=False, targets_hwc=True, gate=gate)
-                self.disps.clamp_(min=1e-5)
+                    self.disps.clamp_(min=1e-5)
                 return True
             elif opt_type == "depth_scale":
                 from . import dspo as _dspo
diff --git a/glorie_slam_amd/droid_backends.py b/glorie_slam_amd/droid_backends.py
--- a/glorie_slam_amd/droid_backends.py
+++ b/glorie_slam_amd/droid_backends.py
@@ -354,7 +354,8 @@
 
 
 def ba(poses, disps, intrinsics, disps_sens, targets, weights, eta, ii, jj, t0, t1,
-       iterations, lm, ep, motion_only, depth_only=False, ctx=None, want_updates=True, targets_hwc=False, gate=None):
+       iterations, lm, ep, motion_only, depth_only=False, ctx=None, want_updates=True, targets_hwc=False, gate=None,
+       disp_floor=0.0):
     L.need_cuda(poses, disps, intrinsics, targets, weights, ii, jj)
     L.need_contiguous(targets=targets, weights=weights, poses=poses, disps=disps,
                       intrinsics=intrinsics, disps_sens=disps_sens, ii=ii, jj=jj)
@@ -377,6 +378,8 @@
     lib = L.load()
     if gate is not None:
         L.check(lib.glorie_ba_set_gate(ctx.handle, L.ptr(gate[0]), L.ptr(gate[1])), "glorie_ba_set_gate")
+    if disp_floor > 0:
+        L.check(lib.glorie_ba_set_disp_floor(ctx.handle, float(disp_floor)), "glorie_ba_set_disp_floor")
     try:
         L.check(lib.glorie_ba(ctx.handle, L.ptr(poses), L.ptr(disps), L.ptr(intrinsics),
                               L.ptr(disps_sens), L.ptr(targets), L.ptr(weights), L.ptr(eta),
@@ -389,6 +392,8 @@
     finally:
         if gate is not None:
             lib.glorie_ba_set_gate(ctx.handle, None, None)
+        if disp_floor > 0:
+            lib.glorie_ba_set_disp_floor(ctx.handle, 0.0)
     if _CHECK_STATUS:
         st = ctx.ba_status()
         if st[0] & 1:
diff --git a/glorie_slam_amd/droid_net.py b/glorie_slam_amd/droid_net.py
--- a/glorie_slam_amd/droid_net.py
+++ b/glorie_slam_amd/droid_net.py
@@ -337,7 +337,7 @@
 
     @torch.no_grad()
     def __call__(self, net, inp, corr, flow=None, ii=None, jj=None, groups=None, context=None, lazy_up=False,
-                 weight_out=None):
+                 weight_out=None, book=None):
         from . import update_ops as U
         self._sync()
         W = self.W
@@ -448,12 +448,18 @@
                 evh.append((h0, h1e))
             wo = weight_out if (weight_out is not None and weight_out.is_cuda and weight_out.dtype == torch.float32
                                 and weight_out.is_contiguous() and weight_out.numel() == n * ht * wd * 2) else None
-            dw = U.conv_stencil(rows, W["h2_b"], n, ht, wd, 2, 2, (U.ACT_NONE, U.ACT_SIGMOID), out_last=wo)
+            finish = book is not None and wo is not None and ii is not None and lazy_up
+            if book is not None and not finish:
+                raise RuntimeError("FusedUpdate: book needs weight_out, ii and lazy_up")
+            dw = None if finish else U.conv_stencil(rows, W["h2_b"], n, ht, wd, 2, 2, (U.ACT_NONE, U.ACT_SIGMOID),
+                                                    out_last=wo)
         else:
+            if book is not None:
+                raise RuntimeError("FusedUpdate: book needs fuse_heads")
             h1 = U.conv_igemm(new, None, W["h1"], 9, 384, cl_map(384), terms=W["h1_b"], act=U.ACT_RELU)
             dw = U.conv3x3_small(h1, W["h2"], W["h2_b"], 2, (U.ACT_NONE, U.ACT_SIGMOID))
             agg_in = h1[:, 256:384]
-        delta = dw[0].view(batch, num, ht, wd, 2)
+        delta = dw[0].view(batch, num, ht, wd, 2) if dw is not None else None
         weight = dw[1].view(batch, num, ht, wd, 2) if (not self.fuse_heads or wo is None) else \
             weight_out.view(batch, num, ht, wd, 2)
         if ii is None:
@@ -467,6 +473,12 @@
         a2 = torch.empty((ngroups, 128, ht, wd), dtype=torch.float16, device=dev,
                          memory_format=torch.channels_last)
         U.conv_igemm(agg, None, W["a2"], 9, 128, a2, terms=W["a2_b"], act=U.ACT_RELU)
+        if dw is None:
+            coords1, target, frames, damping_table, ep, age = book
+            delta, eta, damping_ba = U.update_finish(rows, W["h2_b"], wo, a2, W["eta"], W["eta_b"], coords1, target,
+                                                     frames, damping_table, ep, age)
+            return net_out, delta.view(batch, num, ht, wd, 2), weight, eta.view(batch, ngroups, ht, wd), \
+                U.LazyUpmask(a2, W["up_cvx"], W["up_cvx_b"]), damping_ba
         eta = U.conv3x3_small(a2, W["eta"], W["eta_b"], 1, (U.ACT_SOFTPLUS,), scale=0.01)
         if lazy_up:
             return net_out, delta, weight, eta.view(batch, ngroups, ht, wd), U.LazyUpmask(a2, W["up_cvx"], W["up_cvx_b"])
diff --git a/glorie_slam_amd/dspo.py b/glorie_slam_amd/dspo.py
--- a/glorie_slam_amd/dspo.py
+++ b/glorie_slam_amd/dspo.py
@@ -4,7 +4,7 @@
 from .common import align_scale_and_shift
 
 
-def scale_shift_step(video, target, weight, eta, ii, jj, edge_on, itrs, lm, ep, alpha=0.01):
+def scale_shift_step(video, target, weight, eta, ii, jj, edge_on, itrs, lm, ep, alpha=0.01, disp_floor=0.0):
     h, w = video.ht // video.down_scale, video.wd // video.down_scale
     target = target.reshape(-1, h, w, 2).contiguous().float()
     weight = weight.reshape(-1, h, w, 2).contiguous().float()
@@ -12,12 +12,21 @@
     N, M, B = ii.shape[0], eta.shape[0], video.disps.shape[0]
     vm = video.valid_depth_mask_small.contiguous().view(torch.uint8)
     eo = edge_on.to(torch.uint8).contiguous() if edge_on is not None else None
-    L.check(L.load().glorie_dspo_scale_shift(
-        video.ctx().handle, L.ptr(video.poses), L.ptr(video.disps), L.ptr(video.intrinsics),
-        L.ptr(video.mono_disps), L.ptr(video.depth_scale), L.ptr(video.depth_shift), L.ptr(vm),
-        L.ptr(target), L.ptr(weight), L.ptr(eta), L.ptr(ii.contiguous()), L.ptr(jj.contiguous()),
-        L.ptr(eo), B, N, M, h, w, int(itrs), float(lm), float(ep), float(alpha), None,
-        L.stream_ptr()), "glorie_dspo_scale_shift")
+    floored = disp_floor > 0 and N > 0 and M > 0 and h * w > 0 and int(itrs) > 0 and video.disps.is_contiguous()
+    lib, ctx = L.load(), video.ctx()
+    if floored:
+        L.check(lib.glorie_ba_set_disp_floor(ctx.handle, float(disp_floor)), "glorie_ba_set_disp_floor")
+    try:
+        L.check(lib.glorie_dspo_scale_shift(
+            ctx.handle, L.ptr(video.poses), L.ptr(video.disps), L.ptr(video.intrinsics),
+            L.ptr(video.mono_disps), L.ptr(video.depth_scale), L.ptr(video.depth_shift), L.ptr(vm),
+            L.ptr(target), L.ptr(weight), L.ptr(eta), L.ptr(ii.contiguous()), L.ptr(jj.contiguous()),
+            L.ptr(eo), B, N, M, h, w, int(itrs), float(lm), float(ep), float(alpha), None,
+            L.stream_ptr()), "glorie_dspo_scale_shift")
+    finally:
+        if floored:
+            lib.glorie_ba_set_disp_floor(ctx.handle, 0.0)
+    return floored
 
 
 def _prepare_torch(video, n, ii, jj):
@@ -61,8 +70,8 @@
         if any_on.is_cuda and not video.is_sharded() and not torch.cuda.is_current_stream_capturing():
             if n <= 0:
                 return False
-            scale_shift_step(video, target, weight, eta, ii, jj, edge_on, itrs, lm, ep, alpha=0.01)
-            video.disps.clamp_(min=1e-5)
+            if not scale_shift_step(video, target, weight, eta, ii, jj, edge_on, itrs, lm, ep, alpha=0.01, disp_floor=1e-5):
+                video.disps.clamp_(min=1e-5)
             return any_on
         if any_on.is_cuda and torch.cuda.is_current_stream_capturing():
             if not self_publish:
@@ -72,6 +81,7 @@
             return False
     if n <= 0:
         return False
-    scale_shift_step(video, target, weight, eta, ii, jj, edge_on, itrs, lm, ep, alpha=0.01)
-    video.disps.clamp_(min=1e-5)
+    if not scale_shift_step(video, target, weight, eta, ii, jj, edge_on, itrs, lm, ep, alpha=0.01,
+                            disp_floor=0.0 if video.is_sharded() else 1e-5):
+        video.disps.clamp_(min=1e-5)
     return True
diff --git a/glorie_slam_amd/factor_graph.py b/glorie_slam_amd/factor_graph.py
--- a/glorie_slam_amd/factor_graph.py
+++ b/glorie_slam_amd/factor_graph.py
@@ -363,12 +363,25 @@
         else:
             lookup = lambda: self.corr(coords1)
         uniq = self._unique_ii()
+        damping_done = None
         if self.fast_update is not None:
             ix, _ = self._groups()
-            self.net, delta, weight, damping, upmask = \
-                self.fast_update(self.net, self.inp, lookup, motn, self.ii, self.jj, self._groups(),
-                                 context=(self.video.inps, uniq, ix) if self.share_context else None,
-                                 lazy_up=True, weight_out=self.weight)
+            hw2 = int(self.ii.shape[0]) * self.ht * self.wd * 2
+            finish = (self.fast_update.fuse_heads and not use_inactive and not self.video.is_sharded() and coords1.is_cuda
+                      and self.target.shape == coords1.shape and self.target.dtype == torch.float32
+                      and self.target.is_contiguous() and coords1.is_contiguous() and coords1.dtype == torch.float32
+                      and coords1.numel() == hw2 and self.weight.is_cuda and self.weight.dtype == torch.float32
+                      and self.weight.is_contiguous() and self.weight.numel() == hw2
+                      and self.damping.is_cuda and self.damping.dtype == torch.float32 and self.damping.is_contiguous()
+                      and tuple(self.damping.shape[1:]) == (self.ht, self.wd) and uniq.is_contiguous()
+                      and self.age.is_cuda and self.age.dtype == torch.int64 and self.age.is_contiguous())
+            out = self.fast_update(self.net, self.inp, lookup, motn, self.ii, self.jj, self._groups(),
+                                   context=(self.video.inps, uniq, ix) if self.share_context else None,
+                                   lazy_up=True, weight_out=self.weight,
+                                   book=(coords1, self.target, uniq, self.damping, float(EP), self.age) if finish else None)
+            self.net, delta, weight, damping, upmask = out[:5]
+            if finish:
+                damping_done = out[5]
         else:
             corr = lookup()
             with torch.autocast("cuda", enabled=True):
@@ -385,7 +398,10 @@
                       and self.damping.dtype == torch.float32 and self.damping.is_contiguous()
                       and damping.numel() == uniq.shape[0] * self.ht * self.wd and self.age.is_contiguous())
         damping_ba = None
-        if fused_book:
+        if damping_done is not None:
+            damping_ba, fused_book = damping_done, True
+            self._age_done = True
+        elif fused_book:
             from . import _lib as L
             damping_ba = torch.empty((uniq.shape[0], self.ht, self.wd), dtype=torch.float32, device=coords1.device)
             L.check(L.load().glorie_update_bookkeeping(
diff --git a/glorie_slam_amd/update_ops.py b/glorie_slam_amd/update_ops.py
--- a/glorie_slam_amd/update_ops.py
+++ b/glorie_slam_amd/update_ops.py
@@ -283,6 +283,37 @@
     return out
 
 
+def update_finish(rows, head_bias, weight_out, x, eta_w, eta_bias, coords1, target, frames, damping_table, ep, age):
+    L.need_cuda(rows, x, eta_w, coords1, target, frames, damping_table, weight_out)
+    g, c, h, w = x.shape
+    P = rows.shape[1]
+    n = P // (h * w)
+    f32c = lambda t, numel: t.dtype == torch.float32 and t.is_contiguous() and t.numel() == numel
+    if rows.dtype != torch.float32 or rows.shape[0] != 36 or n * h * w != P or not rows.is_contiguous() or c != 128:
+        raise RuntimeError("update_finish: bad tap planes / hidden map")
+    if not (f32c(coords1, 2 * P) and f32c(target, 2 * P) and f32c(weight_out, 2 * P) and f32c(head_bias, 4)
+            and f32c(eta_bias, 1)):
+        raise RuntimeError("update_finish: coords1 / target / weight_out must be contiguous float32 [n,h,w,2]")
+    if frames.dtype != torch.int64 or frames.numel() != g or not frames.is_contiguous() or damping_table.dtype != torch.float32 \
+            or not damping_table.is_contiguous() or damping_table[0].numel() != h * w:
+        raise RuntimeError("update_finish: frames int64 [g] / damping_table float32 [B,h,w] expected")
+    if eta_w.dtype != torch.float16 or tuple(eta_w.shape) != (1, 1, 4, 64, 8) or not eta_w.is_contiguous():
+        raise RuntimeError("update_finish: eta_w must come from pack_conv3x3_small (one group, K = 1)")
+    if age is not None and (age.dtype != torch.int64 or not age.is_contiguous() or not age.is_cuda):
+        raise RuntimeError("update_finish: age must be a contiguous int64 device tensor")
+    dev = rows.device
+    delta = torch.empty((n, h, w, 2), dtype=torch.float32, device=dev)
+    eta = torch.empty((g, h, w), dtype=torch.float32, device=dev)
+    damping_ba = torch.empty((g, h, w), dtype=torch.float32, device=dev)
+    taps = torch.empty((g * h * w, 9), dtype=torch.float32, device=dev)
+    L.check(L.load().glorie_update_finish(
+        L.ptr(rows), L.ptr(head_bias), L.ptr(delta), L.ptr(weight_out), L.ptr(coords1), L.ptr(target), L.ptr(x),
+        _rows(x, "x"), L.ptr(eta_w), L.ptr(eta_bias), L.ptr(taps), L.ptr(eta), L.ptr(frames), L.ptr(damping_table),
+        L.ptr(damping_ba), float(ep), L.ptr(age), int(age.shape[0]) if age is not None else 0, n, g, h, w,
+        L.stream_ptr()), "glorie_update_finish")
+    return delta, eta, damping_ba
+
+
 def pack_flow_conv7(weight):
     if tuple(weight.shape) != (128, 4, 7, 7):
         raise RuntimeError("pack_flow_conv7: expected [128,4,7,7]")
diff --git a/include/glorie_hip.h b/include/glorie_hip.h
--- a/include/glorie_hip.h
+++ b/include/glorie_hip.h
@@ -73,6 +73,12 @@
 int glorie_update_bookkeeping(const float* coords1, const float* delta, float* target, long n_target,
                               const float* eta, const int64_t* frames, float* damping_table, float* damping_ba,
                               int G, int HW, float ep, int64_t* age, int n_edges, void* stream);
+
+int glorie_update_finish(const float* head_taps, const float* head_bias, float* delta, float* weight,
+                         const float* coords1, float* target, const void* x, int x_stride, const void* eta_w,
+                         const float* eta_bias, float* eta_taps, float* eta, const int64_t* frames,
+                         float* damping_table, float* damping_ba, float ep, int64_t* age, int n_age, int N, int G, int H,
+                         int W, void* stream);
 
 int glorie_bias_act(const void* x, int x_stride, const float* bias, void* y, int y_stride,
                     long P, int C, int act, void* stream);
@@ -168,6 +174,8 @@
 
 int glorie_ba_set_gate(glorie_ctx* ctx, const int* run_if_zero, int* hits);
 
+int glorie_ba_set_disp_floor(glorie_ctx* ctx, float floor);
+
 #define GLORIE_COMM_ID_BYTES 128
 int glorie_comm_unique_id(void* id_out);
 int glorie_comm_init(glorie_ctx* ctx, const void* id, int rank, int world);
```
